# UVA-Computer-Vision-Lab/FrameINO

Hardware: AMD Instinct MI355X
Metric: denoise-steps/sec (Wan2.2-5B FrameINO, 49f 704x1280, cond+uncond DiT forward + CFG + Euler) (higher is better)
Workload: dtype bf16; 1 GPU; wan2.2-5b-49f-704x1280; layers=30, id_frames=1, hip_graph=False, parallelism=single, dead_rows_last_block=1760

## Files before the change

### frameino_amd/_lib.py

```python
import ctypes
import os
import re

_HERE = os.path.dirname(os.path.abspath(__file__))
LIB_PATH = os.environ.get("FINO_LIB_PATH") or os.path.join(_HERE, "lib", "libframeino_hip.so")
HEADER_PATH = os.path.join(os.path.dirname(_HERE), "include", "frameino_hip.h")

c_void_p, c_int, c_i64, c_float = ctypes.c_void_p, ctypes.c_int, ctypes.c_int64, ctypes.c_float

SIGNATURES = {
    "fino_version": [],
    "fino_last_error": [],
    "fino_tune_set": [c_int, c_int],
    "fino_tune_get": [c_int],
    "fino_adaln_modulate": [c_void_p, c_void_p, c_i64, c_int, c_i64, c_i64, c_void_p, c_void_p, c_i64, c_void_p,
                            c_float, c_int, c_void_p],
    "fino_layernorm": [c_void_p, c_void_p, c_i64, c_int, c_i64, c_i64, c_void_p, c_void_p, c_float, c_int, c_void_p],
    "fino_gated_residual": [c_void_p, c_void_p, c_void_p, c_i64, c_int, c_i64, c_i64, c_i64, c_void_p, c_i64,
                            c_void_p, c_int, c_void_p],
    "fino_gated_residual_staged": [c_void_p, c_void_p, c_void_p, c_i64, c_int, c_i64, c_i64, c_i64, c_void_p, c_i64,
                                   c_void_p, c_int, c_void_p],
    "fino_layernorm_zero": [c_void_p, c_void_p, c_i64, c_int, c_i64, c_i64, c_void_p, c_void_p, c_void_p, c_void_p,
                            c_i64, c_void_p, c_float, c_int, c_void_p],
    "fino_rmsnorm_rope": [c_void_p, c_i64, c_int, c_i64, c_void_p, c_float, c_void_p, c_void_p, c_int, c_int,
                          c_void_p],
    "fino_rmsnorm_rope_scaled": [c_void_p, c_i64, c_int, c_i64, c_void_p, c_float, c_void_p, c_void_p, c_int, c_float,
                                 c_int, c_void_p],
    "fino_qkv_rmsnorm_rope": [c_void_p, c_i64, c_int, c_i64, c_void_p, c_float, c_void_p, c_float, c_void_p, c_void_p, c_int,
                              c_float, c_void_p, c_void_p, c_void_p, c_int, c_void_p],
    "fino_rmsnorm_rope_scatter": [c_void_p, c_i64, c_int, c_i64, c_void_p, c_float, c_void_p, c_void_p, c_int, c_float,
                                  c_void_p, c_void_p, c_void_p, c_int, c_void_p],
    "fino_diag_mfma_peak": [c_int, c_int, c_int, c_void_p, ctypes.POINTER(ctypes.c_double), c_void_p],
    "fino_headnorm_rope": [c_void_p, c_int, c_i64, c_int, c_int, c_i64, c_i64, c_void_p, c_void_p, c_float,
                           c_void_p, c_void_p, c_i64, c_int, c_void_p],
    "fino_headnorm_rope_scaled": [c_void_p, c_int, c_i64, c_int, c_int, c_i64, c_i64, c_void_p, c_void_p, c_float,
                                  c_void_p, c_void_p, c_i64, c_float, c_int, c_void_p],
    "fino_attn_fwd": [c_void_p] * 4 + [c_int, c_int, c_i64, c_i64, c_int] + [c_i64] * 12 + [c_float, c_int, c_void_p],
    "fino_attn_fwd_ws": [c_void_p] * 4 + [c_int, c_int, c_i64, c_i64, c_int] + [c_i64] * 12 +
                        [c_float, c_int, c_void_p, c_i64, c_void_p],
    "fino_attn_workspace_bytes": [c_int, c_int, c_i64, c_i64, c_int],
    "fino_attn_tail_supported": [c_int, c_int, c_i64, c_i64, c_int],
    "fino_attn_ranges_supported": [c_int, c_int, c_i64, c_i64, c_int],
    "fino_attn_fwd_ranges": [c_void_p] * 4 + [c_int, c_int, c_i64, c_i64, c_int] + [c_i64] * 12 + [c_float, c_int, c_void_p, c_void_p],
    "fino_attn_tiles_supported": [c_int, c_int, c_i64, c_i64, c_int],
    "fino_attn_fwd_tiles": [c_void_p] * 4 + [c_int, c_int, c_i64, c_i64, c_int] + [c_i64] * 12 + [c_float, c_int, c_void_p, c_i64, c_i64,
                                                                                             c_int, c_void_p],
    "fino_attn_tile_plan_bytes": [c_int, c_int, c_i64, c_i64, c_int],
    "fino_attn_tile_plan": [c_void_p] * 2 + [c_int, c_int, c_i64, c_i64, c_int] + [c_i64] * 6 + [c_float, c_int, c_float, c_void_p,
                                                                                             c_void_p, c_int, c_void_p, c_i64, c_void_p],
    "fino_attn_fp8_ranges_supported": [c_int, c_int, c_i64, c_i64, c_int],
    "fino_attn_fwd_fp8_ranges": [c_void_p] * 4 + [c_int, c_int, c_i64, c_i64, c_int] + [c_i64] * 8 + [c_float, c_int, c_int, c_void_p,
                                                                                               c_i64, c_int, c_void_p, c_void_p],
    "fino_attn_fwd_tail": [c_void_p] * 4 + [c_int, c_int, c_i64, c_i64, c_int] + [c_i64] * 12 + [c_float, c_int, c_void_p, c_void_p,
                                                                                            c_void_p],
    "fino_attn_probs_supported": [c_int, c_int, c_i64, c_i64, c_int],
    "fino_attn_probs": [c_void_p] * 3 + [c_int, c_int, c_i64, c_i64, c_int] + [c_i64] * 6 + [c_int, c_i64, c_i64, c_float, c_int,
                                                                                         c_void_p, c_void_p, c_void_p, c_i64,
                                                                                         c_void_p, c_void_p],
    "fino_row_rrms": [c_void_p, c_i64, c_int, c_i64, c_float, c_void_p, c_int, c_void_p],
    "fino_attn_fp8_kv_bytes": [c_int, c_int, c_i64, c_int],
    "fino_attn_fwd_fp8": [c_void_p] * 4 + [c_int, c_int, c_i64, c_i64, c_int] + [c_i64] * 8 + [c_float, c_int, c_int, c_void_p,
                                                                                           c_i64, c_void_p],
    "fino_attn_fp8_smooth_kv_bytes": [c_int, c_int, c_i64, c_int],
    "fino_attn_fwd_fp8_smooth": [c_void_p] * 4 + [c_int, c_int, c_i64, c_i64, c_int] + [c_i64] * 8 + [c_float, c_int, c_int,
                                                                                                  c_void_p, c_i64, c_void_p],
    "fino_attn_fp8_smoothed_kv_bytes": [c_int, c_int, c_i64, c_int, c_int],
    "fino_attn_fwd_fp8_smoothed": [c_void_p] * 4 + [c_int, c_int, c_i64, c_i64, c_int] + [c_i64] * 8 + [c_float, c_int, c_int,
                                                                                                    c_void_p, c_i64, c_void_p, c_int],
    "fino_attn_partial_bytes": [c_int, c_int, c_i64, c_int],
    "fino_attn_partial": [c_void_p] * 3 + [c_int, c_int, c_i64, c_i64, c_int] + [c_i64] * 9 + [c_float, c_int, c_void_p,
                                                                                               c_i64, c_void_p],
    "fino_attn_merge": [c_void_p, c_int, c_int, c_i64, c_int, c_i64, c_i64, c_i64, c_void_p, c_void_p, c_void_p, c_int,
                        c_void_p],
    "fino_mxfp8_scale_bytes": [c_i64, c_i64],
    "fino_quantize_mxfp8": [c_void_p, c_void_p, c_void_p, c_i64, c_i64, c_i64, c_int, c_void_p],
    "fino_gemm_mxfp8": [c_void_p] * 6 + [c_i64] * 4 + [c_int, c_void_p, c_i64, c_void_p, c_i64, c_void_p, c_int, c_void_p],
    "fino_gemm_mxfp8_keep": [c_void_p] * 6 + [c_i64] * 4 + [c_int, c_void_p, c_i64, c_void_p, c_i64, c_void_p, c_int, c_void_p,
                             c_i64, c_void_p],
    "fino_gemm_mxfp8_q": [c_void_p] * 7 + [c_i64] * 3 + [c_int, c_int, c_void_p],
    "fino_mxfp6_bytes": [c_i64, c_i64],
    "fino_mxfp6_scale_bytes": [c_i64, c_i64],
    "fino_quantize_mxfp6": [c_void_p, c_void_p, c_void_p, c_i64, c_i64, c_i64, c_int, c_void_p],
    "fino_gemm_mxfp6": [c_void_p] * 6 + [c_i64] * 4 + [c_int, c_void_p, c_i64, c_void_p, c_i64, c_void_p, c_int, c_void_p],
    "fino_gemm_mxfp6_keep": [c_void_p] * 6 + [c_i64] * 4 + [c_int, c_void_p, c_i64, c_void_p, c_i64, c_void_p, c_int, c_void_p,
                             c_i64, c_void_p],
    "fino_traj_paint": [c_void_p, c_void_p, c_void_p, c_int, c_int, c_int, c_int, c_void_p],
    "fino_traj_blur_quantize": [c_void_p, c_void_p, c_void_p, c_void_p, c_int, c_int, c_int, c_int, c_void_p],
    "fino_groupnorm_workspace_bytes": [c_int],
    "fino_groupnorm_cl": [c_void_p, c_void_p] + [c_int] * 6 + [c_void_p, c_void_p, c_float, c_void_p, c_void_p] +
                         [c_int] * 4 + [c_void_p, c_i64, c_int, c_void_p],
    "fino_avg_pool_time2": [c_void_p, c_void_p] + [c_int] * 5 + [c_void_p],
    "fino_resize_area_pad_u8": [c_void_p, c_void_p] + [c_int] * 9 + [c_void_p],
    "fino_u8_hwc_to_chw_unit": [c_void_p, c_void_p, c_int, c_int, c_void_p],
    "fino_gemm": [c_void_p] * 4 + [c_i64] * 6 + [c_int, c_void_p, c_i64, c_void_p, c_i64, c_void_p, c_int, c_void_p],
    "fino_gemm_split_n": [c_void_p] * 4 + [c_i64] * 6 + [c_int, c_void_p, c_i64, c_void_p, c_i64, c_void_p, c_int, c_void_p,
                          c_i64, c_i64, c_int, c_void_p],
    "fino_gemm_keep": [c_void_p] * 4 + [c_i64] * 6 + [c_int, c_void_p, c_i64, c_void_p, c_i64, c_void_p, c_int, c_void_p,
                       c_i64, c_int, c_void_p],
    "fino_ln_mxfp8": [c_int, c_void_p, c_void_p, c_void_p, c_i64, c_int, c_i64, c_void_p, c_void_p, c_void_p, c_void_p, c_i64,
                      c_void_p, c_float, c_int, c_void_p],
    "fino_gemm_blocked_a": [c_void_p, c_void_p, c_void_p, c_void_p, c_i64, c_i64, c_i64, c_i64, c_i64, c_int, c_i64, c_i64, c_i64,
                            c_i64, c_void_p, c_i64, c_void_p, c_i64, c_void_p, c_int, c_int, c_void_p],
    "fino_gemm_plan": [c_i64, c_i64, ctypes.POINTER(c_i64), ctypes.POINTER(c_int)],
    "fino_skinny_linear": [c_void_p, c_void_p, c_void_p, c_void_p, c_int, c_i64, c_i64, c_int, c_int, c_void_p],
    "fino_patchify": [c_void_p, c_void_p] + [c_int] * 7 + [c_i64, c_int, c_void_p],
    "fino_unpatchify": [c_void_p, c_void_p] + [c_int] * 7 + [c_i64, c_int, c_void_p],
    "fino_wan_model_input": [c_void_p] * 5 + [c_int] * 6 + [c_void_p],
    "fino_cfg_euler_step": [c_void_p, c_void_p, c_void_p] + [c_int] * 5 + [c_float, c_void_p, c_int, c_int, c_void_p],
    "fino_cfg_unipc_step": [c_void_p] * 6 + [c_int] * 5 + [c_void_p, c_int, c_void_p],
    "fino_cfg_vpred_step": [c_void_p, c_void_p, c_i64, c_i64, c_void_p, c_int, c_int, c_void_p],
    "fino_cfg_dpm_step": [c_void_p, c_void_p, c_void_p, c_void_p, c_i64, c_i64, c_void_p, c_int, c_int, c_void_p],
    "fino_conv3d": [c_void_p] * 4 + [c_int] * 19 + [c_void_p, c_void_p, c_int, c_void_p],
    "fino_rmsnorm_silu_cl": [c_void_p, c_void_p, c_i64, c_int, c_int, c_void_p, c_int, c_int, c_void_p],
    "fino_split_bf16": [c_void_p, c_void_p, c_i64, c_int, c_i64, c_i64, c_int, ctypes.c_uint, c_void_p],
    "fino_rmsnorm_silu_cl_f32": [c_void_p, c_void_p, c_i64, c_int, c_int, c_void_p, c_int, c_int, ctypes.c_uint, c_void_p],
    "fino_conv3d_split": [c_void_p] * 4 + [c_int] * 20 + [c_void_p, c_void_p, c_void_p],
    "fino_vae_blend_tiles": [c_void_p, c_void_p] + [c_int] * 9 + [c_void_p],
    "fino_softmax_rows": [c_void_p, c_i64, c_int, c_i64, c_float, c_int, c_void_p],
    "fino_dup_up3d_add": [c_void_p] * 3 + [c_int] * 10 + [c_void_p],
    "fino_avg_down3d_add": [c_void_p] * 3 + [c_int] * 10 + [c_void_p],
    "fino_vae_unpatchify_clamp": [c_void_p, c_void_p] + [c_int] * 7 + [c_void_p],
    "fino_vae_patchify": [c_void_p, c_void_p] + [c_int] * 7 + [c_void_p],
    "fino_lora_merge": [c_void_p, c_i64, c_void_p, c_i64, c_i64, c_i64, c_int, ctypes.POINTER(c_void_p),
                        ctypes.POINTER(c_i64), ctypes.POINTER(c_void_p), ctypes.POINTER(c_i64), ctypes.POINTER(c_int),
                        ctypes.POINTER(c_float), c_int, c_void_p],
    "fino_step_cache_probe": [c_void_p, c_int, c_i64, c_void_p, c_void_p, c_int, c_void_p],
    "fino_step_cache_residual": [c_void_p, c_i64, c_void_p, c_i64, c_void_p, c_i64, c_i64, c_i64, c_int, c_int, c_void_p],
    "fino_pab_broadcast": [c_void_p, c_i64, c_void_p, c_i64, c_void_p, c_i64, c_i64, c_i64, c_void_p, c_i64, c_void_p, c_int,
                           c_void_p],
}


class StepCacheSegment(ctypes.Structure):
    _fields_ = [("h0", c_void_p), ("h1", c_void_p), ("p", c_void_p), ("r", c_void_p), ("h1_copy", c_void_p),
                ("rows", c_i64), ("ld_h0", c_i64), ("ld_h1", c_i64), ("ld_p", c_i64), ("ld_r", c_i64), ("ld_h1_copy", c_i64)]
_RESTYPES = {"fino_last_error": ctypes.c_char_p, "fino_attn_workspace_bytes": c_i64, "fino_mxfp8_scale_bytes": c_i64,
             "fino_groupnorm_workspace_bytes": c_i64,
             "fino_attn_partial_bytes": c_i64, "fino_attn_fp8_kv_bytes": c_i64, "fino_attn_fp8_smooth_kv_bytes": c_i64,
             "fino_attn_fp8_smoothed_kv_bytes": c_i64, "fino_mxfp6_bytes": c_i64,
             "fino_mxfp6_scale_bytes": c_i64, "fino_attn_tile_plan_bytes": c_i64}


ABI_VERSION = 103


def declared_symbols(header_path=HEADER_PATH):
    text = open(header_path).read()
    text = re.sub(r"/\*.*?\*/", "", text, flags=re.S)
    return sorted(set(re.findall(r"\b(fino_[a-z0-9_]+)\s*\(", text)))


def load(path=LIB_PATH):
    if not os.path.exists(path):
        raise RuntimeError(
            f"frameino_amd: HIP library not found at {path}. Build it with `python -c 'import __graft_entry__ as g; "
            f"g.build()'` (or `make -C frameino_amd/csrc`). There is no CPU fallback for the product path.")
    lib = ctypes.CDLL(path)
    lib.fino_version.restype = c_int
    if lib.fino_version() < 0 and os.environ.get("FINO_ALLOW_EXPERIMENT") != "1":
        raise RuntimeError(
            f"frameino_amd: {path} is a timing-EXPERIMENT build (compiled with -DFINO_EXPERIMENT: its kernels may skip "
            f"work and return wrong results; fino_version() = {lib.fino_version()}).  It is refused as the product library; "
            f"set FINO_ALLOW_EXPERIMENT=1 for the tools/ scripts that time it.")
    if abs(lib.fino_version()) != ABI_VERSION:
        raise RuntimeError(
            f"frameino_amd: {path} reports fino_version() = {lib.fino_version()}, this package binds ABI version "
            f"{ABI_VERSION} (include/frameino_hip.h: FINO_VERSION).  Rebuild it (`make -C frameino_amd/csrc`).")
    for name, argtypes in SIGNATURES.items():
        fn = getattr(lib, name)
        fn.argtypes = argtypes
        fn.restype = _RESTYPES.get(name, c_int)
    return lib


_lib = None


def lib():
    global _lib
    if _lib is None:
        _lib = load()
    return _lib


def check(rc, what=""):
    if rc != 0:
        raise RuntimeError(f"{what} failed ({rc}): {lib().fino_last_error().decode()}")
```

### frameino_amd/csrc/fino_gemm.hip

```cpp
#include <stdlib.h>

#include <atomic>
#include <type_traits>

#include "fino_gemm_common.h"

using namespace fino_gemm_ns;

#ifdef FINO_GEMM_STAMP
extern "C" int fino_gemm_debug_read(unsigned long long* out) {
    return (int)hipMemcpyFromSymbol(out, HIP_SYMBOL(fino_gemm_dbg), sizeof(unsigned long long) * 64);
}
#endif

namespace {

template <typename T, int EPI, bool GENERIC, bool CONV, bool KEEP = false>
__global__ __launch_bounds__(kThreads, 2) void gemm_kernel(const GemmParams p) {
    extern __shared__ __attribute__((aligned(16))) char smem[];
    typedef typename T::vec8 vec8;
    const int tid = threadIdx.x;
    const int lane = tid & 63;
    const int wave = tid >> 6;
    const int wm = wave >> 2;
    const int wn = wave & 3;

    int tm, tn;
    tile_coords(p, tm, tn);
    const int64_t m0 = (int64_t)tm * BM, n0 = (int64_t)tn * BN;

    const int srow = wave * 8 + (lane >> 3);
    const int sch = lane & 7;
    const uint16_t* a_src[4];
    const uint16_t* w_src[4];
    bool a_ok[4], w_ok[4];
    int sk[4];
#pragma unroll
    for (int j = 0; j < 4; ++j) {
        const int row = j * 64 + srow;
        const int lch = sch ^ swz(row);
        sk[j] = lch * 8;
        int64_t gm = m0 + row, gn = n0 + row;
        a_ok[j] = gm < p.m;
        w_ok[j] = gn < p.n;
        if (gm >= p.m) gm = p.m - 1;
        if (gn >= p.n) gn = p.n - 1;
        a_src[j] = p.a + gm * p.lda + sk[j];
        w_src[j] = p.w + gn * p.ldw + sk[j];
    }
    int pos_t[4], pos_h[4], pos_w[4];
    if constexpr (CONV) {
#pragma unroll
        for (int j = 0; j < 4; ++j) {
            int64_t gm = m0 + j * 64 + srow;
            if (gm >= p.m) gm = p.m - 1;
            const int hw = p.ho * p.wo;
            pos_t[j] = (int)(gm / hw);
            const int rem = (int)(gm - (int64_t)pos_t[j] * hw);
            pos_h[j] = rem / p.wo;
            pos_w[j] = rem - pos_h[j] * p.wo;
        }
    }
    auto stage = [&](int buf, int kt) {
        char* ab = smem + buf * kStageBytes;
        char* wb = ab + kTileBytes;
        const int64_t k0 = (int64_t)kt * BK;
        if constexpr (CONV) {
            const int tap = kt / p.cin_chunks;
            const int c0 = (kt - tap * p.cin_chunks) * BK;
            const int dw = tap % p.kw;
            const int dh = (tap / p.kw) % p.kh;
            const int dt = tap / (p.kw * p.kh);
            const int hlim = p.up ? 2 * p.hi : p.hi, wlim = p.up ? 2 * p.wi : p.wi;
#pragma unroll
            for (int j = 0; j < 4; ++j) {
                const int ti = pos_t[j] * p.st + dt - p.pt;
                int hi = pos_h[j] * p.sh + dh - p.ph;
                int wi = pos_w[j] * p.sw + dw - p.pw;
                const bool ok = a_ok[j] && ti >= 0 && ti < p.ti && hi >= 0 && hi < hlim && wi >= 0 && wi < wlim;
                if (p.up) { hi >>= 1; wi >>= 1; }
                const uint16_t* src = ok ? p.a + (((int64_t)ti * p.hi + hi) * p.wi + wi) * p.lda + c0 + sk[j]
                                         : p.zero_page + sk[j];
                __builtin_amdgcn_global_load_lds((const FINO_GLB void*)src,
                                                 (FINO_LDS void*)(ab + j * 8192 + wave * 1024), 16, 0, 0);
                __builtin_amdgcn_global_load_lds((const FINO_GLB void*)(w_src[j] + k0),
                                                 (FINO_LDS void*)(wb + j * 8192 + wave * 1024), 16, 0, 0);
            }
        } else if constexpr (!GENERIC) {
#pragma unroll
            for (int j = 0; j < 4; ++j) {
                __builtin_amdgcn_global_load_lds((const FINO_GLB void*)(a_src[j] + k0),
                                                 (FINO_LDS void*)(ab + j * 8192 + wave * 1024), 16, 0, 0);
                __builtin_amdgcn_global_load_lds((const FINO_GLB void*)(w_src[j] + k0),
                                                 (FINO_LDS void*)(wb + j * 8192 + wave * 1024), 16, 0, 0);
            }
        } else {
#pragma unroll
            for (int j = 0; j < 4; ++j) {
                const bool kin = k0 + sk[j] < p.k;
                uint4 va = make_uint4(0, 0, 0, 0), vw = make_uint4(0, 0, 0, 0);
                if (kin && a_ok[j]) va = *reinterpret_cast<const uint4*>(a_src[j] + k0);
                if (kin && w_ok[j]) vw = *reinterpret_cast<const uint4*>(w_src[j] + k0);
                *reinterpret_cast<uint4*>(ab + j * 8192 + tid * 16) = va;
                *reinterpret_cast<uint4*>(wb + j * 8192 + tid * 16) = vw;
            }
        }
    };

    auto stage_piece = [&](int buf, int kt, int piece) {
        char* ab = smem + buf * kStageBytes;
        char* wb = ab + kTileBytes;
        const int64_t k0 = (int64_t)kt * BK;
        const int j = piece & 3;
        if (piece >= 4) {
            __builtin_amdgcn_global_load_lds((const FINO_GLB void*)(w_src[j] + k0),
                                             (FINO_LDS void*)(wb + j * 8192 + wave * 1024), 16, 0, 0);
        } else if constexpr (CONV) {
            const int tap = kt / p.cin_chunks;
            const int c0 = (kt - tap * p.cin_chunks) * BK;
            const int dw = tap % p.kw;
            const int dh = (tap / p.kw) % p.kh;
            const int dt = tap / (p.kw * p.kh);
            const int hlim = p.up ? 2 * p.hi : p.hi, wlim = p.up ? 2 * p.wi : p.wi;
            const int ti = pos_t[j] * p.st + dt - p.pt;
            int hi = pos_h[j] * p.sh + dh - p.ph;
            int wi = pos_w[j] * p.sw + dw - p.pw;
            const bool ok = a_ok[j] && ti >= 0 && ti < p.ti && hi >= 0 && hi < hlim && wi >= 0 && wi < wlim;
            if (p.up) { hi >>= 1; wi >>= 1; }
            const uint16_t* src = ok ? p.a + (((int64_t)ti * p.hi + hi) * p.wi + wi) * p.lda + c0 + sk[j]
                                     : p.zero_page + sk[j];
            __builtin_amdgcn_global_load_lds((const FINO_GLB void*)src, (FINO_LDS void*)(ab + j * 8192 + wave * 1024),
                                             16, 0, 0);
        } else {
            __builtin_amdgcn_global_load_lds((const FINO_GLB void*)(a_src[j] + k0),
                                             (FINO_LDS void*)(ab + j * 8192 + wave * 1024), 16, 0, 0);
        }
    };

    const int frow = lane & 15;
    const int pch0 = (lane >> 4) ^ (frow >> 1);
    const int a_base = (wm * 128 + frow) * 128;
    const int w_base = kTileBytes + (wn * 64 + frow) * 128;

    f32x4_t acc[8][4];
#pragma unroll
    for (int i = 0; i < 8; ++i)
#pragma unroll
        for (int j = 0; j < 4; ++j) acc[i][j] = f32x4_t{0.f, 0.f, 0.f, 0.f};

    const int nk = (int)((p.k + BK - 1) / BK);
#define LOAD_FRAGS(SB_, KK_, WF_, AF_)                                                                           \
    {                                                                                                            \
        const int pch_ = (pch0 ^ ((KK_) << 2)) << 4;                                                             \
        _Pragma("unroll") for (int j_ = 0; j_ < 4; ++j_)                                                         \
            WF_[j_] = *reinterpret_cast<const u32x4_t*>((SB_) + w_base + j_ * 2048 + pch_);                      \
        _Pragma("unroll") for (int i_ = 0; i_ < 8; ++i_)                                                         \
            AF_[i_] = *reinterpret_cast<const u32x4_t*>((SB_) + a_base + i_ * 2048 + pch_);                      \
    }
#define MFMA_BLOCK(WF_, AF_)                                                                                     \
    _Pragma("unroll") for (int i_ = 0; i_ < 8; ++i_)                                                             \
        _Pragma("unroll") for (int j_ = 0; j_ < 4; ++j_)                                                         \
            acc[i_][j_] = T::mfma16(__builtin_bit_cast(vec8, WF_[j_]), __builtin_bit_cast(vec8, AF_[i_]), acc[i_][j_]);

    if constexpr (GENERIC) {
        stage(0, 0);
        __syncthreads();
        for (int kt = 0; kt < nk; ++kt) {
            const int cur = kt & 1;
            if (kt + 1 < nk) stage(cur ^ 1, kt + 1);
            const char* sb = smem + cur * kStageBytes;
#pragma unroll
            for (int kk = 0; kk < 2; ++kk) {
                u32x4_t wf[4], af[8];
                LOAD_FRAGS(sb, kk, wf, af)
                MFMA_BLOCK(wf, af)
            }
            __syncthreads();
        }
    } else {
        u32x4_t wfa[4], wfb[4], af[8], an;
#define LD_W(SB_, KK_, WF_)                                                                                       \
    _Pragma("unroll") for (int j_ = 0; j_ < 4; ++j_)                                                              \
        WF_[j_] = *reinterpret_cast<const u32x4_t*>((SB_) + w_base + j_ * 2048 + ((pch0 ^ ((KK_) << 2)) << 4));
#define LD_A(SB_, KK_, I_) (*reinterpret_cast<const u32x4_t*>((SB_) + a_base + (I_) * 2048 + ((pch0 ^ ((KK_) << 2)) << 4)))
#define K_STEP(WF_, SBN_, KKN_, HAS_NEXT_, DMA_)                                                                  \
    {                                                                                                             \
        if (HAS_NEXT_) an = LD_A(SBN_, KKN_, 0);                                                                  \
        _Pragma("unroll") for (int i_ = 0; i_ < 8; ++i_) {                                                        \
            if (DMA_) stage_piece(cur, kt + 2, i_);                 \
            _Pragma("unroll") for (int j_ = 0; j_ < 4; ++j_)                                                      \
                acc[i_][j_] = T::mfma16(__builtin_bit_cast(vec8, WF_[j_]), __builtin_bit_cast(vec8, af[i_]),      \
                                        acc[i_][j_]);                                                             \
            if (HAS_NEXT_) {                                                                                      \
                af[i_] = an;                                                                                      \
                if (i_ < 7) an = LD_A(SBN_, KKN_, i_ + 1);                                                        \
            }                                                                                                     \
            __builtin_amdgcn_sched_barrier(0);                                                                    \
        }                                                                                                         \
    }
        stage(0, 0);
        if (nk > 1) stage(1, 1);
        asm volatile("s_waitcnt vmcnt(0)" ::: "memory");
        __builtin_amdgcn_s_barrier();
        LD_W(smem, 0, wfa)
#pragma unroll
        for (int i = 0; i < 8; ++i) af[i] = LD_A(smem, 0, i);
#ifdef FINO_GEMM_STAMP
        unsigned long long t0, t1, t2, t3, t4, acc0 = 0, acc1 = 0, acc2 = 0, acc3 = 0;
#endif
        for (int kt = 0; kt < nk; ++kt) {
            const int cur = kt & 1;
            const char* sb = smem + cur * kStageBytes;
            const char* sbn = smem + (cur ^ 1) * kStageBytes;
#ifdef FINO_GEMM_STAMP
            __builtin_amdgcn_sched_barrier(0); STAMP(t0) __builtin_amdgcn_sched_barrier(0);
#endif
            LD_W(sb, 1, wfb)
            K_STEP(wfa, sb, 1, true, false)
#ifdef FINO_GEMM_STAMP
            __builtin_amdgcn_sched_barrier(0); STAMP(t1) __builtin_amdgcn_sched_barrier(0);
            asm volatile("s_waitcnt vmcnt(0)" ::: "memory");
            __builtin_amdgcn_sched_barrier(0); STAMP(t2) __builtin_amdgcn_sched_barrier(0);
            __builtin_amdgcn_s_barrier();
            __builtin_amdgcn_sched_barrier(0); STAMP(t3) __builtin_amdgcn_sched_barrier(0);
#else
            asm volatile("s_waitcnt vmcnt(0) lgkmcnt(0)" ::: "memory");
            __builtin_amdgcn_s_barrier();
#endif
            __builtin_amdgcn_sched_barrier(0);
            LD_W(sbn, 0, wfa)
            const bool dma = kt + 2 < nk;
            K_STEP(wfb, sbn, 0, true, dma)
#ifdef FINO_GEMM_STAMP
            __builtin_amdgcn_sched_barrier(0); STAMP(t4) __builtin_amdgcn_sched_barrier(0);
            acc0 += t1 - t0; acc1 += t2 - t1; acc2 += t3 - t2; acc3 += t4 - t3;
#endif
        }
#ifdef FINO_GEMM_STAMP
        if (blockIdx.x == 17 && lane == 0) {
            fino_gemm_dbg[wave * 8 + 0] = acc0; fino_gemm_dbg[wave * 8 + 1] = acc1;
            fino_gemm_dbg[wave * 8 + 2] = acc2; fino_gemm_dbg[wave * 8 + 3] = acc3;
            fino_gemm_dbg[wave * 8 + 4] = (unsigned long long)nk;
        }
#endif
        __syncthreads();
    }
#undef LD_W
#undef LD_A
#undef K_STEP
#undef LOAD_FRAGS
#undef MFMA_BLOCK

    gemm_epilogue<T, EPI, false, 8, KEEP>(acc, p, smem, m0, n0, tid, lane, wm, wn);
}

__device__ __forceinline__ int ablk_koff(const GemmParams& p, int kt) {
    const int b = (kt * p.a_inv) >> 16;
    const int j = (b * p.a_ginv) >> 16;
    return (b - j * p.a_groups) * (int)(p.a_grp_elems * 2) + j * (int)(p.a_blk_elems * 2) + (kt - b * p.a_tpb) * (BK * 2);
}

template <typename T, bool CONV, int MI, bool ABLK = false>
__device__ __forceinline__ void pp_mainloop(const GemmParams& p, char* smem, const int64_t m0, const int64_t n0,
                                            const int kb, const int nk, f32x4_t (&acc)[MI][4], const int tid,
                                            const int lane, const int wave, const int wm, const int wn) {
    typedef typename T::vec8 vec8;
    static_assert(MI >= 2 && MI <= 8, "tile height 64 .. 256");
    static_assert(!CONV || MI == 8, "the implicit-GEMM gather is built for 256-row tiles");
    enum : int { NA0 = (MI + 1) / 2, NA1 = MI - (MI + 1) / 2 };

    const int r8 = lane >> 3;
    const int sk = ((lane & 7) ^ ((4 * (wn & 1) + (lane >> 4)) & 7)) * 8;
    const __amdgpu_buffer_rsrc_t w_rsrc = __builtin_amdgcn_make_buffer_rsrc(
        (void*)p.w, 0, (int)(((p.n - 1) * p.ldw + p.k) * 2), 0x00020000);
    const int aq0 = wm == 0 ? 0 : NA0;
    uint32_t a_off[4], w_off[8];
    uint32_t pos[CONV ? 4 : 1];
    int ck = 0, tap_t = 0, tap_h = 0, tap_w = 0, t_first = 0, t_in_first = 0;
    int cseg = 0, seg = 0, a_koff = 0;
    const uint16_t* a_base_ptr = p.a;
    int64_t a_bytes = ((p.m - 1) * p.lda + p.k) * 2;
    if constexpr (ABLK)
        a_bytes = ((p.a_groups - 1) * p.a_grp_elems + (p.k / (BK * p.a_tpb) / p.a_groups - 1) * p.a_blk_elems +
                   (p.m - 1) * p.lda + BK * p.a_tpb) * 2;
    if constexpr (CONV) {
        const int hw = p.ho * p.wo;
        t_first = (int)(m0 / hw);
        t_in_first = t_first * p.st - p.pt;
        t_in_first = t_in_first < 0 ? 0 : t_in_first;
        const int64_t frame = (int64_t)p.hi * p.wi * p.lda;
        a_base_ptr = p.a + (int64_t)t_in_first * frame;
        a_bytes = (int64_t)(p.ti - t_in_first) * frame * 2;
        a_bytes = a_bytes > 0x7fffffffll ? 0x7fffffffll : a_bytes;
#pragma unroll
        for (int q = 0; q < NA0; ++q) {
            int64_t gm = m0 + (aq0 + q) * 32 + wn * 8 + r8;
            gm = gm < p.m ? gm : p.m - 1;
            const int t = (int)(gm / hw);
            const int rem = (int)(gm - (int64_t)t * hw);
            const int h = rem / p.wo;
            pos[q] = ((uint32_t)(t - t_first) << 24) | ((uint32_t)h << 12) | (uint32_t)(rem - h * p.wo);
        }
    }
    const __amdgpu_buffer_rsrc_t a_rsrc = __builtin_amdgcn_make_buffer_rsrc((void*)a_base_ptr, 0, (int)a_bytes, 0x00020000);
    auto conv_offsets = [&]() {
        const int hlim = p.up ? 2 * p.hi : p.hi, wlim = p.up ? 2 * p.wi : p.wi;
#pragma unroll
        for (int q = 0; q < NA0; ++q) {
            const int ti = (t_first + (int)(pos[CONV ? q : 0] >> 24)) * p.st + tap_t - p.pt;
            int hi = (int)((pos[CONV ? q : 0] >> 12) & 0xfffu) * p.sh + tap_h - p.ph;
            int wi = (int)(pos[CONV ? q : 0] & 0xfffu) * p.sw + tap_w - p.pw;
            const bool ok = (unsigned)ti < (unsigned)p.ti && (unsigned)hi < (unsigned)hlim && (unsigned)wi < (unsigned)wlim;
            if (p.up) { hi >>= 1; wi >>= 1; }
            const uint32_t off = (uint32_t)(((((ti - t_in_first) * p.hi + hi) * p.wi + wi) * (int)p.lda + sk) * 2);
            a_off[q] = ok ? off : 0x80000000u;
        }
    };
    auto conv_next = [&]() {
        if (p.a_cc > 0 && ++cseg == p.a_cc) { cseg = 0; ++seg; }
        if (++ck == p.cin_chunks) {
            ck = 0; cseg = 0; seg = 0;
            if (++tap_w == p.kw) {
                tap_w = 0;
                if (++tap_h == p.kh) { tap_h = 0; ++tap_t; }
            }
            conv_offsets();
        }
        if (p.a_cc > 0) {
            const int plane = p.a_nplanes == 3 ? (seg >= 3) + (seg >= 5) : (seg >= 2);
            a_koff = (plane * p.a_cc + cseg) * (BK * 2);
        } else {
            a_koff = ck * (BK * 2);
        }
    };
    if constexpr (CONV) {
        conv_offsets();
    } else {
#pragma unroll
        for (int q = 0; q < NA0; ++q) {
            int64_t gm = m0 + (aq0 + q) * 32 + wn * 8 + r8;
            gm = gm < p.m ? gm : p.m - 1;
            a_off[q] = (uint32_t)((gm * p.lda + sk) * 2);
        }
    }
    const int w_piece_bytes = (int)(32 * p.ldw * 2);
    const int w_pieces = CONV ? (int)((p.n - n0 + 31) / 32) : 8;
#pragma unroll
    for (int q = 0; q < 8; ++q) {
        int64_t gn = n0 + q * 32 + wn * 8 + r8;
        gn = gn < p.n ? gn : p.n - 1;
        w_off[q] = (uint32_t)((gn * p.ldw + sk) * 2);
    }
#ifndef GP_DMA_AUX
#define GP_DMA_AUX 0
#endif
#define PP_DMA_A(STAGE_, KT_, QI_)                                                                                \
    if ((QI_) < NA1 || wm == 0)                                                                                   \
        __builtin_amdgcn_raw_ptr_buffer_load_lds(                                                                 \
            a_rsrc, (FINO_LDS void*)(smem + (STAGE_) * kStageBytes + ((aq0 + (QI_)) * 32 + wn * 8) * 128), 16,    \
            a_off[QI_], CONV ? a_koff : (ABLK ? ablk_koff(p, kb + (KT_)) : (kb + (KT_)) * (BK * 2)), 0, GP_DMA_AUX);
#define PP_DMA_W(STAGE_, KT_, Q_)                                                                                 \
    if (!CONV || (Q_) < w_pieces)                                                                                 \
        __builtin_amdgcn_raw_ptr_buffer_load_lds(                                                                 \
            w_rsrc, (FINO_LDS void*)(smem + (STAGE_) * kStageBytes + kTileBytes + ((Q_) * 32 + wn * 8) * 128), 16, \
            w_off[CONV ? 0 : (Q_)], (kb + (KT_)) * (BK * 2) + (CONV ? (Q_) * w_piece_bytes : 0), 0, GP_DMA_AUX);

    const int frow = lane & 15;
    const int pch0 = (lane >> 4) ^ (frow >> 1);
    const int a_base = (wm * (16 * MI) + frow) * 128;
    const int w_base = kTileBytes + (wn * 64 + frow) * 128;

#pragma unroll
    for (int i = 0; i < MI; ++i)
#pragma unroll
        for (int j = 0; j < 4; ++j) acc[i][j] = f32x4_t{0.f, 0.f, 0.f, 0.f};

#pragma unroll
    for (int q = 0; q < 4; ++q) {
        if (q < NA0) { PP_DMA_A(0, 0, q) }
        if (wm == 0) { PP_DMA_W(0, 0, q) } else { PP_DMA_W(0, 0, 4 + q) }
    }
    if constexpr (CONV) conv_next();
    if (nk > 1) {
#pragma unroll
        for (int q = 0; q < 4; ++q) {
            if (q < NA0) { PP_DMA_A(1, 1, q) }
            if (wm == 0) { PP_DMA_W(1, 1, q) } else { PP_DMA_W(1, 1, 4 + q) }
        }
        if constexpr (CONV) conv_next();
    }
    asm volatile("s_waitcnt vmcnt(0)" ::: "memory");
    __builtin_amdgcn_s_barrier();
    if (wm == 1) __builtin_amdgcn_s_barrier();

    u32x4_t af[2][MI], wf[2][4];
#ifdef FINO_GEMM_STAMP
    unsigned long long t0, t1, t2, t3, t4, acc0 = 0, acc1 = 0, acc2 = 0, acc3 = 0;
#define PSTAMP(V_) { __builtin_amdgcn_sched_barrier(0); STAMP(V_) __builtin_amdgcn_sched_barrier(0); }
#else
#define PSTAMP(V_)
#endif
    for (int t = 0; t < nk; ++t) {
        const int cur = t & 1;
        const char* sb = smem + cur * kStageBytes;
        PSTAMP(t0)
#pragma unroll
        for (int kk = 0; kk < 2; ++kk) {
            const int pch = (pch0 ^ (kk << 2)) << 4;
#pragma unroll
            for (int j = 0; j < 4; ++j) wf[kk][j] = *reinterpret_cast<const u32x4_t*>(sb + w_base + j * 2048 + pch);
#pragma unroll
            for (int i = 0; i < MI; ++i) af[kk][i] = *reinterpret_cast<const u32x4_t*>(sb + a_base + i * 2048 + pch);
        }
        if (t >= 1 && t + 1 < nk) {
#pragma unroll
            for (int q = 0; q < NA0; ++q) PP_DMA_A(cur ^ 1, t + 1, q)
            if (wm == 0) {
#pragma unroll
                for (int q = 0; q < 8; ++q) { PP_DMA_W(cur ^ 1, t + 1, q) }
            }
            if constexpr (CONV) conv_next();
        }
        __builtin_amdgcn_sched_barrier(0);
        asm volatile("s_waitcnt lgkmcnt(0)" ::: "memory");
        PSTAMP(t1)
        __builtin_amdgcn_s_barrier();
        __builtin_amdgcn_sched_barrier(0);
        PSTAMP(t2)
#ifndef GP_ORDER
#define GP_ORDER 3
#endif
#pragma unroll
        for (int kk = 0; kk < 2; ++kk) {
#if GP_ORDER == 0
#pragma unroll
            for (int i = 0; i < MI; ++i) {
#pragma unroll
                for (int j = 0; j < 4; ++j)
                    acc[i][j] = T::mfma16(__builtin_bit_cast(vec8, wf[kk][j]), __builtin_bit_cast(vec8, af[kk][i]),
                                          acc[i][j]);
            }
#elif GP_ORDER == 1
#pragma unroll
            for (int j = 0; j < 4; ++j) {
#pragma unroll
                for (int i = 0; i < MI; ++i)
                    acc[i][j] = T::mfma16(__builtin_bit_cast(vec8, wf[kk][j]), __builtin_bit_cast(vec8, af[kk][i]),
                                          acc[i][j]);
            }
#elif GP_ORDER == 2
#pragma unroll
            for (int j = 0; j < 4; ++j) {
#pragma unroll
                for (int ii = 0; ii < MI; ++ii) {
                    const int i = ((j + 4 * kk) & 1) ? MI - 1 - ii : ii;
                    acc[i][j] = T::mfma16(__builtin_bit_cast(vec8, wf[kk][j]), __builtin_bit_cast(vec8, af[kk][i]),
                                          acc[i][j]);
                }
            }
#else
#pragma unroll
            for (int i = 0; i < MI; ++i) {
#pragma unroll
                for (int jj = 0; jj < 4; ++jj) {
                    const int j = ((i + MI * kk) & 1) ? 3 - jj : jj;
                    acc[i][j] = T::mfma16(__builtin_bit_cast(vec8, wf[kk][j]), __builtin_bit_cast(vec8, af[kk][i]),
                                          acc[i][j]);
                }
            }
#endif
        }
        __builtin_amdgcn_sched_barrier(0);
        asm volatile("s_waitcnt vmcnt(0)" ::: "memory");
        PSTAMP(t3)
        __builtin_amdgcn_s_barrier();
        __builtin_amdgcn_sched_barrier(0);
#ifdef FINO_GEMM_STAMP
        STAMP(t4)
        acc0 += t1 - t0; acc1 += t2 - t1; acc2 += t3 - t2; acc3 += t4 - t3;
#endif
    }
#ifdef FINO_GEMM_STAMP
    if (blockIdx.x == 17 && lane == 0) {
        fino_gemm_dbg[wave * 8 + 0] = acc0; fino_gemm_dbg[wave * 8 + 1] = acc1;
        fino_gemm_dbg[wave * 8 + 2] = acc2; fino_gemm_dbg[wave * 8 + 3] = acc3;
        fino_gemm_dbg[wave * 8 + 4] = (unsigned long long)nk;
    }
#endif
    if (wm == 0) __builtin_amdgcn_s_barrier();
    asm volatile("s_waitcnt vmcnt(0)" ::: "memory");
#undef PP_DMA_A
#undef PP_DMA_W
}

template <typename T, int EPI, bool CONV = false, int MI = 8, bool ABLK = false, bool KEEP = false>
__global__ __launch_bounds__(kThreads, 2) void gemm_pp_kernel(const GemmParams p) {
    extern __shared__ __attribute__((aligned(16))) char smem[];
    const int tid = threadIdx.x;
    const int lane = tid & 63;
    const int wave = __builtin_amdgcn_readfirstlane(tid >> 6);
    const int wm = wave >> 2;
    const int wn = wave & 3;
    int tm, tn;
    tile_coords(p, tm, tn);
    const int64_t m0 = (int64_t)tm * (32 * MI), n0 = (int64_t)tn * BN;
    int nk = (int)(p.k / BK);
#ifndef GP_RAGGED
#define GP_RAGGED 1
#endif
    if constexpr (GP_RAGGED && MI == 8 && !CONV && EPI != FINO_EPI_F32 && EPI != FINO_EPI_F32_RESIDUAL) {
        const int64_t rows = p.m - m0;
        if (rows <= 64) {
            f32x4_t acc2[2][4];
            pp_mainloop<T, false, 2, ABLK>(p, smem, m0, n0, 0, nk, acc2, tid, lane, wave, wm, wn);
            gemm_epilogue<T, EPI, false, 2, KEEP>(acc2, p, smem, m0, n0, tid, lane, wm, wn);
            return;
        }
        if (rows <= 128) {
            f32x4_t acc4[4][4];
            pp_mainloop<T, false, 4, ABLK>(p, smem, m0, n0, 0, nk, acc4, tid, lane, wave, wm, wn);
            gemm_epilogue<T, EPI, false, 4, KEEP>(acc4, p, smem, m0, n0, tid, lane, wm, wn);
            return;
        }
    }
    f32x4_t acc[MI][4];
#ifdef FINO_GEMM_STAMP
    unsigned long long ts0, ts1;
    STAMP(ts0)
#endif
    pp_mainloop<T, CONV, MI, ABLK>(p, smem, m0, n0, 0, nk, acc, tid, lane, wave, wm, wn);
#ifdef FINO_GEMM_STAMP
    STAMP(ts1)
    if (blockIdx.x == 17 && lane == 0) fino_gemm_dbg[wave * 8 + 5] = ts1 - ts0;
#endif
    gemm_epilogue<T, EPI, false, MI, KEEP>(acc, p, smem, m0, n0, tid, lane, wm, wn);
}

template <typename T, int EPI, bool GENERIC, bool CONV = false, bool KEEP = false>
int launch_gemm_t(const GemmParams& p, hipStream_t st) {
    static FinoPerDeviceOnce once;
    if (int rc = fino_max_smem_once(once, reinterpret_cast<const void*>(&gemm_kernel<T, EPI, GENERIC, CONV, KEEP>), kSmemBytes, "fino_gemm")) return rc;
    gemm_kernel<T, EPI, GENERIC, CONV, KEEP><<<dim3((unsigned)(p.tiles_m * p.tiles_n)), kThreads, kSmemBytes, st>>>(p);
    FINO_LAUNCH_CHECK();
    return FINO_OK;
}

template <typename T, int EPI, bool CONV = false, int MI = 8, bool ABLK = false, bool KEEP = false>
int launch_gemm_pp(const GemmParams& p, hipStream_t st) {
    static FinoPerDeviceOnce once;
    if (int rc = fino_max_smem_once(once, reinterpret_cast<const void*>(&gemm_pp_kernel<T, EPI, CONV, MI, ABLK, KEEP>), kSmemBytes, "fino_gemm")) return rc;
    gemm_pp_kernel<T, EPI, CONV, MI, ABLK, KEEP><<<dim3((unsigned)(p.tiles_m * p.tiles_n)), kThreads, kSmemBytes, st>>>(p);
    FINO_LAUNCH_CHECK();
    return FINO_OK;
}

inline int gemm_device_cus() {
    static std::atomic<int> cus[kFinoMaxDevices];
    const int dev = fino_current_device();
    int c = cus[dev].load(std::memory_order_relaxed);
    if (c == 0) {
        int n = 0;
        c = (hipDeviceGetAttribute(&n, hipDeviceAttributeMultiprocessorCount, dev) == hipSuccess && n > 0) ? n : 256;
        cus[dev].store(c, std::memory_order_relaxed);
    }
    return c;
}

struct TilePlan { int64_t rows1; int mi2; };
inline double plan_launch_cost(int64_t rows, int mi, int tiles_n, int cus) {
    if (rows <= 0) return 0.0;
    const double bm = 32.0 * mi;
    const int64_t tiles = ((rows + 32 * mi - 1) / (32 * mi)) * tiles_n;
    const double mfma_raw = 0.85 * bm / 256.0, mfma = mfma_raw > 0.80 ? mfma_raw : 0.80, deliver = (bm + 256.0) / 512.0;
    const int64_t full = tiles / cus, rem = tiles % cus;
    double c = (double)full * (mfma > deliver ? mfma : deliver);
    if (rem) {
        const double d = deliver * (double)rem / cus;
        c += mfma > d ? mfma : d;
    }
    return c + 0.07;
}
inline TilePlan plan_tiles_search(int64_t m, int tiles_n, int cus);
inline TilePlan plan_tiles(int64_t m, int tiles_n, int cus, int tile_m = 0) {
    const int forced = tile_m ? tile_m : fino_tune_get(FINO_TUNE_GEMM_TILE_M);
    if (forced >= 2 && forced <= 7) return TilePlan{0, forced};
    if (forced == 8 || m <= 0) return TilePlan{m, 8};
    static std::atomic<uint64_t> memo[64];
    const bool memoable = m < (1ll << 24) && tiles_n > 0 && tiles_n < 512 && cus > 0 && cus < 512;
    const uint64_t key = ((uint64_t)m << 18) | ((uint64_t)tiles_n << 9) | (uint64_t)cus;
    std::atomic<uint64_t>& slot = memo[(key * 0x9E3779B97F4A7C15ull) >> 58];
    if (memoable) {
        const uint64_t e = slot.load(std::memory_order_relaxed);
        if ((e & 1) && (e >> 22) == key) {
            const uint64_t r = (e >> 6) & 0xffff;
            return TilePlan{r == 0xffff ? m : (int64_t)r * 256, (int)((e >> 3) & 7) + 1};
        }
    }
    const TilePlan tp = plan_tiles_search(m, tiles_n, cus);
    if (memoable && (tp.rows1 == m || (tp.rows1 % 256 == 0 && tp.rows1 / 256 < 0xffff)) && tp.mi2 >= 2 && tp.mi2 <= 8)
        slot.store((key << 22) | ((tp.rows1 == m ? 0xffffull : (uint64_t)(tp.rows1 / 256)) << 6) |
                       ((uint64_t)(tp.mi2 - 1) << 3) | 1ull, std::memory_order_relaxed);
    return tp;
}
inline TilePlan plan_tiles_search(int64_t m, int tiles_n, int cus) {
    TilePlan best{m, 8};
    double best_c = plan_launch_cost(m, 8, tiles_n, cus);
    const double base_c = best_c;
    const int64_t rows256 = (m + 255) / 256;
    for (int64_t r1 = 0; r1 < rows256; ++r1) {
        const int64_t rows1 = r1 * 256;
        const double c1 = plan_launch_cost(rows1, 8, tiles_n, cus);
        for (int mi = 2; mi <= 8; ++mi) {
            if (rows1 > 0 && mi == 8) continue;
            const double c = c1 + plan_launch_cost(m - rows1, mi, tiles_n, cus);
            if (c < best_c - 1e-9) { best_c = c; best = TilePlan{rows1, mi}; }
        }
    }
    if (best_c > (best.rows1 > 0 ? 0.97 : 0.985) * base_c) return TilePlan{m, 8};
    return best;
}

inline bool use_pingpong() {
    static int v = -1;
    if (v < 0) {
        const char* e = getenv("FINO_GEMM_PP");
        v = (e && e[0] == '0') ? 0 : 1;
    }
    return v == 1;
}

template <typename T, int EPI, bool KEEP = false>
int launch_gemm_pp_mi(const GemmParams& p, int mi, hipStream_t st) {
    if constexpr (KEEP) {
        switch (mi) {
            case 2: return launch_gemm_pp<T, EPI, false, 2, false, true>(p, st);
            case 3: return launch_gemm_pp<T, EPI, false, 3, false, true>(p, st);
            case 4: return launch_gemm_pp<T, EPI, false, 4, false, true>(p, st);
            case 5: return launch_gemm_pp<T, EPI, false, 5, false, true>(p, st);
            case 6: return launch_gemm_pp<T, EPI, false, 6, false, true>(p, st);
            case 7: return launch_gemm_pp<T, EPI, false, 7, false, true>(p, st);
            default: return launch_gemm_pp<T, EPI, false, 8, false, true>(p, st);
        }
    }
    if (p.a_tpb > 0) {
        if constexpr (EPI == FINO_EPI_GATED_RESIDUAL) {
            switch (mi) {
                case 2: return launch_gemm_pp<T, EPI, false, 2, true>(p, st);
                case 3: return launch_gemm_pp<T, EPI, false, 3, true>(p, st);
                case 4: return launch_gemm_pp<T, EPI, false, 4, true>(p, st);
                case 5: return launch_gemm_pp<T, EPI, false, 5, true>(p, st);
                case 6: return launch_gemm_pp<T, EPI, false, 6, true>(p, st);
                case 7: return launch_gemm_pp<T, EPI, false, 7, true>(p, st);
                default: return launch_gemm_pp<T, EPI, false, 8, true>(p, st);
            }
        } else {
            fino_set_error("fino_gemm_blocked_a: epilogue must be FINO_EPI_GATED_RESIDUAL");
            return FINO_ERR_UNSUPPORTED;
        }
    }
    switch (mi) {
        case 2: return launch_gemm_pp<T, EPI, false, 2>(p, st);
        case 3: return launch_gemm_pp<T, EPI, false, 3>(p, st);
        case 4: return launch_gemm_pp<T, EPI, false, 4>(p, st);
        case 5: return launch_gemm_pp<T, EPI, false, 5>(p, st);
        case 6: return launch_gemm_pp<T, EPI, false, 6>(p, st);
        case 7: return launch_gemm_pp<T, EPI, false, 7>(p, st);
        default: return launch_gemm_pp<T, EPI, false, 8>(p, st);
    }
}

template <typename T, bool KEEP = false>
int launch_gemm_rows(GemmParams p, int64_t r0, int64_t rows, int mi, int epi, hipStream_t st) {
    p.a += r0 * p.lda;
    p.c += r0 * p.ldc;
    if (p.c2) p.c2 += r0 * p.ldc2;
    if (p.r) p.r += r0 * p.ldr;
    if (p.sel) p.sel += r0;
    p.m = rows;
    p.tiles_m = (int)((rows + 32 * mi - 1) / (32 * mi));
    if constexpr (KEEP) {
        switch (epi) {
            case FINO_EPI_RESIDUAL: return launch_gemm_pp_mi<T, FINO_EPI_RESIDUAL, true>(p, mi, st);
            case FINO_EPI_GATED_RESIDUAL_STAGED: return launch_gemm_pp_mi<T, FINO_EPI_GATED_RESIDUAL_STAGED, true>(p, mi, st);
            default: return launch_gemm_pp_mi<T, FINO_EPI_GATED_RESIDUAL, true>(p, mi, st);
        }
    }
    switch (epi) {
        case FINO_EPI_NONE: return launch_gemm_pp_mi<T, FINO_EPI_NONE>(p, mi, st);
        case FINO_EPI_GELU_TANH: return launch_gemm_pp_mi<T, FINO_EPI_GELU_TANH>(p, mi, st);
        case FINO_EPI_RESIDUAL: return launch_gemm_pp_mi<T, FINO_EPI_RESIDUAL>(p, mi, st);
        case FINO_EPI_GATED_RESIDUAL_STAGED: return launch_gemm_pp_mi<T, FINO_EPI_GATED_RESIDUAL_STAGED>(p, mi, st);
        default: return launch_gemm_pp_mi<T, FINO_EPI_GATED_RESIDUAL>(p, mi, st);
    }
}

template <typename T, bool GENERIC, bool KEEP = false>
int launch_gemm_e(const GemmParams& p, int epi, int tile_m, hipStream_t st) {
    const bool fits32 = ((p.m - 1) * p.lda + p.k) * 2 < (1ll << 31) && ((p.n - 1) * p.ldw + p.k) * 2 < (1ll << 31);
    if (epi == FINO_EPI_F32 || epi == FINO_EPI_F32_RESIDUAL) {
        if (GENERIC || !fits32) {
            fino_set_error("fino_gemm: the fp32-output epilogues need K %% 64 == 0, 16-byte aligned operands and operands < 2 GiB");
            return FINO_ERR_UNSUPPORTED;
        }
        return epi == FINO_EPI_F32 ? launch_gemm_pp<T, FINO_EPI_F32, false, 8>(p, st)
                                   : launch_gemm_pp<T, FINO_EPI_F32_RESIDUAL, false, 8>(p, st);
    }
    if (!GENERIC && use_pingpong() && fits32) {
        const TilePlan tp = plan_tiles(p.m, p.tiles_n, gemm_device_cus(), tile_m);
        if (tp.rows1 > 0)
            if (int rc = launch_gemm_rows<T, KEEP>(p, 0, tp.rows1, 8, epi, st)) return rc;
        if (tp.rows1 < p.m) return launch_gemm_rows<T, KEEP>(p, tp.rows1, p.m - tp.rows1, tp.mi2, epi, st);
        return FINO_OK;
    }
    if constexpr (KEEP) {
        switch (epi) {
            case FINO_EPI_RESIDUAL: return launch_gemm_t<T, FINO_EPI_RESIDUAL, GENERIC, false, true>(p, st);
            case FINO_EPI_GATED_RESIDUAL_STAGED: return launch_gemm_t<T, FINO_EPI_GATED_RESIDUAL_STAGED, GENERIC, false, true>(p, st);
            default: return launch_gemm_t<T, FINO_EPI_GATED_RESIDUAL, GENERIC, false, true>(p, st);
        }
    }
    switch (epi) {
        case FINO_EPI_NONE: return launch_gemm_t<T, FINO_EPI_NONE, GENERIC>(p, st);
        case FINO_EPI_GELU_TANH: return launch_gemm_t<T, FINO_EPI_GELU_TANH, GENERIC>(p, st);
        case FINO_EPI_RESIDUAL: return launch_gemm_t<T, FINO_EPI_RESIDUAL, GENERIC>(p, st);
        case FINO_EPI_GATED_RESIDUAL_STAGED: return launch_gemm_t<T, FINO_EPI_GATED_RESIDUAL_STAGED, GENERIC>(p, st);
        default: return launch_gemm_t<T, FINO_EPI_GATED_RESIDUAL, GENERIC>(p, st);
    }
}

template <int WT>
__global__ __launch_bounds__(256) void skinny_linear_kernel(const float* __restrict__ x, const void* __restrict__ w,
                                                            const void* __restrict__ b, float* __restrict__ y, int m,
                                                            int64_t n, int64_t k, int silu_input) {
    const int lane = threadIdx.x & 63;
    const int64_t col = (int64_t)blockIdx.x * 4 + (threadIdx.x >> 6);
    if (col >= n) return;
    float acc[16];
#pragma unroll
    for (int i = 0; i < 16; ++i) acc[i] = 0.f;
    for (int64_t kk = lane; kk < k; kk += 64) {
        float wv;
        if (WT == -1) wv = ((const float*)w)[col * k + kk];
        else if (WT == FINO_BF16) wv = BF16::to_f32(((const uint16_t*)w)[col * k + kk]);
        else wv = F16::to_f32(((const uint16_t*)w)[col * k + kk]);
#pragma unroll
        for (int i = 0; i < 16; ++i) {
            if (i < m) {
                float xv = x[(int64_t)i * k + kk];
                if (silu_input) xv = xv / (1.0f + __expf(-xv));
                acc[i] += xv * wv;
            }
        }
    }
    float bias = 0.f;
    if (b) {
        if (WT == -1) bias = ((const float*)b)[col];
        else if (WT == FINO_BF16) bias = BF16::to_f32(((const uint16_t*)b)[col]);
        else bias = F16::to_f32(((const uint16_t*)b)[col]);
    }
#pragma unroll
    for (int i = 0; i < 16; ++i) {
        if (i < m) {
            const float s = wave_sum(acc[i]);
            if (lane == 0) y[(int64_t)i * n + col] = s + bias;
        }
    }
}

}

extern "C" int fino_gemm_plan(int64_t m, int64_t n, int64_t* rows_256, int* tile_rows_rest) {
    if (m <= 0 || n <= 0) return FINO_ERR_ARG;
    const TilePlan tp = plan_tiles(m, (int)((n + BN - 1) / BN), gemm_device_cus());
    if (rows_256) *rows_256 = tp.rows1;
    if (tile_rows_rest) *tile_rows_rest = tp.rows1 < m ? 32 * tp.mi2 : 0;
    return FINO_OK;
}

extern "C" int fino_gemm(const void* a, const void* w, const void* bias, void* c, int64_t m, int64_t n, int64_t k,
                         int64_t lda, int64_t ldw, int64_t ldc, int epilogue, const void* r, int64_t ldr,
                         const float* gate, int64_t mod_stride, const int32_t* sel, int dtype, void* stream) {
    return fino_gemm_split_n(a, w, bias, c, m, n, k, lda, ldw, ldc, epilogue, r, ldr, gate, mod_stride, sel, dtype, nullptr,
                             0, 0, 0, stream);
}

static int gemm_impl(const void* a, const void* w, const void* bias, void* c, int64_t m, int64_t n, int64_t k, int64_t lda,
                     int64_t ldw, int64_t ldc, int epilogue, const void* r, int64_t ldr, const float* gate,
                     int64_t mod_stride, const int32_t* sel, int dtype, void* c2, int64_t ldc2, int64_t n_split, void* keep,
                     int64_t ldk, int tile_m, void* stream) {
    FINO_CHECK(dtype == FINO_BF16 || dtype == FINO_F16, FINO_ERR_ARG, "fino_gemm: dtype %d", dtype);
    FINO_CHECK(tile_m == 0 || (tile_m >= 2 && tile_m <= 8), FINO_ERR_ARG, "fino_gemm: tile_m=%d (0 = planned, 2 .. 8)", tile_m);
    if (c2 || n_split) {
        FINO_CHECK(c2 && n_split > 0 && n_split < n && n_split % BN == 0 && ldc2 % 8 == 0 && ldc2 >= n - n_split &&
                       fino_aligned16(c2) && k % BK == 0 && epilogue <= FINO_EPI_GELU_TANH,
                   FINO_ERR_ARG,
                   "fino_gemm_split_n: needs c2, 0 < n_split < N a multiple of %d, ldc2 >= N - n_split, K %% %d == 0, no "
                   "residual epilogue", BN, BK);
        FINO_CHECK(ldc >= n_split, FINO_ERR_ARG, "fino_gemm_split_n: ldc must cover the first n_split columns");
    }
    FINO_CHECK(a && w && c, FINO_ERR_ARG, "fino_gemm: null pointer");
    FINO_CHECK(m >= 0 && n > 0 && k > 0, FINO_ERR_ARG, "fino_gemm: bad shape M=%lld N=%lld K=%lld", (long long)m,
               (long long)n, (long long)k);
    FINO_CHECK(n % 8 == 0 && k % 8 == 0, FINO_ERR_ARG, "fino_gemm: N=%lld and K=%lld must be multiples of 8",
               (long long)n, (long long)k);
    FINO_CHECK(lda % 8 == 0 && ldw % 8 == 0 && ldc % 8 == 0 && lda >= k && ldw >= k && ldc >= (n_split > 0 ? n_split : n),
               FINO_ERR_ARG, "fino_gemm: leading dimensions must be multiples of 8 and cover the row");
    FINO_CHECK(fino_aligned16(a) && fino_aligned16(w) && fino_aligned16(c), FINO_ERR_ARG,
               "fino_gemm: A/W/C must be 16-byte aligned");
    FINO_CHECK(epilogue >= FINO_EPI_NONE && epilogue <= FINO_EPI_F32_RESIDUAL, FINO_ERR_ARG,
               "fino_gemm: epilogue %d", epilogue);
    if (epilogue == FINO_EPI_F32 || epilogue == FINO_EPI_F32_RESIDUAL)
        FINO_CHECK(!c2 && tile_m == 0 && fino_aligned16(bias), FINO_ERR_ARG,
                   "fino_gemm: the fp32-output epilogues take one output, the planned tiling and a 16-byte aligned fp32 bias");
    if (epilogue >= FINO_EPI_RESIDUAL && epilogue != FINO_EPI_F32)
        FINO_CHECK(r && ldr % 8 == 0 && ldr >= n && fino_aligned16(r), FINO_ERR_ARG, "fino_gemm: residual operand");
    if (epilogue == FINO_EPI_GATED_RESIDUAL || epilogue == FINO_EPI_GATED_RESIDUAL_STAGED)
        FINO_CHECK(gate && fino_aligned16(gate) && mod_stride % 4 == 0, FINO_ERR_ARG, "fino_gemm: gate operand");
    if (m == 0) return FINO_OK;
    GemmParams p = {};
    p.c2 = (uint16_t*)c2; p.ldc2 = ldc2; p.n_split = n_split;
    if (keep) { p.c2 = (uint16_t*)keep; p.ldc2 = ldk; p.n_split = 0; }
    p.a = (const uint16_t*)a; p.w = (const uint16_t*)w; p.bias = (const uint16_t*)bias; p.c = (uint16_t*)c;
    p.r = (const uint16_t*)r; p.gate = gate; p.sel = sel;
    p.m = m; p.n = n; p.k = k; p.lda = lda; p.ldw = ldw; p.ldc = ldc; p.ldr = ldr; p.mod_stride = mod_stride;
    p.tiles_m = (int)((m + BM - 1) / BM);
    p.tiles_n = (int)((n + BN - 1) / BN);
    p.group_m = fino_tune_get(FINO_TUNE_GEMM_GROUP_M);
    hipStream_t st = (hipStream_t)stream;
    const bool generic = (k % BK) != 0;
    if (p.group_m <= 0) p.group_m = gemm_default_group_m(p.tiles_n, k);
    {
        const int rk = fino_tune_get(FINO_TUNE_GEMM_RASTER);
        if (rk == 1 || (rk == 3 && (k >= 8192 || n >= 8192)) || (rk != 2 && rk != 3 && k >= 8192)) p.group_m |= 0x100;
    }
    if (keep) {
        if (dtype == FINO_BF16)
            return generic ? launch_gemm_e<BF16, true, true>(p, epilogue, tile_m, st)
                           : launch_gemm_e<BF16, false, true>(p, epilogue, tile_m, st);
        return generic ? launch_gemm_e<F16, true, true>(p, epilogue, tile_m, st)
                       : launch_gemm_e<F16, false, true>(p, epilogue, tile_m, st);
    }
    if (dtype == FINO_BF16)
        return generic ? launch_gemm_e<BF16, true>(p, epilogue, tile_m, st) : launch_gemm_e<BF16, false>(p, epilogue, tile_m, st);
    return generic ? launch_gemm_e<F16, true>(p, epilogue, tile_m, st) : launch_gemm_e<F16, false>(p, epilogue, tile_m, st);
}

extern "C" int fino_gemm_split_n(const void* a, const void* w, const void* bias, void* c, int64_t m, int64_t n, int64_t k,
                                 int64_t lda, int64_t ldw, int64_t ldc, int epilogue, const void* r, int64_t ldr,
                                 const float* gate, int64_t mod_stride, const int32_t* sel, int dtype, void* c2,
                                 int64_t ldc2, int64_t n_split, int tile_m, void* stream) {
    return gemm_impl(a, w, bias, c, m, n, k, lda, ldw, ldc, epilogue, r, ldr, gate, mod_stride, sel, dtype, c2, ldc2, n_split,
                     nullptr, 0, tile_m, stream);
}

extern "C" int fino_gemm_keep(const void* a, const void* w, const void* bias, void* c, int64_t m, int64_t n, int64_t k,
                              int64_t lda, int64_t ldw, int64_t ldc, int epilogue, const void* r, int64_t ldr,
                              const float* gate, int64_t mod_stride, const int32_t* sel, int dtype, void* keep, int64_t ldk,
                              int tile_m, void* stream) {
    FINO_CHECK(dtype == FINO_BF16 || dtype == FINO_F16, FINO_ERR_ARG, "fino_gemm_keep: dtype %d", dtype);
    FINO_CHECK(epilogue == FINO_EPI_RESIDUAL || epilogue == FINO_EPI_GATED_RESIDUAL ||
                   epilogue == FINO_EPI_GATED_RESIDUAL_STAGED,
               FINO_ERR_ARG, "fino_gemm_keep: epilogue %d (the residual epilogues %d, %d and %d keep y)", epilogue,
               FINO_EPI_RESIDUAL, FINO_EPI_GATED_RESIDUAL, FINO_EPI_GATED_RESIDUAL_STAGED);
    FINO_CHECK(keep && fino_aligned16(keep) && ldk % 8 == 0 && ldk >= n, FINO_ERR_ARG,
               "fino_gemm_keep: needs a 16-byte aligned keep buffer with ldk >= N a multiple of 8");
    return gemm_impl(a, w, bias, c, m, n, k, lda, ldw, ldc, epilogue, r, ldr, gate, mod_stride, sel, dtype, nullptr, 0, 0,
                     keep, ldk, tile_m, stream);
}

extern "C" int fino_gemm_blocked_a(const void* a, const void* w, const void* bias, void* c, int64_t m, int64_t n, int64_t k,
                                   int64_t a_block_k, int64_t a_block_stride, int a_groups, int64_t a_group_stride,
                                   int64_t lda, int64_t ldw, int64_t ldc,
                                   const void* r, int64_t ldr, const float* gate, int64_t mod_stride, const int32_t* sel,
                                   int dtype, int tile_m, void* stream) {
    FINO_CHECK(dtype == FINO_BF16 || dtype == FINO_F16, FINO_ERR_ARG, "fino_gemm_blocked_a: dtype %d", dtype);
    FINO_CHECK(tile_m == 0 || (tile_m >= 2 && tile_m <= 8), FINO_ERR_ARG, "fino_gemm_blocked_a: tile_m=%d (0 = planned, 2 .. 8)",
               tile_m);
    FINO_CHECK(a && w && c && r && gate, FINO_ERR_ARG, "fino_gemm_blocked_a: null pointer");
    FINO_CHECK(m >= 0 && n > 0 && k > 0 && n % 8 == 0, FINO_ERR_ARG, "fino_gemm_blocked_a: bad shape");
    FINO_CHECK(a_block_k > 0 && a_block_k % BK == 0 && k % a_block_k == 0 && a_block_k / BK <= 256 && k / BK <= 4096,
               FINO_ERR_ARG, "fino_gemm_blocked_a: a_block_k=%lld must be a multiple of %d dividing K=%lld",
               (long long)a_block_k, BK, (long long)k);
    FINO_CHECK(lda % 8 == 0 && lda >= a_block_k && a_block_stride % 8 == 0 && ldw % 8 == 0 && ldw >= k && ldc % 8 == 0 &&
                   ldc >= n && ldr % 8 == 0 && ldr >= n && mod_stride % 4 == 0,
               FINO_ERR_ARG, "fino_gemm_blocked_a: leading dimensions");
    FINO_CHECK(fino_aligned16(a) && fino_aligned16(w) && fino_aligned16(c) && fino_aligned16(r) && fino_aligned16(gate),
               FINO_ERR_ARG, "fino_gemm_blocked_a: 16-byte alignment required");
    const int64_t nblk = k / a_block_k;
    FINO_CHECK(a_groups >= 1 && a_groups <= 16 && nblk % a_groups == 0 && a_group_stride % 8 == 0, FINO_ERR_ARG,
               "fino_gemm_blocked_a: a_groups=%d must divide the %lld K blocks", a_groups, (long long)nblk);
    const int64_t span = ((a_groups - 1) * a_group_stride + (nblk / a_groups - 1) * a_block_stride +
                          (m > 0 ? m - 1 : 0) * lda + a_block_k) * 2;
    FINO_CHECK(span < (1ll << 31) && ((n - 1) * ldw + k) * 2 < (1ll << 31), FINO_ERR_ARG,
               "fino_gemm_blocked_a: operands must span < 2 GiB");
    if (m == 0) return FINO_OK;
    GemmParams p = {};
    p.a = (const uint16_t*)a; p.w = (const uint16_t*)w; p.bias = (const uint16_t*)bias; p.c = (uint16_t*)c;
    p.r = (const uint16_t*)r; p.gate = gate; p.sel = sel;
    p.m = m; p.n = n; p.k = k; p.lda = lda; p.ldw = ldw; p.ldc = ldc; p.ldr = ldr; p.mod_stride = mod_stride;
    p.a_tpb = (int)(a_block_k / BK); p.a_inv = (65536 + p.a_tpb - 1) / p.a_tpb; p.a_blk_elems = a_block_stride;
    p.a_groups = a_groups; p.a_ginv = (65536 + a_groups - 1) / a_groups; p.a_grp_elems = a_group_stride;
    FINO_CHECK((k / BK - 1) * ((int64_t)p.a_inv * p.a_tpb - 65536) < 65536 &&
                   (nblk - 1) * ((int64_t)p.a_ginv * a_groups - 65536) < 65536,
               FINO_ERR_UNSUPPORTED,
               "fino_gemm_blocked_a: a_block_k=%lld / a_groups=%d with K=%lld is beyond the exact range of the kernel's "
               "reciprocal index arithmetic", (long long)a_block_k, a_groups, (long long)k);
    p.tiles_m = (int)((m + BM - 1) / BM);
    p.tiles_n = (int)((n + BN - 1) / BN);
    p.group_m = fino_tune_get(FINO_TUNE_GEMM_GROUP_M);
    if (p.group_m <= 0) p.group_m = gemm_default_group_m(p.tiles_n, k);
    hipStream_t st = (hipStream_t)stream;
    const TilePlan tp = plan_tiles(p.m, p.tiles_n, gemm_device_cus(), tile_m);
    auto rows = [&](int64_t r0, int64_t nr, int mi) {
        return dtype == FINO_BF16 ? launch_gemm_rows<BF16>(p, r0, nr, mi, FINO_EPI_GATED_RESIDUAL, st)
                                  : launch_gemm_rows<F16>(p, r0, nr, mi, FINO_EPI_GATED_RESIDUAL, st);
    };
    if (tp.rows1 > 0)
        if (int rc = rows(0, tp.rows1, 8)) return rc;
    if (tp.rows1 < p.m) return rows(tp.rows1, p.m - tp.rows1, tp.mi2);
    return FINO_OK;
}

static int conv3d_impl(const void* x, const void* w, const void* bias, void* y, int t_in, int h_in, int w_in,
                       int c_in_pad, int t_out, int h_out, int w_out, int c_out_pad, int kt, int kh, int kw, int st,
                       int sh, int sw, int pt, int ph, int pw, int upsample2x, int epilogue, const void* r,
                       const void* zero_page, int dtype, int planes, void* stream);

extern "C" int fino_conv3d(const void* x, const void* w, const void* bias, void* y, int t_in, int h_in, int w_in,
                           int c_in_pad, int t_out, int h_out, int w_out, int c_out_pad, int kt, int kh, int kw, int st,
                           int sh, int sw, int pt, int ph, int pw, int upsample2x, int epilogue, const void* r,
                           const void* zero_page, int dtype, void* stream) {
    return conv3d_impl(x, w, bias, y, t_in, h_in, w_in, c_in_pad, t_out, h_out, w_out, c_out_pad, kt, kh, kw, st, sh, sw, pt, ph,
                       pw, upsample2x, epilogue, r, zero_page, dtype, 0, stream);
}

extern "C" int fino_conv3d_split(const void* x_planes, const void* w_products, const float* bias, float* y, int t_in, int h_in,
                                 int w_in, int c_in_pad, int planes, int t_out, int h_out, int w_out, int c_out_pad, int kt,
                                 int kh, int kw, int st, int sh, int sw, int pt, int ph, int pw, int upsample2x, int epilogue,
                                 const float* r, const void* zero_page, void* stream) {
    FINO_CHECK(planes == 2 || planes == 3, FINO_ERR_ARG, "fino_conv3d_split: planes = %d (2: hi | lo, 3: hi | mid | lo)", planes);
    return conv3d_impl(x_planes, w_products, bias, y, t_in, h_in, w_in, c_in_pad, t_out, h_out, w_out, c_out_pad, kt, kh, kw, st,
                       sh, sw, pt, ph, pw, upsample2x, epilogue, r, zero_page, FINO_BF16, planes, stream);
}

static int conv3d_impl(const void* x, const void* w, const void* bias, void* y, int t_in, int h_in, int w_in,
                       int c_in_pad, int t_out, int h_out, int w_out, int c_out_pad, int kt, int kh, int kw, int st,
                       int sh, int sw, int pt, int ph, int pw, int upsample2x, int epilogue, const void* r,
                       const void* zero_page, int dtype, int planes, void* stream) {
    FINO_CHECK(dtype == FINO_BF16 || dtype == FINO_F16, FINO_ERR_ARG, "fino_conv3d: dtype %d", dtype);
    FINO_CHECK(x && w && y && zero_page, FINO_ERR_ARG, "fino_conv3d: null pointer");
    FINO_CHECK(c_in_pad > 0 && c_in_pad % BK == 0, FINO_ERR_ARG,
               "fino_conv3d: c_in_pad=%d must be a multiple of %d (pad channels with zeros)", c_in_pad, BK);
    FINO_CHECK(c_out_pad > 0 && c_out_pad % 8 == 0, FINO_ERR_ARG, "fino_conv3d: c_out_pad=%d %% 8 != 0", c_out_pad);
    FINO_CHECK(t_in > 0 && h_in > 0 && w_in > 0 && t_out > 0 && h_out > 0 && w_out > 0 && kt > 0 && kh > 0 && kw > 0 &&
                   st > 0 && sh > 0 && sw > 0 && pt >= 0 && ph >= 0 && pw >= 0,
               FINO_ERR_ARG, "fino_conv3d: bad geometry");
    FINO_CHECK(epilogue == FINO_EPI_NONE || (epilogue == FINO_EPI_RESIDUAL && r), FINO_ERR_ARG,
               "fino_conv3d: epilogue %d (NONE or RESIDUAL with r)", epilogue);
    FINO_CHECK(fino_aligned16(x) && fino_aligned16(w) && fino_aligned16(y) && fino_aligned16(r) &&
                   fino_aligned16(zero_page),
               FINO_ERR_ARG, "fino_conv3d: 16-byte alignment required");
    FINO_CHECK(planes == 0 || fino_aligned16(bias), FINO_ERR_ARG, "fino_conv3d_split: bias must be 16-byte aligned");
    const int products = planes == 0 ? 1 : (planes == 2 ? 3 : 6);
    const int64_t a_width = (int64_t)(planes == 0 ? 1 : planes) * c_in_pad;
    GemmParams p = {};
    p.a = (const uint16_t*)x; p.w = (const uint16_t*)w; p.bias = (const uint16_t*)bias; p.c = (uint16_t*)y;
    p.r = (const uint16_t*)r; p.gate = nullptr; p.sel = nullptr;
    p.m = (int64_t)t_out * h_out * w_out; p.n = c_out_pad; p.k = (int64_t)kt * kh * kw * c_in_pad * products;
    p.lda = a_width; p.ldw = p.k; p.ldc = c_out_pad; p.ldr = c_out_pad; p.mod_stride = 0;
    p.a_cc = planes == 0 ? 0 : c_in_pad / BK; p.a_nplanes = planes;
    p.tiles_m = (int)((p.m + BM - 1) / BM); p.tiles_n = (int)((p.n + BN - 1) / BN);
    p.group_m = fino_tune_get(FINO_TUNE_GEMM_GROUP_M);
    p.to = t_out; p.ho = h_out; p.wo = w_out; p.ti = t_in; p.hi = h_in; p.wi = w_in;
    p.kt = kt; p.kh = kh; p.kw = kw; p.st = st; p.sh = sh; p.sw = sw; p.pt = pt; p.ph = ph; p.pw = pw;
    p.up = upsample2x; p.cin_chunks = c_in_pad / BK * products; p.zero_page = (const uint16_t*)zero_page;
    hipStream_t s = (hipStream_t)stream;
    const int64_t hw_out = (int64_t)h_out * w_out;
    const int64_t t_span = (BM - 1 + hw_out - 1) / hw_out + 1;
    const int64_t in_span_bytes = (t_span * st + kt) * (int64_t)h_in * w_in * a_width * 2;
    const bool pp = use_pingpong() && fino_tune_get(FINO_TUNE_CONV_LOOP) != 1 && in_span_bytes < (1ll << 31) &&
                    h_out < 4096 && w_out < 4096 && t_span < 256 && c_out_pad % 32 == 0 && ((p.n - 1) * p.ldw + p.k) * 2 < (1ll << 31);
    if (planes > 0) {
        if (!pp) {
            fino_set_error("fino_conv3d_split: a 256-row tile's input span (%lld bytes) exceeds the 2 GiB the gather offsets cover, "
                           "or c_out_pad %% 32 != 0 -- run the layer in chunks of fewer frames", (long long)in_span_bytes);
            return FINO_ERR_UNSUPPORTED;
        }
        return epilogue == FINO_EPI_NONE ? launch_gemm_pp<BF16, FINO_EPI_F32, true>(p, s)
                                         : launch_gemm_pp<BF16, FINO_EPI_F32_RESIDUAL, true>(p, s);
    }
    if (pp) {
        if (dtype == FINO_BF16)
            return epilogue == FINO_EPI_NONE ? launch_gemm_pp<BF16, FINO_EPI_NONE, true>(p, s)
                                             : launch_gemm_pp<BF16, FINO_EPI_RESIDUAL, true>(p, s);
        return epilogue == FINO_EPI_NONE ? launch_gemm_pp<F16, FINO_EPI_NONE, true>(p, s)
                                         : launch_gemm_pp<F16, FINO_EPI_RESIDUAL, true>(p, s);
    }
    if (dtype == FINO_BF16)
        return epilogue == FINO_EPI_NONE ? launch_gemm_t<BF16, FINO_EPI_NONE, false, true>(p, s)
                                         : launch_gemm_t<BF16, FINO_EPI_RESIDUAL, false, true>(p, s);
    return epilogue == FINO_EPI_NONE ? launch_gemm_t<F16, FINO_EPI_NONE, false, true>(p, s)
                                     : launch_gemm_t<F16, FINO_EPI_RESIDUAL, false, true>(p, s);
}

extern "C" int fino_skinny_linear(const float* x, const void* w, const void* b, float* y, int m, int64_t n,
                                  int64_t k, int w_dtype, int silu_input, void* stream) {
    FINO_CHECK(x && w && y, FINO_ERR_ARG, "fino_skinny_linear: null pointer");
    FINO_CHECK(m >= 1 && m <= 16 && n > 0 && k > 0, FINO_ERR_ARG, "fino_skinny_linear: need 1 <= M <= 16 (M=%d)", m);
    FINO_CHECK(w_dtype == -1 || w_dtype == FINO_BF16 || w_dtype == FINO_F16, FINO_ERR_ARG,
               "fino_skinny_linear: w_dtype %d", w_dtype);
    const dim3 grid((unsigned)((n + 3) / 4));
    hipStream_t st = (hipStream_t)stream;
    if (w_dtype == -1) skinny_linear_kernel<-1><<<grid, 256, 0, st>>>(x, w, b, y, m, n, k, silu_input);
    else if (w_dtype == FINO_BF16) skinny_linear_kernel<FINO_BF16><<<grid, 256, 0, st>>>(x, w, b, y, m, n, k, silu_input);
    else skinny_linear_kernel<FINO_F16><<<grid, 256, 0, st>>>(x, w, b, y, m, n, k, silu_input);
    FINO_LAUNCH_CHECK();
    return FINO_OK;
}
```

### frameino_amd/csrc/fino_gemm_common.h

```cpp
#pragma once
#include <type_traits>

#include "fino_common.h"

#ifdef FINO_GEMM_STAMP
__device__ unsigned long long fino_gemm_dbg[8 * 8];
#define STAMP(V_) { asm volatile("s_memtime %0\n\ts_waitcnt lgkmcnt(0)" : "=s"(V_) :: "memory"); }
#endif

namespace fino_gemm_ns {

constexpr int BM = 256, BN = 256, BK = 64;
constexpr int kThreads = 512;
constexpr int kTileBytes = BM * BK * 2;
constexpr int kStageBytes = 2 * kTileBytes;
constexpr int kCsStride = BN * 2 + 16;
constexpr int kSmemBytes = (2 * kStageBytes > BM * kCsStride) ? 2 * kStageBytes : BM * kCsStride;

struct GemmParams {
    const uint16_t* a;
    const uint16_t* w;
    const uint16_t* bias;
    uint16_t* c;
    const uint16_t* r;
    const float* gate;
    const int32_t* sel;
    int64_t m, n, k, lda, ldw, ldc, ldr, mod_stride;
    int tiles_m, tiles_n;
    int group_m;
    uint16_t* c2;
    int64_t ldc2, n_split;
    int a_tpb, a_inv;
    int64_t a_blk_elems;
    int a_groups, a_ginv;
    int64_t a_grp_elems;
    int to, ho, wo, ti, hi, wi;
    int kt, kh, kw, st, sh, sw, pt, ph, pw, up, cin_chunks;
    const uint16_t* zero_page;
    int a_cc, a_nplanes;
    uint8_t* cq;
    uint8_t* cs;
    int64_t cs_rows_pad;
};

__device__ __forceinline__ uint2 mx_quant8(const float (&v)[8], int& e_out) {
    float amax = 0.f;
#pragma unroll
    for (int j = 0; j < 8; ++j) amax = fmaxf(amax, fabsf(v[j]));
    amax = fmaxf(amax, __shfl_xor(amax, 1, 64));
    amax = fmaxf(amax, __shfl_xor(amax, 2, 64));
    int e = -127;
    if (amax > 0.f) {
        int ex;
        (void)frexpf(amax * (1.0f / 448.0f), &ex);
        e = ex < -127 ? -127 : (ex > 127 ? 127 : ex);
    }
    const float inv = __builtin_amdgcn_ldexpf(1.0f, -e);
    int w0 = 0, w1 = 0;
    w0 = __builtin_amdgcn_cvt_pk_fp8_f32(v[0] * inv, v[1] * inv, w0, false);
    w0 = __builtin_amdgcn_cvt_pk_fp8_f32(v[2] * inv, v[3] * inv, w0, true);
    w1 = __builtin_amdgcn_cvt_pk_fp8_f32(v[4] * inv, v[5] * inv, w1, false);
    w1 = __builtin_amdgcn_cvt_pk_fp8_f32(v[6] * inv, v[7] * inv, w1, true);
    e_out = e;
    return make_uint2((uint32_t)w0, (uint32_t)w1);
}

__device__ __forceinline__ int64_t mx_scale_index(int64_t row, int64_t col, int64_t rows_pad) {
    const int rr = (int)(row & 255);
    return ((col >> 7) * (rows_pad >> 8) + (row >> 8)) * 1024 + ((col >> 5) & 3) * 256 + (rr & 15) * 16 + (rr >> 4);
}

__device__ __forceinline__ float gelu_tanh_f32(float x) {
    const float c1 = 2.0f * 0.7978845608028654f * 1.4426950408889634f;
    const float c3 = 0.044715f * c1;
    const float e = __builtin_amdgcn_exp2f(-x * (c3 * x * x + c1));
    return x * __builtin_amdgcn_rcpf(1.0f + e);
}

inline int gemm_default_group_m(int tiles_n, int64_t k) {
    if (k >= 8192) return 1;
    if (tiles_n >= 48) return 2;
    if (tiles_n <= 12) return 16;
    return 4;
}

__device__ __forceinline__ int swz(int row) { return (row >> 1) & 7; }

__device__ __forceinline__ int xcd_remap(int orig, int nwg) {
    const int xcd = orig & 7, q = nwg >> 3, rr = nwg & 7;
    return (xcd < rr ? xcd * (q + 1) : rr * (q + 1) + (xcd - rr) * q) + (orig >> 3);
}
__device__ __forceinline__ void tile_raster(const GemmParams& p, int id, int& tm, int& tn) {
    const int GROUP_M = (p.group_m & 0xff) > 0 ? (p.group_m & 0xff) : 4;
    const int group = id / (GROUP_M * p.tiles_n);
    const int first_m = group * GROUP_M;
    const int gsz = (p.tiles_m - first_m) < GROUP_M ? (p.tiles_m - first_m) : GROUP_M;
    const int in_group = id - group * GROUP_M * p.tiles_n;
    tm = first_m + in_group % gsz;
    tn = in_group / gsz;
    if (p.group_m & 0x100) tm = p.tiles_m - 1 - tm;
}
__device__ __forceinline__ void tile_coords(const GemmParams& p, int& tm, int& tn) {
    tile_raster(p, xcd_remap((int)blockIdx.x, p.tiles_m * p.tiles_n), tm, tn);
}

template <typename T>
__device__ __forceinline__ void gemm_load_bias(const GemmParams& p, int64_t n0, int lane, int wn, float (&bv)[4][4]) {
    const bool fast = p.bias && n0 + BN <= p.n && (reinterpret_cast<uintptr_t>(p.bias) & 7) == 0;
    if (fast) {
        uint2 b4[4];
#pragma unroll
        for (int j = 0; j < 4; ++j)
            b4[j] = *reinterpret_cast<const uint2*>(p.bias + n0 + wn * 64 + j * 16 + (lane >> 4) * 4);
#pragma unroll
        for (int j = 0; j < 4; ++j) {
            bv[j][0] = T::to_f32((uint16_t)(b4[j].x & 0xffffu)); bv[j][1] = T::to_f32((uint16_t)(b4[j].x >> 16));
            bv[j][2] = T::to_f32((uint16_t)(b4[j].y & 0xffffu)); bv[j][3] = T::to_f32((uint16_t)(b4[j].y >> 16));
        }
    } else {
#pragma unroll
        for (int j = 0; j < 4; ++j) {
#pragma unroll
            for (int e = 0; e < 4; ++e) {
                int64_t gn = n0 + wn * 64 + j * 16 + (lane >> 4) * 4 + e;
                if (gn >= p.n) gn = p.n - 1;
                bv[j][e] = p.bias ? T::to_f32(p.bias[gn]) : 0.f;
            }
        }
    }
}

template <int EPI, int MI>
__device__ __forceinline__ void gemm_epilogue_f32(f32x4_t (&acc)[MI][4], const GemmParams& p, int64_t m0, int64_t n0, int lane,
                                                  int wm, int wn) {
    const float* bias = reinterpret_cast<const float*>(p.bias);
    const float* r = reinterpret_cast<const float*>(p.r);
    float* c = reinterpret_cast<float*>(p.c);
#pragma unroll
    for (int j = 0; j < 4; ++j) {
        const int64_t gn = n0 + wn * 64 + j * 16 + (lane >> 4) * 4;
        if (gn >= p.n) continue;
        float4 b4 = make_float4(0.f, 0.f, 0.f, 0.f);
        if (bias) b4 = *reinterpret_cast<const float4*>(bias + gn);
#pragma unroll
        for (int i = 0; i < MI; ++i) {
            const int64_t gm = m0 + wm * (16 * MI) + i * 16 + (lane & 15);
            if (gm >= p.m) continue;
            float4 y = make_float4(acc[i][j][0] + b4.x, acc[i][j][1] + b4.y, acc[i][j][2] + b4.z, acc[i][j][3] + b4.w);
            if (EPI == FINO_EPI_F32_RESIDUAL) {
                const float4 rv = *reinterpret_cast<const float4*>(r + gm * p.ldr + gn);
                y.x += rv.x; y.y += rv.y; y.z += rv.z; y.w += rv.w;
            }
            *reinterpret_cast<float4*>(c + gm * p.ldc + gn) = y;
        }
    }
}

template <typename T, int EPI, bool QOUT, int MI, bool KEEP = false>
__device__ __forceinline__ void gemm_epilogue_t(f32x4_t (&acc)[MI][4], const GemmParams& p, char* smem, int64_t m0,
                                                int64_t n0, int tid, int lane, int wm, int wn) {
    constexpr bool kHasRes =
        EPI == FINO_EPI_RESIDUAL || EPI == FINO_EPI_GATED_RESIDUAL || EPI == FINO_EPI_GATED_RESIDUAL_STAGED;
    constexpr bool kGated = EPI == FINO_EPI_GATED_RESIDUAL || EPI == FINO_EPI_GATED_RESIDUAL_STAGED;
    constexpr int kIters = (32 * MI * BN / 8) / kThreads;
#ifdef FINO_GEMM_STAMP
    unsigned long long te0, te1, te2;
    __builtin_amdgcn_sched_barrier(0); STAMP(te0) __builtin_amdgcn_sched_barrier(0);
#endif
    float bv[4][4];
    gemm_load_bias<T>(p, n0, lane, wn, bv);
    __builtin_amdgcn_sched_barrier(0);
    uint4 rres[kHasRes ? kIters : 1];
    int rsel[kGated ? kIters : 1];
    constexpr int kFirst = MI == 8 ? kIters / 2 : kIters;
    auto load_residual = [&](int it0, int it1) {
#pragma unroll
        for (int it = 0; it < kIters; ++it) {
            if (it < it0 || it >= it1) continue;
            const int idx = it * kThreads + tid;
            int64_t gm = m0 + (idx >> 5), gn = n0 + (idx & 31) * 8;
            gm = gm < p.m ? gm : p.m - 1;
            gn = gn < p.n ? gn : p.n - 8;
            rres[kHasRes ? it : 0] = *reinterpret_cast<const uint4*>(p.r + gm * p.ldr + gn);
            if (kGated) rsel[kGated ? it : 0] = p.sel ? p.sel[gm] : 0;
        }
    };
    if (kHasRes) load_residual(0, kFirst);
    __builtin_amdgcn_sched_barrier(0);
#pragma unroll
    for (int i = 0; i < MI; ++i) {
        const int row = wm * (16 * MI) + i * 16 + (lane & 15);
#pragma unroll
        for (int j = 0; j < 4; ++j) {
            float y[4];
#pragma unroll
            for (int e = 0; e < 4; ++e) {
                y[e] = acc[i][j][e] + bv[j][e];
                if (EPI == FINO_EPI_GELU_TANH) y[e] = gelu_tanh_f32(round_to<T>(y[e]));
            }
            const uint32_t w0 = (uint32_t)T::from_f32(y[0]) | ((uint32_t)T::from_f32(y[1]) << 16);
            const uint32_t w1 = (uint32_t)T::from_f32(y[2]) | ((uint32_t)T::from_f32(y[3]) << 16);
            const int col = wn * 64 + j * 16 + (lane >> 4) * 4;
            *reinterpret_cast<uint2*>(smem + row * kCsStride + col * 2) = make_uint2(w0, w1);
        }
    }
    __builtin_amdgcn_sched_barrier(0);
    asm volatile("s_waitcnt lgkmcnt(0)" ::: "memory");
    __builtin_amdgcn_s_barrier();
    __builtin_amdgcn_sched_barrier(0);
    if (kHasRes && kFirst < kIters) load_residual(kFirst, kIters);
    __builtin_amdgcn_sched_barrier(0);
#ifdef FINO_GEMM_STAMP
    __builtin_amdgcn_sched_barrier(0); STAMP(te1) __builtin_amdgcn_sched_barrier(0);
#endif
    int gsel = -1;
    float gg[8] = {0.f, 0.f, 0.f, 0.f, 0.f, 0.f, 0.f, 0.f};
#pragma unroll
    for (int it = 0; it < kIters; ++it) {
        const int idx = it * kThreads + tid;
        const int row = idx >> 5;
        const int ch = idx & 31;
        const int64_t gm = m0 + row, gn = n0 + ch * 8;
        if (gm >= p.m || gn >= p.n) continue;
        uint4 yv = *reinterpret_cast<const uint4*>(smem + row * kCsStride + ch * 16);
        if constexpr (KEEP) *reinterpret_cast<uint4*>(p.c2 + gm * p.ldc2 + gn) = yv;
        if (kHasRes) {
            float y[8], rv[8], o[8];
            unpack8<T>(yv, y);
            unpack8<T>(rres[kHasRes ? it : 0], rv);
            if (kGated) {
                if (rsel[kGated ? it : 0] != gsel) {
                    gsel = rsel[kGated ? it : 0];
                    const float* g = p.gate + (int64_t)gsel * p.mod_stride + gn;
                    const float4 g0 = *reinterpret_cast<const float4*>(g);
                    const float4 g1 = *reinterpret_cast<const float4*>(g + 4);
                    gg[0] = g0.x; gg[1] = g0.y; gg[2] = g0.z; gg[3] = g0.w;
                    gg[4] = g1.x; gg[5] = g1.y; gg[6] = g1.z; gg[7] = g1.w;
                }
#pragma unroll
                for (int e = 0; e < 8; ++e)
                    o[e] = rv[e] + (EPI == FINO_EPI_GATED_RESIDUAL_STAGED ? round_to<T>(y[e] * gg[e]) : y[e] * gg[e]);
            } else {
#pragma unroll
                for (int e = 0; e < 8; ++e) o[e] = rv[e] + y[e];
            }
            yv = pack8<T>(o);
        }
        if constexpr (QOUT) {
            float y[8];
            unpack8<T>(yv, y);
            int e;
            const uint2 qv = mx_quant8(y, e);
            *reinterpret_cast<uint2*>(p.cq + gm * p.n + gn) = qv;
            if ((ch & 3) == 0) p.cs[mx_scale_index(gm, gn, p.cs_rows_pad)] = (uint8_t)(e + 127);
        } else if (p.n_split > 0 && n0 >= p.n_split) {
            *reinterpret_cast<uint4*>(p.c2 + gm * p.ldc2 + (gn - p.n_split)) = yv;
        } else {
            *reinterpret_cast<uint4*>(p.c + gm * p.ldc + gn) = yv;
        }
    }
#ifdef FINO_GEMM_STAMP
    __builtin_amdgcn_sched_barrier(0); STAMP(te2) __builtin_amdgcn_sched_barrier(0);
    if (blockIdx.x == 17 && (tid & 63) == 0) {
        fino_gemm_dbg[(tid >> 6) * 8 + 6] = te1 - te0;
        fino_gemm_dbg[(tid >> 6) * 8 + 7] = te2 - te1;
    }
#endif
}

template <typename T, int EPI, bool QOUT = false, int MI = 8, bool KEEP = false>
__device__ __forceinline__ void gemm_epilogue(f32x4_t (&acc)[MI][4], const GemmParams& p, char* smem, int64_t m0,
                                              int64_t n0, int tid, int lane, int wm, int wn) {
    if constexpr (EPI == FINO_EPI_F32 || EPI == FINO_EPI_F32_RESIDUAL)
        gemm_epilogue_f32<EPI, MI>(acc, p, m0, n0, lane, wm, wn);
    else
        gemm_epilogue_t<T, EPI, QOUT, MI, KEEP>(acc, p, smem, m0, n0, tid, lane, wm, wn);
}

struct MxGemmParams {
    GemmParams g;
    const uint8_t* sa;
    const uint8_t* sw;
    int64_t m_pad, n_pad;
};

inline int mx_gemm_params(MxGemmParams& fp, const char* who, bool qout, const void* aq, const void* a_scales, const void* wq,
                          const void* w_scales, const void* bias, void* c, int64_t m, int64_t n, int64_t k, int64_t ldc,
                          int epilogue, const void* r, int64_t ldr, const float* gate, int64_t mod_stride,
                          const int32_t* sel, int dtype) {
    FINO_CHECK(dtype == FINO_BF16 || dtype == FINO_F16, FINO_ERR_ARG, "%s: dtype %d", who, dtype);
    FINO_CHECK(aq && a_scales && wq && w_scales && (qout || c), FINO_ERR_ARG, "%s: null pointer", who);
    FINO_CHECK(m >= 0 && n > 0 && k > 0 && k % 128 == 0 && n % 8 == 0, FINO_ERR_ARG,
               "%s: K=%lld must be a multiple of 128, N=%lld of 8", who, (long long)k, (long long)n);
    FINO_CHECK((qout || (ldc % 8 == 0 && ldc >= n && fino_aligned16(c))) && fino_aligned16(aq) && fino_aligned16(wq) &&
                   fino_aligned16(a_scales) && fino_aligned16(w_scales),
               FINO_ERR_ARG, "%s: alignment / leading dimension", who);
    FINO_CHECK(epilogue >= FINO_EPI_NONE && epilogue <= FINO_EPI_GATED_RESIDUAL_STAGED, FINO_ERR_ARG, "%s: epilogue %d", who,
               epilogue);
    if (epilogue >= FINO_EPI_RESIDUAL)
        FINO_CHECK(r && ldr % 8 == 0 && ldr >= n && fino_aligned16(r), FINO_ERR_ARG, "%s: residual operand", who);
    if (epilogue == FINO_EPI_GATED_RESIDUAL || epilogue == FINO_EPI_GATED_RESIDUAL_STAGED)
        FINO_CHECK(gate && fino_aligned16(gate) && mod_stride % 4 == 0, FINO_ERR_ARG, "%s: gate operand", who);
    fp = {};
    GemmParams& p = fp.g;
    p.a = (const uint16_t*)aq; p.w = (const uint16_t*)wq; p.bias = (const uint16_t*)bias; p.c = (uint16_t*)c;
    p.r = (const uint16_t*)r; p.gate = gate; p.sel = sel;
    p.m = m; p.n = n; p.k = k; p.lda = k; p.ldw = k; p.ldc = ldc; p.ldr = ldr; p.mod_stride = mod_stride;
    p.tiles_m = (int)((m + BM - 1) / BM);
    p.tiles_n = (int)((n + BN - 1) / BN);
    p.group_m = fino_tune_get(FINO_TUNE_GEMM_GROUP_M);
    fp.sa = (const uint8_t*)a_scales; fp.sw = (const uint8_t*)w_scales;
    fp.m_pad = (m + 255) / 256 * 256; fp.n_pad = (n + 255) / 256 * 256;
    return FINO_OK;
}

template <typename F>
int mx_dispatch_epilogue(int epi, F&& launch) {
    switch (epi) {
        case FINO_EPI_NONE: return launch(std::integral_constant<int, FINO_EPI_NONE>{});
        case FINO_EPI_GELU_TANH: return launch(std::integral_constant<int, FINO_EPI_GELU_TANH>{});
        case FINO_EPI_RESIDUAL: return launch(std::integral_constant<int, FINO_EPI_RESIDUAL>{});
        case FINO_EPI_GATED_RESIDUAL_STAGED: return launch(std::integral_constant<int, FINO_EPI_GATED_RESIDUAL_STAGED>{});
        default: return launch(std::integral_constant<int, FINO_EPI_GATED_RESIDUAL>{});
    }
}

inline int mx_gemm_keep_params(MxGemmParams& fp, const char* who, int epilogue, void* keep, int64_t ldk) {
    FINO_CHECK(epilogue == FINO_EPI_RESIDUAL || epilogue == FINO_EPI_GATED_RESIDUAL ||
                   epilogue == FINO_EPI_GATED_RESIDUAL_STAGED,
               FINO_ERR_ARG, "%s: epilogue %d (the residual epilogues %d, %d and %d keep y)", who, epilogue,
               FINO_EPI_RESIDUAL, FINO_EPI_GATED_RESIDUAL, FINO_EPI_GATED_RESIDUAL_STAGED);
    FINO_CHECK(keep && fino_aligned16(keep) && ldk % 8 == 0 && ldk >= fp.g.n, FINO_ERR_ARG,
               "%s: needs a 16-byte aligned keep buffer with ldk >= N a multiple of 8", who);
    fp.g.c2 = (uint16_t*)keep; fp.g.ldc2 = ldk; fp.g.n_split = 0;
    return FINO_OK;
}

template <typename F>
int mx_dispatch_keep_epilogue(int epi, F&& launch) {
    switch (epi) {
        case FINO_EPI_RESIDUAL: return launch(std::integral_constant<int, FINO_EPI_RESIDUAL>{});
        case FINO_EPI_GATED_RESIDUAL_STAGED: return launch(std::integral_constant<int, FINO_EPI_GATED_RESIDUAL_STAGED>{});
        default: return launch(std::integral_constant<int, FINO_EPI_GATED_RESIDUAL>{});
    }
}

}
```

### frameino_amd/ops.py

```python
import os

import torch

from . import _lib

BF16, F16 = 0, 1
EPI_NONE, EPI_GELU_TANH, EPI_RESIDUAL, EPI_GATED_RESIDUAL, EPI_GATED_RESIDUAL_STAGED = 0, 1, 2, 3, 4
EPI_F32, EPI_F32_RESIDUAL = 5, 6


class KernelTimer:

    active = None

    def __init__(self, names):
        self.names = set(names)
        self.events = {n: [] for n in self.names}
        self.flops = {}
        self.bytes = {}

    def __enter__(self):
        KernelTimer.active = self
        return self

    def __exit__(self, *exc):
        KernelTimer.active = None

    def summary(self):
        torch.cuda.synchronize()
        out = {}
        for n, evs in self.events.items():
            ms = [s.elapsed_time(e) for s, e in evs]
            if ms:
                out[n] = {"launches": len(ms), "avg_us": 1e3 * sum(ms) / len(ms), "total_ms": sum(ms)}
        return out


def _timed(name):
    kt = KernelTimer.active
    if kt is None or name not in kt.names:
        return None
    s, e = torch.cuda.Event(enable_timing=True), torch.cuda.Event(enable_timing=True)
    kt.events[name].append((s, e))
    s.record()
    return e


def _timed_gemm(epilogue, flops, nbytes=0.0):
    kt = KernelTimer.active
    if kt is None:
        return None
    name = "gemm" if epilogue is None else f"gemm_epi{int(epilogue)}"
    if name not in kt.names:
        name = "gemm"
        if name not in kt.names:
            return None
    ev = _timed(name)

    def done():
        ev.record()
        kt.flops[name] = kt.flops.get(name, 0.0) + flops
        kt.bytes[name] = kt.bytes.get(name, 0.0) + nbytes
    return done


def _dt(t):
    if t.dtype == torch.bfloat16:
        return BF16
    if t.dtype == torch.float16:
        return F16
    raise TypeError(f"frameino_amd: activations must be bf16 or fp16, got {t.dtype}")


F32 = 2


def _dt3(t):
    return F32 if t.dtype == torch.float32 else _dt(t)


def _stream():
    return torch.cuda.current_stream().cuda_stream


def _p(t):
    return 0 if t is None else t.data_ptr()


def _rows2d(t):
    if not t.is_cuda:
        raise RuntimeError("frameino_amd ops need CUDA(HIP) tensors; there is no CPU path")
    if t.stride(-1) != 1:
        raise ValueError("last dimension must be contiguous")
    t2 = t if t.dim() == 2 else t.reshape(-1, t.shape[-1]) if t.is_contiguous() else None
    if t2 is None:
        if t.dim() == 3 and t.shape[0] == 1:
            t2 = t[0]
        else:
            raise ValueError("need a 2-D row-strided view")
    return t2, t2.shape[0], t2.shape[1], t2.stride(0)


def _epi_operands(residual, gate):
    r2, ldr = (None, 0)
    if residual is not None:
        r2, _, _, ldr = _rows2d(residual)
    return r2, ldr, gate.stride(0) if (gate is not None and gate.dim() == 2) else 0


def _mx_pair(shape, scale_bytes, device, out):
    if out is not None:
        return out
    return (torch.empty(shape, dtype=torch.uint8, device=device), torch.zeros(scale_bytes, dtype=torch.uint8, device=device))


def adaln_modulate(x, shift, scale, sel=None, eps=1e-6, out=None):
    x2, rows, dim, ldx = _rows2d(x)
    out = torch.empty_like(x2) if out is None else out
    o2, _, _, ldy = _rows2d(out)
    assert shift.dtype == torch.float32 and scale.dtype == torch.float32
    ms = shift.stride(0) if shift.dim() == 2 else 0
    if scale.dim() == 2:
        assert scale.stride(0) == ms
    _lib.check(_lib.lib().fino_adaln_modulate(_p(x2), _p(o2), rows, dim, ldx, ldy, _p(shift), _p(scale), ms, _p(sel),
                                             eps, _dt(x), _stream()), "fino_adaln_modulate")
    return out.view(x.shape) if out.shape != x.shape and out.numel() == x.numel() else out


def layernorm(x, weight=None, bias=None, eps=1e-5, out=None):
    x2, rows, dim, ldx = _rows2d(x)
    out = torch.empty_like(x2) if out is None else out
    o2, _, _, ldy = _rows2d(out)
    for t in (weight, bias):
        assert t is None or t.dtype == torch.float32
    _lib.check(_lib.lib().fino_layernorm(_p(x2), _p(o2), rows, dim, ldx, ldy, _p(weight), _p(bias), eps, _dt(x),
                                        _stream()), "fino_layernorm")
    return out.view(x.shape) if out.shape != x.shape and out.numel() == x.numel() else out


def layernorm_zero(x, weight, bias, shift, scale, sel=None, eps=1e-5, out=None):
    x2, rows, dim, ldx = _rows2d(x)
    out = torch.empty_like(x2) if out is None else out
    o2, _, _, ldy = _rows2d(out)
    for t in (weight, bias, shift, scale):
        assert t is None or t.dtype == torch.float32
    ms = shift.stride(0) if shift.dim() == 2 else 0
    _lib.check(_lib.lib().fino_layernorm_zero(_p(x2), _p(o2), rows, dim, ldx, ldy, _p(weight), _p(bias), _p(shift),
                                             _p(scale), ms, _p(sel), eps, _dt(x), _stream()), "fino_layernorm_zero")
    return out.view(x.shape) if out.shape != x.shape and out.numel() == x.numel() else out


def gated_residual(x, y, gate=None, sel=None, out=None, staged=False):
    x2, rows, dim, ldx = _rows2d(x)
    y2, _, _, ldy = _rows2d(y)
    out = torch.empty_like(x2) if out is None else out
    o2, _, _, ldo = _rows2d(out)
    ms = gate.stride(0) if (gate is not None and gate.dim() == 2) else 0
    fn = _lib.lib().fino_gated_residual_staged if staged else _lib.lib().fino_gated_residual
    _lib.check(fn(_p(x2), _p(y2), _p(o2), rows, dim, ldx, ldy, ldo, _p(gate), ms, _p(sel), _dt(x), _stream()),
               "fino_gated_residual")
    return out.view(x.shape) if out.shape != x.shape and out.numel() == x.numel() else out


SCALE_FOLDED = -1.0
LOG2E = 1.4426950408889634


def rmsnorm_rope_(x, weight, eps, cos=None, sin=None, head_dim=0, out_scale=1.0):
    x2, rows, dim, ldx = _rows2d(x)
    if cos is not None:
        assert cos.dtype == torch.float32 and cos.is_contiguous() and cos.shape == (rows, head_dim // 2)
        assert sin.dtype == torch.float32 and sin.is_contiguous() and sin.shape == cos.shape
    _lib.check(_lib.lib().fino_rmsnorm_rope_scaled(_p(x2), rows, dim, ldx, _p(weight), eps, _p(cos), _p(sin), head_dim,
                                                  float(out_scale), _dt(x), _stream()), "fino_rmsnorm_rope")
    return x


def qkv_rmsnorm_rope_(qkv, dim, q_weight, q_eps, k_weight, k_eps, cos, sin, head_dim, q_out_scale=1.0, out=None,
                      head_off=None, head_ld=None):
    x2, rows, width, ldx = _rows2d(qkv)
    assert width == 3 * dim
    assert cos.dtype == torch.float32 and cos.is_contiguous() and cos.shape == (rows, head_dim // 2) and sin.shape == cos.shape
    if out is not None:
        assert head_off.dtype == torch.int64 and head_off.numel() == 3 * (dim // head_dim) and head_off.is_contiguous()
        assert head_ld.dtype == torch.int64 and head_ld.numel() == dim // head_dim and out.is_contiguous()
    _lib.check(_lib.lib().fino_qkv_rmsnorm_rope(_p(x2), rows, dim, ldx, _p(q_weight), q_eps, _p(k_weight), k_eps, _p(cos),
                                                _p(sin), head_dim, float(q_out_scale), _p(out), _p(head_off), _p(head_ld),
                                                _dt(qkv), _stream()), "fino_qkv_rmsnorm_rope")
    return qkv if out is None else out


def rmsnorm_rope_scatter(x, weight, eps, cos, sin, head_dim, out, head_off, head_ld, out_scale=1.0):
    x2, rows, dim, ldx = _rows2d(x)
    assert head_off.dtype == torch.int64 and head_ld.dtype == torch.int64 and head_off.is_cuda and head_ld.is_cuda
    assert head_off.numel() == dim // head_dim == head_ld.numel() and out.is_contiguous() and out.dtype == x.dtype
    if cos is not None:
        assert cos.dtype == torch.float32 and cos.is_contiguous() and cos.shape == (rows, head_dim // 2)
        assert sin.dtype == torch.float32 and sin.is_contiguous() and sin.shape == cos.shape
    _lib.check(_lib.lib().fino_rmsnorm_rope_scatter(_p(x2), rows, dim, ldx, _p(weight), eps, _p(cos), _p(sin), head_dim,
                                                    float(out_scale), _p(out), _p(head_off), _p(head_ld), _dt(x),
                                                    _stream()), "fino_rmsnorm_rope_scatter")
    return out


def headnorm_rope_(x, heads, head_dim, weight, bias, eps, cos=None, sin=None, rope_row0=0, out_scale=1.0):
    assert x.dim() == 3 and x.stride(2) == 1
    b, rows, _ = x.shape
    _lib.check(_lib.lib().fino_headnorm_rope_scaled(_p(x), b, rows, heads, head_dim, x.stride(1), x.stride(0), _p(weight),
                                                   _p(bias), eps, _p(cos), _p(sin), rope_row0, float(out_scale), _dt(x),
                                                   _stream()), "fino_headnorm_rope")
    return x


SPLIT_ATTENTION_TAIL = os.environ.get("FINO_ATTN_SPLIT", "1") != "0"
_attn_ws = {}


def _attention_workspace(b, heads, lq, lk, dh, device):
    need = _lib.lib().fino_attn_workspace_bytes(b, heads, lq, lk, dh)
    if need <= 0:
        return None, 0
    key = (device.index, torch.cuda.current_stream().cuda_stream)
    ws = _attn_ws.get(key)
    if ws is None or ws.numel() * 4 < need:
        ws = _attn_ws[key] = torch.empty(need // 4, dtype=torch.float32, device=device)
    return ws, need


def _attn_args(q, k, v, heads, out, scale):
    assert q.dim() == 3 and k.dim() == 3 and v.dim() == 3
    b, lq, hd = q.shape
    lk = k.shape[1]
    dh = hd // heads
    for t in (q, k, v):
        assert t.stride(2) == 1 and t.is_cuda
    if out is None:
        out = torch.empty((b, lq, hd), dtype=q.dtype, device=q.device)
    scale = dh ** -0.5 if scale is None else scale
    return b, lq, lk, hd, dh, out, scale


def _check_ranges(ranges, lq):
    nqb = (lq + 255) // 256
    assert ranges.dtype == torch.int32 and ranges.is_cuda and ranges.is_contiguous() and tuple(ranges.shape) == (nqb, 3, 2), \
        f"ranges: an int32 device tensor [{nqb}, 3, 2] is needed, got {ranges.dtype} {tuple(ranges.shape)} on {ranges.device}"


def _timed_attn(b, lq, lk, hd, ranges=None, nbytes=False):
    name = "attn_self" if ranges is not None or lk > 1024 else "attn_cross"
    ev = _timed(name)
    if ev is None:
        return None

    def done():
        ev.record()
        kt_ = KernelTimer.active
        pairs = lq * lk if ranges is None else _ranges_pairs(ranges, lq, lk)
        kt_.flops[name] = kt_.flops.get(name, 0.0) + 4.0 * b * pairs * hd
        if nbytes:
            kt_.bytes[name] = kt_.bytes.get(name, 0.0) + 2.0 * b * hd * (2 * lq + 2 * lk)
    return done


def attention(q, k, v, heads, out=None, scale=None):
    b, lq, lk, hd, dh, out, scale = _attn_args(q, k, v, heads, out, scale)
    done = _timed_attn(b, lq, lk, hd, nbytes=True)
    ws, ws_bytes = _attention_workspace(b, heads, lq, lk, dh, q.device) if SPLIT_ATTENTION_TAIL else (None, 0)
    _lib.check(_lib.lib().fino_attn_fwd_ws(_p(q), _p(k), _p(v), _p(out), b, heads, lq, lk, dh,
                                          q.stride(0), q.stride(1), dh, k.stride(0), k.stride(1), dh,
                                          v.stride(0), v.stride(1), dh, out.stride(0), out.stride(1), dh,
                                          float(scale), _dt(q), _p(ws), ws_bytes, _stream()), "fino_attn_fwd_ws")
    if done is not None:
        done()
    return out


def _ranges_pairs(ranges, lq, lk):
    nta = (lk + 63) // 64
    pairs = 0.0
    for i, blk in enumerate(ranges.clamp(0, nta).tolist()):
        keys = sum(max(0, min(e * 64, lk) - s * 64) for s, e in blk)
        pairs += float(min(256, lq - 256 * i)) * keys
    return pairs


def attention_ranges_supported(b, heads, lq, lk, dh):
    return bool(_lib.lib().fino_attn_ranges_supported(int(b), int(heads), int(lq), int(lk), int(dh)))


def attention_ranges(q, k, v, heads, ranges, out=None, scale=None):
    b, lq, lk, hd, dh, out, scale = _attn_args(q, k, v, heads, out, scale)
    _check_ranges(ranges, lq)
    done = _timed_attn(b, lq, lk, hd, ranges, nbytes=True)
    _lib.check(_lib.lib().fino_attn_fwd_ranges(_p(q), _p(k), _p(v), _p(out), b, heads, lq, lk, dh,
                                              q.stride(0), q.stride(1), dh, k.stride(0), k.stride(1), dh,
                                              v.stride(0), v.stride(1), dh, out.stride(0), out.stride(1), dh,
                                              float(scale), _dt(q), _p(ranges), _stream()), "fino_attn_fwd_ranges")
    if done is not None:
        done()
    return out


def attention_tiles_supported(b, heads, lq, lk, dh):
    return bool(_lib.lib().fino_attn_tiles_supported(int(b), int(heads), int(lq), int(lk), int(dh)))


_MASK_DTYPES = tuple(d for d in (torch.int32, getattr(torch, "uint32", None)) if d is not None)


def _check_tile_mask(mask, b, heads, lq, lk):
    nqb, nta = (lq + 255) // 256, (lk + 63) // 64
    ok = (isinstance(mask, torch.Tensor) and mask.dtype in _MASK_DTYPES and mask.is_cuda and mask.dim() == 4
          and mask.is_contiguous() and mask.shape[0] in (1, b) and mask.shape[1] in (1, heads) and mask.shape[2] == nqb
          and mask.shape[3] * 32 >= nta)
    if not ok:
        got = f"{mask.dtype} {tuple(mask.shape)} on {mask.device}" if isinstance(mask, torch.Tensor) else type(mask)
        raise ValueError(f"mask: a contiguous int32 / uint32 device tensor [{b} | 1, {heads} | 1, {nqb}, >= {(nta + 31) // 32}] is "
                         f"needed, got {got}")
    words = mask.shape[3]
    return words, (mask.shape[1] * nqb * words if mask.shape[0] == b and b > 1 else 0), (nqb * words if mask.shape[1] == heads and heads > 1 else 0)


def _tile_mask_bits(mask, lk):
    from .window_attention import unpack_tile_mask
    return unpack_tile_mask(mask, lk)


def tile_mask_density(mask, lk):
    return float(_tile_mask_bits(mask, lk).float().mean())


def attention_tile_plan_bytes(b, heads, lq, lk, dh):
    return int(_lib.lib().fino_attn_tile_plan_bytes(int(b), int(heads), int(lq), int(lk), int(dh)))


_plan_ws = {}


def attention_tile_plan(q, k, heads, cdf, keep_ranges=None, scale=None, out=None, workspace=None):
    assert q.dim() == 3 and k.dim() == 3 and q.shape[0] == k.shape[0] and q.shape[2] == k.shape[2]
    for t in (q, k):
        assert t.stride(2) == 1 and t.is_cuda
    b, lq, hd = q.shape
    lk = k.shape[1]
    dh = hd // heads
    nqb, words = (lq + 255) // 256, ((lk + 63) // 64 + 31) // 32
    if keep_ranges is not None:
        _check_ranges(keep_ranges, lq)
    if out is None:
        out = torch.empty((b, heads, nqb, words), dtype=torch.int32, device=q.device)
    assert out.dtype in _MASK_DTYPES and out.is_cuda and out.is_contiguous() and \
        tuple(out.shape[:3]) == (b, heads, nqb) and out.dim() == 4 and out.shape[3] * 32 >= (lk + 63) // 64, \
        f"out: a contiguous int32 device tensor [{b}, {heads}, {nqb}, >= {words}] is needed, got {out.dtype} {tuple(out.shape)}"
    need = _lib.lib().fino_attn_tile_plan_bytes(b, heads, lq, lk, dh)
    if need <= 0:
        raise NotImplementedError(f"attention_tile_plan: B={b} H={heads} Lq={lq} Lk={lk} head_dim={dh} is not supported "
                                  f"(head_dim 64 | 128, at most 65536 keys)")
    if workspace is None:
        key = (q.device.index, torch.cuda.current_stream().cuda_stream)
        workspace = _plan_ws.get(key)
        if workspace is None or workspace.numel() * 4 < need:
            workspace = _plan_ws[key] = torch.empty(need // 4, dtype=torch.float32, device=q.device)
    assert workspace.dtype == torch.float32 and workspace.is_cuda and workspace.is_contiguous() and workspace.numel() * 4 >= need
    scale = dh ** -0.5 if scale is None else scale
    ev = _timed("attn_tile_plan")
    _lib.check(_lib.lib().fino_attn_tile_plan(_p(q), _p(k), b, heads, lq, lk, dh, q.stride(0), q.stride(1), dh,
                                             k.stride(0), k.stride(1), dh, float(scale), _dt(q), float(cdf),
                                             _p(keep_ranges), _p(out), out.shape[3], _p(workspace), workspace.numel() * 4,
                                             _stream()), "fino_attn_tile_plan")
    if ev is not None:
        ev.record()
    return out


def attention_tiles(q, k, v, heads, mask, out=None, scale=None):
    b, lq, lk, hd, dh, out, scale = _attn_args(q, k, v, heads, out, scale)
    words, mask_bs, mask_hs = _check_tile_mask(mask, b, heads, lq, lk)
    ev = _timed("attn_self")
    _lib.check(_lib.lib().fino_attn_fwd_tiles(_p(q), _p(k), _p(v), _p(out), b, heads, lq, lk, dh,
                                             q.stride(0), q.stride(1), dh, k.stride(0), k.stride(1), dh,
                                             v.stride(0), v.stride(1), dh, out.stride(0), out.stride(1), dh,
                                             float(scale), _dt(q), _p(mask), mask_bs, mask_hs, words, _stream()),
               "fino_attn_fwd_tiles")
    if ev is not None:
        ev.record()
        kt_ = KernelTimer.active
        bits = _tile_mask_bits(mask, lk).expand(b, heads, -1, -1).to(torch.float64)
        keys = torch.full((bits.shape[-1],), 64.0, dtype=torch.float64)
        keys[-1] = lk - 64 * (bits.shape[-1] - 1)
        rows = torch.tensor([min(256, lq - 256 * i) for i in range(bits.shape[2])], dtype=torch.float64)
        pairs = float(((bits * keys).sum(-1) * rows).sum())
        kt_.flops["attn_self"] = kt_.flops.get("attn_self", 0.0) + 4.0 * pairs * dh
        kt_.bytes["attn_self"] = kt_.bytes.get("attn_self", 0.0) + 2.0 * b * hd * (2 * lq + 2 * lk)
    return out


def attention_tail_supported(b, heads, lq, lk, dh):
    return bool(_lib.lib().fino_attn_tail_supported(int(b), int(heads), int(lq), int(lk), int(dh)))


def attention_tail(q, k, v, heads, lk_b, tail_mult, out=None, scale=None):
    import ctypes
    b, lq, lk, hd, dh, out, scale = _attn_args(q, k, v, heads, out, scale)
    assert len(lk_b) == b and len(tail_mult) == b
    lk_arr = (ctypes.c_int * b)(*[int(x) for x in lk_b])
    mult_arr = (ctypes.c_float * b)(*[float(x) for x in tail_mult])
    ev = _timed("attn_cross")
    _lib.check(_lib.lib().fino_attn_fwd_tail(_p(q), _p(k), _p(v), _p(out), b, heads, lq, lk, dh,
                                            q.stride(0), q.stride(1), dh, k.stride(0), k.stride(1), dh,
                                            v.stride(0), v.stride(1), dh, out.stride(0), out.stride(1), dh,
                                            float(scale), _dt(q), ctypes.cast(lk_arr, ctypes.c_void_p),
                                            ctypes.cast(mult_arr, ctypes.c_void_p), _stream()), "fino_attn_fwd_tail")
    if ev is not None:
        ev.record()
        kt_ = KernelTimer.active
        kt_.flops["attn_cross"] = kt_.flops.get("attn_cross", 0.0) + 4.0 * lq * hd * sum(int(x) for x in lk_b)
    return out


def attention_probs_supported(b, heads, lq, lk, dh):
    return bool(_lib.lib().fino_attn_probs_supported(int(b), int(heads), int(lq), int(lk), int(dh)))


def row_rrms(x, eps, out=None):
    x2, rows, dim, ldx = _rows2d(x)
    if out is None:
        out = torch.empty(rows, dtype=torch.float32, device=x.device)
    assert out.dtype == torch.float32 and out.is_contiguous() and out.numel() >= rows
    _lib.check(_lib.lib().fino_row_rrms(_p(x2), rows, dim, ldx, float(eps), _p(out), _dt(x), _stream()), "fino_row_rrms")
    return out


def attention_probs(q, k, heads, lk_b, tail_mult, kp, out=None, scale=None, q_rrms=None, q_weight=None):
    import ctypes
    assert q.dim() == 3 and k.dim() == 3
    b, lq, hd = q.shape
    lk = k.shape[1]
    dh = hd // heads
    for t in (q, k):
        assert t.stride(2) == 1 and t.is_cuda
    if out is None:
        out = torch.empty((b, lq, heads * kp), dtype=q.dtype, device=q.device)
    assert out.shape == (b, lq, heads * kp) and out.stride(2) == 1
    scale = dh ** -0.5 if scale is None else scale
    lk_arr = (ctypes.c_int * b)(*[int(x) for x in lk_b])
    mult_arr = (ctypes.c_float * b)(*[float(x) for x in tail_mult])
    ev = _timed("attn_cross")
    _lib.check(_lib.lib().fino_attn_probs(_p(q), _p(k), _p(out), b, heads, lq, lk, dh, q.stride(0), q.stride(1), dh,
                                         k.stride(0), k.stride(1), dh, int(kp), out.stride(0), out.stride(1), float(scale),
                                         _dt(q), ctypes.cast(lk_arr, ctypes.c_void_p), ctypes.cast(mult_arr, ctypes.c_void_p),
                                         _p(q_rrms), q_rrms.stride(0) if q_rrms is not None else 0, _p(q_weight), _stream()),
               "fino_attn_probs")
    if ev is not None:
        ev.record()
        kt_ = KernelTimer.active
        kt_.flops["attn_cross"] = kt_.flops.get("attn_cross", 0.0) + 2.0 * lq * hd * sum(int(x) for x in lk_b)
    return out


_attn_fp8_ws = {}


FP8_P_EXP2, FP8_P_RAMP = 0, 1
FP8_P_MODES = {"exp2": FP8_P_EXP2, "ramp": FP8_P_RAMP}
_p_env = os.environ.get("FINO_FP8_P_MODE", "ramp")
if _p_env not in FP8_P_MODES:
    raise ValueError(f"FINO_FP8_P_MODE={_p_env!r}: expected one of {' | '.join(FP8_P_MODES)} (how the opt-in fp8 attention turns a "
                     f"softmax weight into its e4m3 byte; 'ramp' -- a piecewise-linear exp2, the default since round 4 -- adds "
                     f"~0.3e-2 to the 5.5e-2 rel-RMS of the fp8 operands, 'exp2' is the exact form)")
FP8_P_DEFAULT = FP8_P_MODES[_p_env]


def _attn_fp8_workspace(need, device):
    key = (device.index, torch.cuda.current_stream().cuda_stream)
    ws = _attn_fp8_ws.get(key)
    if ws is None or ws.numel() < need:
        ws = _attn_fp8_ws[key] = torch.empty(need, dtype=torch.uint8, device=device)
    return ws


def _fp8_smooth_flags(smooth_k, smooth_v):
    return (1 if smooth_k else 0) | (2 if smooth_v else 0)


def attention_fp8(q, k, v, heads, out=None, scale=None, p_mode=None, smooth_k=False, smooth_v=False):
    p_mode = FP8_P_DEFAULT if p_mode is None else FP8_P_MODES.get(p_mode, p_mode)
    b, lq, lk, hd, dh, out, scale = _attn_args(q, k, v, heads, out, scale)
    flags = _fp8_smooth_flags(smooth_k, smooth_v)
    fwd = "fino_attn_fwd_fp8_smoothed" if smooth_v else ("fino_attn_fwd_fp8_smooth" if smooth_k else "fino_attn_fwd_fp8")
    need = _lib.lib().fino_attn_fp8_smoothed_kv_bytes(b, heads, lk, dh, flags)
    if need <= 0:
        raise RuntimeError(f"attention_fp8: head_dim {dh} is not supported (64 or 128)")
    ws = _attn_fp8_workspace(need, q.device)
    done = _timed_attn(b, lq, lk, hd)
    _lib.check(getattr(_lib.lib(), fwd)(_p(q), _p(k), _p(v), _p(out), b, heads, lq, lk, dh, q.stride(0), q.stride(1),
                                        k.stride(0), k.stride(1), v.stride(0), v.stride(1), out.stride(0), out.stride(1),
                                        float(scale), _dt(q), int(p_mode), _p(ws), need, _stream(),
                                        *((flags,) if smooth_v else ())), fwd)
    if done is not None:
        done()
    return out


def attention_fp8_ranges_supported(b, heads, lq, lk, dh):
    return bool(_lib.lib().fino_attn_fp8_ranges_supported(int(b), int(heads), int(lq), int(lk), int(dh)))


def attention_fp8_ranges(q, k, v, heads, ranges, out=None, scale=None, p_mode=None, smooth_k=False, smooth_v=False):
    p_mode = FP8_P_DEFAULT if p_mode is None else FP8_P_MODES.get(p_mode, p_mode)
    b, lq, lk, hd, dh, out, scale = _attn_args(q, k, v, heads, out, scale)
    _check_ranges(ranges, lq)
    if dh != 64:
        raise RuntimeError(f"attention_fp8_ranges: head_dim {dh} is not supported (64 only)")
    flags = _fp8_smooth_flags(smooth_k, smooth_v)
    need = _lib.lib().fino_attn_fp8_smoothed_kv_bytes(b, heads, lk, dh, flags)
    ws = _attn_fp8_workspace(need, q.device)
    done = _timed_attn(b, lq, lk, hd, ranges)
    _lib.check(_lib.lib().fino_attn_fwd_fp8_ranges(_p(q), _p(k), _p(v), _p(out), b, heads, lq, lk, dh, q.stride(0), q.stride(1),
                                                  k.stride(0), k.stride(1), v.stride(0), v.stride(1), out.stride(0),
                                                  out.stride(1), float(scale), _dt(q), int(p_mode), _p(ws), need,
                                                  flags, _p(ranges), _stream()), "fino_attn_fwd_fp8_ranges")
    if done is not None:
        done()
    return out


def attention_partial_floats(batch, heads, lq, head_dim):
    return _lib.lib().fino_attn_partial_bytes(batch, heads, lq, head_dim) // 4


def attention_partial(q, k, v, heads, out=None, scale=None):
    assert q.dim() == 3 and k.dim() == 3 and v.dim() == 3
    b, lq, hd = q.shape
    lk = k.shape[1]
    dh = hd // heads
    for t in (q, k, v):
        assert t.stride(2) == 1 and t.is_cuda
    need = _lib.lib().fino_attn_partial_bytes(b, heads, lq, dh)
    if out is None or out.numel() * 4 < need:
        out = torch.empty(need // 4, dtype=torch.float32, device=q.device)
    scale = dh ** -0.5 if scale is None else scale
    _lib.check(_lib.lib().fino_attn_partial(_p(q), _p(k), _p(v), b, heads, lq, lk, dh, q.stride(0), q.stride(1), dh,
                                           k.stride(0), k.stride(1), dh, v.stride(0), v.stride(1), dh, float(scale),
                                           _dt(q), _p(out), need, _stream()), "fino_attn_partial")
    return out


def attention_merge(parts, batch, lq, heads, head_dim, dtype, out=None):
    assert 1 <= len(parts) <= 3
    if out is None:
        out = torch.empty((batch, lq, heads * head_dim), dtype=dtype, device=parts[0].device)
    ps = list(parts) + [None] * (3 - len(parts))
    _lib.check(_lib.lib().fino_attn_merge(_p(out), batch, heads, lq, head_dim, out.stride(0), out.stride(1), head_dim,
                                         _p(ps[0]), _p(ps[1]), _p(ps[2]), _dt(out), _stream()), "fino_attn_merge")
    return out


def gemm_plan(m, n):
    import ctypes
    r, t = ctypes.c_int64(), ctypes.c_int()
    _lib.check(_lib.lib().fino_gemm_plan(m, n, ctypes.byref(r), ctypes.byref(t)), "fino_gemm_plan")
    return r.value, t.value


def gemm(a, w, bias=None, epilogue=EPI_NONE, residual=None, gate=None, sel=None, out=None, out2=None, split=0, tile_m=0,
         keep=None):
    a2, m, k, lda = _rows2d(a)
    assert w.dim() == 2 and w.stride(1) == 1 and w.shape[1] == k and w.dtype == a.dtype
    n = w.shape[0]
    if out is None:
        out = torch.empty((m, split or n), dtype=a.dtype, device=a.device)
    o2, _, _, ldc = _rows2d(out)
    if out2 is not None:
        if keep is not None:
            raise ValueError("gemm: keep= goes with a residual epilogue, out2= / split= with none: they do not combine")
        assert 0 < split < n and residual is None
        c2, _, _, ldc2 = _rows2d(out2)
        done = _timed_gemm(None, 2.0 * m * n * k)
        _lib.check(_lib.lib().fino_gemm_split_n(_p(a2), _p(w), _p(bias), _p(o2), m, n, k, lda, w.stride(0), ldc, epilogue,
                                               0, 0, 0, 0, 0, _dt(a), _p(c2), ldc2, split, tile_m, _stream()),
                   "fino_gemm_split_n")
        if done is not None:
            done()
        return out, out2
    r2, ldr, ms = _epi_operands(residual, gate)
    if bias is not None:
        assert bias.dtype == a.dtype and bias.is_contiguous()
    done = _timed_gemm(epilogue, 2.0 * m * n * k, 2.0 * (m * k + n * k + m * n * (2 if residual is not None else 1)))
    if keep is not None:
        k2, km, kn, ldk = _rows2d(keep)
        assert (km, kn) == (m, n) and keep.dtype == a.dtype and keep.is_cuda
        _lib.check(_lib.lib().fino_gemm_keep(_p(a2), _p(w), _p(bias), _p(o2), m, n, k, lda, w.stride(0), ldc, epilogue,
                                            _p(r2), ldr, _p(gate), ms, _p(sel), _dt(a), _p(k2), ldk, tile_m, _stream()),
                   "fino_gemm_keep")
    elif tile_m:
        _lib.check(_lib.lib().fino_gemm_split_n(_p(a2), _p(w), _p(bias), _p(o2), m, n, k, lda, w.stride(0), ldc, epilogue,
                                               _p(r2), ldr, _p(gate), ms, _p(sel), _dt(a), None, 0, 0, tile_m, _stream()),
                   "fino_gemm_split_n")
    else:
        _lib.check(_lib.lib().fino_gemm(_p(a2), _p(w), _p(bias), _p(o2), m, n, k, lda, w.stride(0), ldc, epilogue, _p(r2),
                                       ldr, _p(gate), ms, _p(sel), _dt(a), _stream()), "fino_gemm")
    if done is not None:
        done()
    return out


def gemm_blocked_a(a_blocks, rows, w, bias, residual, gate, sel, out, tile_m=0):
    if a_blocks.dim() == 3:
        a_blocks = a_blocks[None]
    assert a_blocks.dim() == 4 and a_blocks.stride(3) == 1 and w.dtype == a_blocks.dtype and w.stride(1) == 1
    groups, peers, _, bk = a_blocks.shape
    n, k = w.shape
    assert k == groups * peers * bk and residual.shape == (rows, n) and out.shape == (rows, n)
    r2, _, _, ldr = _rows2d(residual)
    o2, _, _, ldc = _rows2d(out)
    ms = gate.stride(0) if gate.dim() == 2 else 0
    done = _timed_gemm(None, 2.0 * rows * n * k)
    _lib.check(_lib.lib().fino_gemm_blocked_a(_p(a_blocks), _p(w), _p(bias), _p(o2), rows, n, k, bk, a_blocks.stride(1),
                                              groups, a_blocks.stride(0), a_blocks.stride(2), w.stride(0), ldc, _p(r2),
                                              ldr, _p(gate), ms, _p(sel), _dt(a_blocks), tile_m, _stream()),
               "fino_gemm_blocked_a")
    if done is not None:
        done()
    return out


def quantize_mxfp8(x, out=None):
    x2, rows, cols, ldx = _rows2d(x)
    nbytes = _lib.lib().fino_mxfp8_scale_bytes(rows, cols)
    if nbytes <= 0:
        raise ValueError(f"quantize_mxfp8: cols={cols} must be a positive multiple of 128")
    q, s = _mx_pair((rows, cols), nbytes, x.device, out)
    _lib.check(_lib.lib().fino_quantize_mxfp8(_p(x2), _p(q), _p(s), rows, cols, ldx, _dt(x), _stream()),
               "fino_quantize_mxfp8")
    return q, s


def ln_mxfp8(mode, x, weight=None, bias=None, shift=None, scale=None, sel=None, eps=1e-6, out=None):
    x2, rows, dim, ldx = _rows2d(x)
    nbytes = _lib.lib().fino_mxfp8_scale_bytes(rows, dim)
    if nbytes <= 0:
        raise ValueError(f"ln_mxfp8: dim={dim} must be a positive multiple of 128")
    q, s = _mx_pair((rows, dim), nbytes, x.device, out)
    for t in (weight, bias, shift, scale):
        assert t is None or t.dtype == torch.float32
    ms = shift.stride(0) if (shift is not None and shift.dim() == 2) else 0
    _lib.check(_lib.lib().fino_ln_mxfp8(mode, _p(x2), _p(q), _p(s), rows, dim, ldx, _p(weight), _p(bias), _p(shift),
                                       _p(scale), ms, _p(sel), eps, _dt(x), _stream()), "fino_ln_mxfp8")
    return q, s


def _mx_gemm(entry, aq, a_scales, wq, w_scales, bias, epilogue, residual, gate, sel, out, out_dtype, m, n, k, keep=None):
    if out is None:
        out = torch.empty((m, n), dtype=out_dtype, device=aq.device)
    o2, _, _, ldc = _rows2d(out)
    r2, ldr, ms = _epi_operands(residual, gate)
    done = _timed_gemm(None, 2.0 * m * n * k)
    if keep is not None:
        k2, km, kn, ldk = _rows2d(keep)
        assert (km, kn) == (m, n) and keep.dtype == out.dtype and keep.is_cuda
        entry += "_keep"
        _lib.check(getattr(_lib.lib(), entry)(_p(aq), _p(a_scales), _p(wq), _p(w_scales), _p(bias), _p(o2), m, n, k, ldc,
                                              epilogue, _p(r2), ldr, _p(gate), ms, _p(sel), _dt(out), _p(k2), ldk, _stream()),
                   entry)
    else:
        _lib.check(getattr(_lib.lib(), entry)(_p(aq), _p(a_scales), _p(wq), _p(w_scales), _p(bias), _p(o2), m, n, k, ldc,
                                              epilogue, _p(r2), ldr, _p(gate), ms, _p(sel), _dt(out), _stream()), entry)
    if done is not None:
        done()
    return out


def gemm_mxfp8(aq, a_scales, wq, w_scales, bias=None, epilogue=EPI_NONE, residual=None, gate=None, sel=None, out=None,
               out_dtype=torch.bfloat16, keep=None):
    m, k = aq.shape
    n = wq.shape[0]
    assert wq.shape[1] == k and aq.dtype == torch.uint8 and wq.dtype == torch.uint8 and aq.is_contiguous() \
        and wq.is_contiguous()
    return _mx_gemm("fino_gemm_mxfp8", aq, a_scales, wq, w_scales, bias, epilogue, residual, gate, sel, out, out_dtype, m, n, k,
                    keep)


def gemm_mxfp8_q(aq, a_scales, wq, w_scales, bias, epilogue=EPI_NONE, out=None):
    m, k = aq.shape
    n = wq.shape[0]
    assert bias is not None and wq.shape[1] == k
    q, s = _mx_pair((m, n), _lib.lib().fino_mxfp8_scale_bytes(m, n), aq.device, out)
    done = _timed_gemm(None, 2.0 * m * n * k)
    _lib.check(_lib.lib().fino_gemm_mxfp8_q(_p(aq), _p(a_scales), _p(wq), _p(w_scales), _p(bias), _p(q), _p(s), m, n, k,
                                           epilogue, _dt(bias), _stream()), "fino_gemm_mxfp8_q")
    if done is not None:
        done()
    return q, s


def quantize_mxfp6(x, out=None):
    x2, rows, cols, ldx = _rows2d(x)
    nbytes = _lib.lib().fino_mxfp6_scale_bytes(rows, cols)
    if nbytes <= 0:
        raise ValueError(f"quantize_mxfp6: cols={cols} must be a positive multiple of 128")
    q, s = _mx_pair(_lib.lib().fino_mxfp6_bytes(rows, cols), nbytes, x.device, out)
    _lib.check(_lib.lib().fino_quantize_mxfp6(_p(x2), _p(q), _p(s), rows, cols, ldx, _dt(x), _stream()),
               "fino_quantize_mxfp6")
    q.mx_shape = (rows, cols)
    return q, s


def gemm_mxfp6(aq, a_scales, wq, w_scales, bias=None, epilogue=EPI_NONE, residual=None, gate=None, sel=None, out=None,
               out_dtype=torch.bfloat16, m=None, n=None, k=None, keep=None):
    assert aq.dtype == torch.uint8 and wq.dtype == torch.uint8 and aq.is_contiguous() and wq.is_contiguous()
    sa_, sw_ = getattr(aq, "mx_shape", None), getattr(wq, "mx_shape", None)
    m = m if m is not None else (sa_[0] if sa_ else None)
    n = n if n is not None else (sw_[0] if sw_ else None)
    k = k if k is not None else (sa_[1] if sa_ else (sw_[1] if sw_ else None))
    if m is None or n is None or k is None:
        raise ValueError("gemm_mxfp6: operands without mx_shape need m / n / k")
    if sw_ and sw_[1] != k:
        raise ValueError(f"gemm_mxfp6: K of A ({k}) and of W ({sw_[1]}) differ")
    lib = _lib.lib()
    if aq.numel() != lib.fino_mxfp6_bytes(m, k) or wq.numel() != lib.fino_mxfp6_bytes(n, k):
        raise ValueError(f"gemm_mxfp6: operand sizes {aq.numel()} / {wq.numel()} do not match M={m} N={n} K={k}")
    return _mx_gemm("fino_gemm_mxfp6", aq, a_scales, wq, w_scales, bias, epilogue, residual, gate, sel, out, out_dtype, m, n, k,
                    keep)


def skinny_linear(x, w, b=None, silu_input=False):
    assert x.dtype == torch.float32 and x.dim() == 2 and x.is_contiguous() and w.is_contiguous()
    m, k = x.shape
    n = w.shape[0]
    wd = -1 if w.dtype == torch.float32 else _dt(w)
    if b is not None:
        assert b.dtype == w.dtype
    y = torch.empty((m, n), dtype=torch.float32, device=x.device)
    _lib.check(_lib.lib().fino_skinny_linear(_p(x), _p(w), _p(b), _p(y), m, n, k, wd, int(silu_input), _stream()),
               "fino_skinny_linear")
    return y


def patchify(x, patch, out=None):
    assert x.dim() == 4 and x.is_contiguous()
    c, f, h, w = x.shape
    pt, ph, pw = patch
    L = (f // pt) * (h // ph) * (w // pw)
    if out is None:
        out = torch.empty((L, c * pt * ph * pw), dtype=x.dtype, device=x.device)
    _lib.check(_lib.lib().fino_patchify(_p(x), _p(out), c, f, h, w, pt, ph, pw, out.stride(0), _dt(x), _stream()),
               "fino_patchify")
    return out


def unpatchify(y, cout, frames, height, width, patch, out=None):
    pt, ph, pw = patch
    if out is None:
        out = torch.empty((cout, frames, height, width), dtype=y.dtype, device=y.device)
    _lib.check(_lib.lib().fino_unpatchify(_p(y), _p(out), cout, frames, height, width, pt, ph, pw, y.stride(0), _dt(y),
                                         _stream()), "fino_unpatchify")
    return out


def wan_model_input(lat, cond, id_lat, traj, dtype, out=None):
    c, fg, h, w = lat.shape
    nid = 0 if id_lat is None else id_lat.shape[1]
    for t in (lat, cond, id_lat, traj):
        assert t is None or (t.dtype == torch.float32 and t.is_contiguous())
    assert traj.shape == (c, fg + nid, h, w) and cond.shape == (c, 1, h, w)
    if out is None:
        out = torch.empty((2 * c, fg + nid, h, w), dtype=dtype, device=lat.device)
    _lib.check(_lib.lib().fino_wan_model_input(_p(lat), _p(cond), _p(id_lat), _p(traj), _p(out), c, fg, nid, h, w,
                                              _dt(out), _stream()), "fino_wan_model_input")
    return out


def cfg_euler_step_(lat, cond_pred, uncond_pred, guidance, dt_dev, round_out=True):
    c, fg, h, w = lat.shape
    ft = cond_pred.shape[1]
    assert lat.dtype == torch.float32 and lat.is_contiguous() and cond_pred.is_contiguous()
    assert dt_dev.dtype == torch.float32 and dt_dev.is_cuda
    _lib.check(_lib.lib().fino_cfg_euler_step(_p(cond_pred), _p(uncond_pred), _p(lat), c, fg, ft, h, w, float(guidance),
                                             _p(dt_dev), int(round_out), _dt(cond_pred), _stream()),
               "fino_cfg_euler_step")
    return lat


def cfg_unipc_step_(x, last, m0, m1, cond_pred, uncond_pred, coef_dev):
    c, fg, h, w = x.shape
    ft = cond_pred.shape[1]
    for t in (x, last, m0, m1):
        assert t.dtype == torch.float32 and t.is_contiguous() and t.shape == x.shape
    assert coef_dev.dtype == torch.float32 and coef_dev.numel() >= 10 and cond_pred.is_contiguous()
    _lib.check(_lib.lib().fino_cfg_unipc_step(_p(cond_pred), _p(uncond_pred), _p(x), _p(last), _p(m0), _p(m1), c, fg,
                                             ft, h, w, _p(coef_dev), _dt(cond_pred), _stream()), "fino_cfg_unipc_step")
    return x


def cfg_vpred_step_(lat, pred, coef_dev, has_uncond=True):
    assert lat.is_contiguous() and pred.is_contiguous() and coef_dev.dtype == torch.float32 and lat.dtype == pred.dtype
    _lib.check(_lib.lib().fino_cfg_vpred_step(_p(pred), _p(lat), lat.numel(), pred[0].numel(), _p(coef_dev),
                                             int(has_uncond), _dt(lat), _stream()), "fino_cfg_vpred_step")
    return lat


def cfg_dpm_step_(lat, pred, x0_old, noise, coef_dev, has_uncond=True):
    assert lat.is_contiguous() and pred.is_contiguous() and noise.is_contiguous() and x0_old.is_contiguous()
    assert coef_dev.dtype == torch.float32 and coef_dev.numel() >= 9 and lat.dtype == pred.dtype == noise.dtype
    assert x0_old.dtype == torch.float32 and x0_old.numel() == lat.numel() == noise.numel()
    _lib.check(_lib.lib().fino_cfg_dpm_step(_p(pred), _p(lat), _p(x0_old), _p(noise), lat.numel(), pred[0].numel(),
                                           _p(coef_dev), int(has_uncond), _dt(lat), _stream()), "fino_cfg_dpm_step")
    return lat


_ZERO_PAGE = {}


def zero_page(device):
    z = _ZERO_PAGE.get(str(device))
    if z is None:
        z = _ZERO_PAGE[str(device)] = torch.zeros(256, dtype=torch.uint8, device=device)
    return z


def conv3d_cl(x, w2, bias, kernel, stride=(1, 1, 1), pad=(0, 0, 0), out_thw=None, upsample2x=False, residual=None,
              out=None):
    assert x.dim() == 4 and x.is_contiguous() and w2.is_contiguous()
    t, h, w, cin = x.shape
    kt, kh, kw = kernel
    cout = w2.shape[0]
    assert w2.shape[1] == kt * kh * kw * cin, (w2.shape, kernel, cin)
    if out_thw is None:
        up = 2 if upsample2x else 1
        out_thw = ((t + pad[0] - kt) // stride[0] + 1, (h * up + 2 * pad[1] - kh) // stride[1] + 1,
                   (w * up + 2 * pad[2] - kw) // stride[2] + 1)
    to, ho, wo = out_thw
    if out is None:
        out = torch.empty((to, ho, wo, cout), dtype=x.dtype, device=x.device)
    ev = _timed("conv3d")
    _lib.check(_lib.lib().fino_conv3d(_p(x), _p(w2), _p(bias), _p(out), t, h, w, cin, to, ho, wo, cout, kt, kh, kw,
                                     stride[0], stride[1], stride[2], pad[0], pad[1], pad[2], int(upsample2x),
                                     EPI_RESIDUAL if residual is not None else EPI_NONE, _p(residual),
                                     _p(zero_page(x.device)), _dt(x), _stream()), "fino_conv3d")
    if ev is not None:
        ev.record()
        kt_ = KernelTimer.active
        kt_.flops["conv3d"] = kt_.flops.get("conv3d", 0.0) + 2.0 * to * ho * wo * cout * w2.shape[1]
    return out


def rmsnorm_silu_cl(x, gamma, c_valid, silu=True, out=None):
    assert x.is_contiguous() and gamma.dtype == torch.float32
    cpad = x.shape[-1]
    rows = x.numel() // cpad
    out = torch.empty_like(x) if out is None else out
    _lib.check(_lib.lib().fino_rmsnorm_silu_cl(_p(x), _p(out), rows, c_valid, cpad, _p(gamma), int(silu), _dt(x),
                                              _stream()), "fino_rmsnorm_silu_cl")
    return out


def softmax_rows_(s, n, scale):
    assert s.dim() == 2 and s.stride(1) == 1
    _lib.check(_lib.lib().fino_softmax_rows(_p(s), s.shape[0], n, s.stride(0), float(scale), _dt3(s), _stream()),
               "fino_softmax_rows")
    return s


def dup_up3d_add(main, x, c_in, c_out, factor_t, factor_s):
    t, h, w, cin_pad = x.shape
    out = torch.empty_like(main)
    assert main.shape == (1 + (t - 1) * factor_t, h * factor_s, w * factor_s, main.shape[3])
    _lib.check(_lib.lib().fino_dup_up3d_add(_p(main), _p(x), _p(out), t, h, w, c_in, cin_pad, c_out, main.shape[3],
                                           factor_t, factor_s, _dt3(x), _stream()), "fino_dup_up3d_add")
    return out


def avg_down3d_add(main, x, c_in, c_out, factor_t, factor_s):
    t, h, w, cin_pad = x.shape
    out = torch.empty_like(main)
    _lib.check(_lib.lib().fino_avg_down3d_add(_p(main), _p(x), _p(out), t, h, w, c_in, cin_pad, c_out, main.shape[3],
                                             factor_t, factor_s, _dt3(x), _stream()), "fino_avg_down3d_add")
    return out


def vae_unpatchify_clamp(y, channels, patch):
    t, h, w, cpad = y.shape
    out = torch.empty((channels, t, h * patch, w * patch), dtype=torch.float32, device=y.device)
    _lib.check(_lib.lib().fino_vae_unpatchify_clamp(_p(y), _p(out), t, h, w, cpad, channels, patch, _dt3(y), _stream()),
               "fino_vae_unpatchify_clamp")
    return out


def vae_patchify(x, c_pad, patch, dtype):
    c, t, hp, wp = x.shape
    assert x.dtype == torch.float32 and x.is_contiguous()
    y = torch.empty((t, hp // patch, wp // patch, c_pad), dtype=dtype, device=x.device)
    _lib.check(_lib.lib().fino_vae_patchify(_p(x), _p(y), t, hp // patch, wp // patch, c_pad, c, patch, _dt3(y),
                                           _stream()), "fino_vae_patchify")
    return y


SPLIT_PRODUCTS = {2: ((0, 0), (0, 1), (1, 0)),
                  3: ((0, 0), (0, 1), (0, 2), (1, 0), (1, 1), (2, 0))}


def _pack_planes(planes):
    v = 0
    for i, q in enumerate(planes):
        v |= int(q) << (2 * i)
    return v


def split_bf16(x, layout, nplanes=3, out=None):
    assert x.dtype == torch.float32 and x.stride(-1) == 1
    x2 = x if x.dim() == 2 else x.reshape(-1, x.shape[-1])
    rows, cols = x2.shape
    prod = SPLIT_PRODUCTS[nplanes]
    planes = tuple(range(nplanes)) if layout == "planes" else tuple(p[0 if layout == "A" else 1] for p in prod)
    nseg = len(planes)
    if out is None:
        out = torch.empty(tuple(x.shape[:-1]) + (nseg * cols,), dtype=torch.bfloat16, device=x.device)
    assert out.is_contiguous() and out.numel() == rows * nseg * cols
    _lib.check(_lib.lib().fino_split_bf16(_p(x2), _p(out), rows, cols, x2.stride(0), nseg * cols, nseg, _pack_planes(planes),
                                         _stream()), "fino_split_bf16")
    return out


def rmsnorm_silu_cl_f32(x, gamma, c_valid, silu=True, split=None, nplanes=3):
    assert x.is_contiguous() and x.dtype == torch.float32 and gamma.dtype == torch.float32
    cpad = x.shape[-1]
    rows = x.numel() // cpad
    if split is None:
        planes, out = (), torch.empty_like(x)
    else:
        prod = SPLIT_PRODUCTS[nplanes]
        planes = tuple(range(nplanes)) if split == "planes" else tuple(p[0 if split == "A" else 1] for p in prod)
        out = torch.empty(tuple(x.shape[:-1]) + (len(planes) * cpad,), dtype=torch.bfloat16, device=x.device)
    _lib.check(_lib.lib().fino_rmsnorm_silu_cl_f32(_p(x), _p(out), rows, c_valid, cpad, _p(gamma), int(silu), len(planes),
                                                  _pack_planes(planes), _stream()), "fino_rmsnorm_silu_cl_f32")
    return out


def conv3d_split_cl(xp, w6, bias, kernel, nplanes, stride=(1, 1, 1), pad=(0, 0, 0), out_thw=None, upsample2x=False,
                    residual=None):
    assert xp.dim() == 4 and xp.is_contiguous() and w6.is_contiguous() and xp.dtype == torch.bfloat16 and w6.dtype == torch.bfloat16
    t, h, w, cw = xp.shape
    cin = cw // nplanes
    kt, kh, kw = kernel
    cout = w6.shape[0]
    nprod = len(SPLIT_PRODUCTS[nplanes])
    assert cin * nplanes == cw and w6.shape[1] == kt * kh * kw * nprod * cin, (xp.shape, w6.shape, kernel)
    assert bias is None or bias.dtype == torch.float32
    if out_thw is None:
        up = 2 if upsample2x else 1
        out_thw = ((t + pad[0] - kt) // stride[0] + 1, (h * up + 2 * pad[1] - kh) // stride[1] + 1,
                   (w * up + 2 * pad[2] - kw) // stride[2] + 1)
    to, ho, wo = out_thw
    out = torch.empty((to, ho, wo, cout), dtype=torch.float32, device=xp.device)
    if residual is not None:
        assert residual.dtype == torch.float32 and residual.is_contiguous() and residual.shape == out.shape
    ev = _timed("conv3d")
    _lib.check(_lib.lib().fino_conv3d_split(_p(xp), _p(w6), _p(bias), _p(out), t, h, w, cin, nplanes, to, ho, wo, cout, kt, kh, kw,
                                           stride[0], stride[1], stride[2], pad[0], pad[1], pad[2], int(upsample2x),
                                           EPI_RESIDUAL if residual is not None else EPI_NONE, _p(residual),
                                           _p(zero_page(xp.device)), _stream()), "fino_conv3d_split")
    if ev is not None:
        ev.record()
        kt_ = KernelTimer.active
        kt_.flops["conv3d"] = kt_.flops.get("conv3d", 0.0) + 2.0 * to * ho * wo * cout * w6.shape[1]
    return out


def gemm_f32(a_split, w_split, bias=None, residual=None, out=None):
    a2, m, k, lda = _rows2d(a_split)
    assert w_split.dim() == 2 and w_split.stride(1) == 1 and w_split.shape[1] == k and a_split.dtype == w_split.dtype == torch.bfloat16
    n = w_split.shape[0]
    if out is None:
        out = torch.empty((m, n), dtype=torch.float32, device=a_split.device)
    assert out.dtype == torch.float32 and out.stride(-1) == 1
    o2 = out if out.dim() == 2 else out.view(-1, out.shape[-1])
    r2, ldr = None, 0
    if residual is not None:
        assert residual.dtype == torch.float32 and residual.stride(-1) == 1
        r2 = residual if residual.dim() == 2 else residual.view(-1, residual.shape[-1])
        ldr = r2.stride(0)
    assert bias is None or (bias.dtype == torch.float32 and bias.is_contiguous())
    _lib.check(_lib.lib().fino_gemm(_p(a2), _p(w_split), _p(bias), _p(o2), m, n, k, lda, w_split.stride(0), o2.stride(0),
                                   EPI_F32_RESIDUAL if residual is not None else EPI_F32, _p(r2), ldr, None, 0, None, BF16,
                                   _stream()), "fino_gemm")
    return out


def vae_blend_tiles_(a, b, extent, axis):
    assert a.dim() == 4 and b.dim() == 4 and a.is_contiguous() and b.is_contiguous() and a.dtype == b.dtype
    assert a.shape[0] == b.shape[0] and a.shape[3] == b.shape[3]
    _lib.check(_lib.lib().fino_vae_blend_tiles(_p(a), _p(b), a.shape[0], a.shape[1], a.shape[2], b.shape[1], b.shape[2],
                                              a.shape[3], int(extent), int(axis), _dt(a), _stream()), "fino_vae_blend_tiles")
    return b


_GN_WS = {}


def groupnorm_cl(x, c_valid, groups, gamma, beta, eps=1e-6, mod=None, silu=False, out=None):
    assert x.dim() == 4 and x.is_contiguous() and gamma.dtype == torch.float32 and beta.dtype == torch.float32
    t, h, w, cp = x.shape
    out = torch.empty_like(x) if out is None else out
    need = _lib.lib().fino_groupnorm_workspace_bytes(cp)
    key = (x.device.index, torch.cuda.current_stream().cuda_stream, cp)
    ws = _GN_WS.get(key)
    if ws is None:
        ws = _GN_WS[key] = torch.empty(need // 4, dtype=torch.float32, device=x.device)
    ms = mh = None
    tz = hz = wz = 0
    if mod is not None:
        ms, mh = mod
        assert ms.shape == mh.shape and ms.shape[3] == cp and ms.is_contiguous() and mh.is_contiguous() \
            and ms.dtype == x.dtype
        tz, hz, wz = ms.shape[:3]
    _lib.check(_lib.lib().fino_groupnorm_cl(_p(x), _p(out), t, h, w, c_valid, cp, groups, _p(gamma), _p(beta), eps,
                                           _p(ms), _p(mh), tz, hz, wz, int(silu), _p(ws), need, _dt(x), _stream()),
               "fino_groupnorm_cl")
    return out


def avg_pool_time2(x):
    t, h, w, cp = x.shape
    assert x.is_contiguous() and t > 1
    out = torch.empty(((t & 1) + (t - (t & 1)) // 2, h, w, cp), dtype=x.dtype, device=x.device)
    _lib.check(_lib.lib().fino_avg_pool_time2(_p(x), _p(out), t, h, w, cp, _dt(x), _stream()), "fino_avg_pool_time2")
    return out


LORA_MAX_ADAPTERS = 8


def lora_merge_(w_base, adapters, out=None):
    out = w_base if out is None else out
    if not (w_base.is_cuda and out.is_cuda):
        raise RuntimeError("frameino_amd ops need CUDA(HIP) tensors; there is no CPU path")
    if w_base.dim() != 2 or out.shape != w_base.shape or out.dtype != w_base.dtype:
        raise ValueError(f"lora_merge_: weight {tuple(w_base.shape)} {w_base.dtype} / out {tuple(out.shape)} {out.dtype}")
    if w_base.stride(1) != 1 or out.stride(1) != 1:
        raise ValueError("lora_merge_: the weight's last dimension must be contiguous")
    if len(adapters) > LORA_MAX_ADAPTERS:
        raise ValueError(f"lora_merge_: {len(adapters)} adapters in one call (at most {LORA_MAX_ADAPTERS})")
    n, k = w_base.shape
    na = len(adapters)
    ptr_a, ptr_b = (_lib.c_void_p * max(na, 1))(), (_lib.c_void_p * max(na, 1))()
    lda, ldb = (_lib.c_i64 * max(na, 1))(), (_lib.c_i64 * max(na, 1))()
    rank, scale = (_lib.c_int * max(na, 1))(), (_lib.c_float * max(na, 1))()
    for i, (a, b, s) in enumerate(adapters):
        r = a.shape[0]
        if a.dim() != 2 or b.dim() != 2 or a.shape[1] != k or b.shape != (n, r):
            raise ValueError(f"lora_merge_: adapter {i}: A {tuple(a.shape)} / B {tuple(b.shape)} for a weight {tuple(w_base.shape)}")
        if a.dtype != w_base.dtype or b.dtype != w_base.dtype or not (a.is_cuda and b.is_cuda):
            raise ValueError(f"lora_merge_: adapter {i}: factors must be {w_base.dtype} device tensors")
        if a.stride(1) != 1 or b.stride(1) != 1:
            raise ValueError(f"lora_merge_: adapter {i}: factors need a contiguous last dimension")
        ptr_a[i], ptr_b[i] = a.data_ptr(), b.data_ptr()
        lda[i], ldb[i], rank[i], scale[i] = a.stride(0), b.stride(0), r, float(s)
    _lib.check(_lib.lib().fino_lora_merge(_p(w_base), w_base.stride(0), _p(out), out.stride(0), n, k, na, ptr_a, lda, ptr_b,
                                          ldb, rank, scale, _dt3(w_base), _stream()), "fino_lora_merge")
    return out


STEP_CACHE_MAX_SEGMENTS = 4
_STEP_CACHE_WS = {}


def _rows_of(t, dtype, what):
    if not t.is_cuda:
        raise RuntimeError("frameino_amd ops need CUDA(HIP) tensors; there is no CPU path")
    if t.dim() != 2 or t.stride(1) != 1 or t.dtype != dtype:
        raise ValueError(f"{what}: need a row-strided [rows, D] {dtype} tensor, got {tuple(t.shape)} {t.dtype} strides {t.stride()}")
    return t


def step_cache_probe(h0, h1, p, r, h1_copy=None):
    one = not isinstance(h0, (list, tuple))
    h0, h1, p, r = ([t] for t in (h0, h1, p, r)) if one else (h0, h1, p, r)
    n = len(h0)
    h1_copy = ([h1_copy] if one else h1_copy) if h1_copy is not None else [None] * n
    if not (1 <= n <= STEP_CACHE_MAX_SEGMENTS) or not (len(h1) == len(p) == len(r) == len(h1_copy) == n):
        raise ValueError(f"step_cache_probe: {n} segments (1 .. {STEP_CACHE_MAX_SEGMENTS}), one entry per operand each")
    dt, d, dev = h0[0].dtype, h0[0].shape[-1], h0[0].device
    segs = (_lib.StepCacheSegment * n)()
    for s in range(n):
        rows = h0[s].shape[0]
        for t, what in ((h0[s], "h0"), (h1[s], "h1"), (p[s], "p"), (r[s], "r"), (h1_copy[s], "h1_copy")):
            if t is not None and (_rows_of(t, dt, f"step_cache_probe {what}").shape != (rows, d) or t.device != dev):
                raise ValueError(f"step_cache_probe: segment {s}: {what} is {tuple(t.shape)} on {t.device}, want {(rows, d)} on {dev}")
        g = segs[s]
        g.h0, g.h1, g.p, g.r, g.h1_copy = _p(h0[s]), _p(h1[s]), _p(p[s]), _p(r[s]), _p(h1_copy[s])
        g.rows, g.ld_h0, g.ld_h1, g.ld_r = rows, h0[s].stride(0), h1[s].stride(0), r[s].stride(0)
        g.ld_p = p[s].stride(0) if p[s] is not None else 0
        g.ld_h1_copy = h1_copy[s].stride(0) if h1_copy[s] is not None else 0
    key = (str(dev), _stream())
    if key not in _STEP_CACHE_WS:
        _STEP_CACHE_WS[key] = (torch.zeros((STEP_CACHE_MAX_SEGMENTS, 2), dtype=torch.float32, device=dev),
                               torch.empty(2 * STEP_CACHE_MAX_SEGMENTS * 1024, dtype=torch.float32, device=dev))
    sums, ws = _STEP_CACHE_WS[key]
    _lib.check(_lib.lib().fino_step_cache_probe(segs, n, d, _p(sums), _p(ws), _dt3(h0[0]), _stream()), "fino_step_cache_probe")
    return sums[:n]


def step_cache_residual(a, b, out=None, subtract=True):
    _rows_of(a, a.dtype, "step_cache_residual a")
    _rows_of(b, a.dtype, "step_cache_residual b")
    out = torch.empty_like(a) if out is None else _rows_of(out, a.dtype, "step_cache_residual out")
    if a.shape != b.shape or out.shape != a.shape:
        raise ValueError(f"step_cache_residual: shapes {tuple(a.shape)} / {tuple(b.shape)} / {tuple(out.shape)}")
    rows, d = a.shape
    _lib.check(_lib.lib().fino_step_cache_residual(_p(a), a.stride(0), _p(b), b.stride(0), _p(out), out.stride(0), rows, d,
                                                   int(bool(subtract)), _dt3(a), _stream()), "fino_step_cache_residual")
    return out


def pab_broadcast(x, y, gate=None, sel=None, out=None):
    _rows_of(x, x.dtype, "pab_broadcast x")
    _rows_of(y, x.dtype, "pab_broadcast y")
    out = torch.empty_like(x) if out is None else _rows_of(out, x.dtype, "pab_broadcast out")
    if x.shape != y.shape or out.shape != x.shape:
        raise ValueError(f"pab_broadcast: shapes {tuple(x.shape)} / {tuple(y.shape)} / {tuple(out.shape)}")
    if gate is not None:
        assert gate.dtype == torch.float32 and gate.stride(-1) == 1 and gate.shape[-1] == x.shape[1]
    rows, d = x.shape
    ms = gate.stride(0) if (gate is not None and gate.dim() == 2) else 0
    _lib.check(_lib.lib().fino_pab_broadcast(_p(x), x.stride(0), _p(y), y.stride(0), _p(out), out.stride(0), rows, d, _p(gate),
                                             ms, _p(sel), _dt(x), _stream()), "fino_pab_broadcast")
    return out
```

### include/frameino_hip.h

```cpp
#ifndef FRAMEINO_HIP_H
#define FRAMEINO_HIP_H
#include <stdint.h>

#ifdef __cplusplus
extern "C" {
#endif

#define FINO_VERSION 103

enum { FINO_BF16 = 0, FINO_F16 = 1, FINO_F32 = 2 };
enum {
    FINO_OK = 0,
    FINO_ERR_ARG = -1,
    FINO_ERR_LAUNCH = -2,
    FINO_ERR_UNSUPPORTED = -3
};

int fino_version(void);
const char* fino_last_error(void);

enum { FINO_TUNE_GEMM_GROUP_M = 0, FINO_TUNE_GEMM_RASTER = 1, FINO_TUNE_CONV_LOOP = 2, FINO_TUNE_GEMM_TILE_M = 3,
       FINO_TUNE_ATTN_KERNEL = 4, FINO_TUNE_ATTN_FP8_KERNEL = 5, FINO_TUNE_ATTN_WALK_GRID = 6, FINO_TUNE_COUNT = 8 };
int fino_tune_set(int key, int value);
int fino_tune_get(int key);

int fino_adaln_modulate(const void* x, void* y, int64_t rows, int dim, int64_t ldx, int64_t ldy,
                        const float* shift, const float* scale, int64_t mod_stride, const int32_t* sel,
                        float eps, int dtype, void* stream);

int fino_layernorm(const void* x, void* y, int64_t rows, int dim, int64_t ldx, int64_t ldy, const float* w,
                   const float* b, float eps, int dtype, void* stream);

int fino_gated_residual(const void* x, const void* y, void* out, int64_t rows, int dim, int64_t ldx, int64_t ldy,
                        int64_t ldo, const float* gate, int64_t mod_stride, const int32_t* sel, int dtype,
                        void* stream);

int fino_gated_residual_staged(const void* x, const void* y, void* out, int64_t rows, int dim, int64_t ldx, int64_t ldy,
                               int64_t ldo, const float* gate, int64_t mod_stride, const int32_t* sel, int dtype,
                               void* stream);

int fino_layernorm_zero(const void* x, void* y, int64_t rows, int dim, int64_t ldx, int64_t ldy, const float* w,
                        const float* b, const float* shift, const float* scale, int64_t mod_stride, const int32_t* sel,
                        float eps, int dtype, void* stream);

int fino_ln_mxfp8(int mode, const void* x, void* q, void* scales, int64_t rows, int dim, int64_t ldx, const float* w,
                  const float* b, const float* shift, const float* scale, int64_t mod_stride, const int32_t* sel,
                  float eps, int dtype, void* stream);

int fino_rmsnorm_rope(void* x, int64_t rows, int dim, int64_t ldx, const void* weight, float eps,
                      const float* cos_t, const float* sin_t, int head_dim, int dtype, void* stream);
int fino_rmsnorm_rope_scaled(void* x, int64_t rows, int dim, int64_t ldx, const void* weight, float eps,
                             const float* cos_t, const float* sin_t, int head_dim, float out_scale, int dtype,
                             void* stream);

int fino_rmsnorm_rope_scatter(const void* x, int64_t rows, int dim, int64_t ldx, const void* weight, float eps,
                              const float* cos_t, const float* sin_t, int head_dim, float out_scale, void* out,
                              const int64_t* head_off, const int64_t* head_ld, int dtype, void* stream);

int fino_qkv_rmsnorm_rope(void* qkv, int64_t rows, int dim, int64_t ldx, const void* q_weight, float q_eps,
                          const void* k_weight, float k_eps, const float* cos_t, const float* sin_t, int head_dim,
                          float q_out_scale, void* out, const int64_t* head_off, const int64_t* head_ld, int dtype,
                          void* stream);

int fino_headnorm_rope(void* x, int batch, int64_t rows, int heads, int head_dim, int64_t ldx, int64_t batch_stride,
                       const void* w, const void* b, float eps, const float* cos_t, const float* sin_t,
                       int64_t rope_row0, int dtype, void* stream);
int fino_headnorm_rope_scaled(void* x, int batch, int64_t rows, int heads, int head_dim, int64_t ldx,
                              int64_t batch_stride, const void* w, const void* b, float eps, const float* cos_t,
                              const float* sin_t, int64_t rope_row0, float out_scale, int dtype, void* stream);

#define FINO_ATTN_SCALE_FOLDED (-1.0f)
int fino_attn_fwd(const void* q, const void* k, const void* v, void* o, int batch, int heads, int64_t lq,
                  int64_t lk, int head_dim, int64_t q_bs, int64_t q_rs, int64_t q_hs, int64_t k_bs, int64_t k_rs,
                  int64_t k_hs, int64_t v_bs, int64_t v_rs, int64_t v_hs, int64_t o_bs, int64_t o_rs,
                  int64_t o_hs, float scale, int dtype, void* stream);
enum { FINO_FP8_P_EXP2 = 0, FINO_FP8_P_RAMP = 1 };
int64_t fino_attn_fp8_kv_bytes(int batch, int heads, int64_t lk, int head_dim);
int fino_attn_fwd_fp8(const void* q, const void* k, const void* v, void* o, int batch, int heads, int64_t lq, int64_t lk,
                      int head_dim, int64_t q_bs, int64_t q_rs, int64_t k_bs, int64_t k_rs, int64_t v_bs, int64_t v_rs,
                      int64_t o_bs, int64_t o_rs, float scale, int dtype, int p_mode, void* kv_workspace,
                      int64_t kv_workspace_bytes, void* stream);
int64_t fino_attn_fp8_smooth_kv_bytes(int batch, int heads, int64_t lk, int head_dim);
int fino_attn_fwd_fp8_smooth(const void* q, const void* k, const void* v, void* o, int batch, int heads, int64_t lq, int64_t lk,
                             int head_dim, int64_t q_bs, int64_t q_rs, int64_t k_bs, int64_t k_rs, int64_t v_bs, int64_t v_rs,
                             int64_t o_bs, int64_t o_rs, float scale, int dtype, int p_mode, void* kv_workspace,
                             int64_t kv_workspace_bytes, void* stream);
#define FINO_FP8_SMOOTH_K 1
#define FINO_FP8_SMOOTH_V 2
int64_t fino_attn_fp8_smoothed_kv_bytes(int batch, int heads, int64_t lk, int head_dim, int smooth);
int fino_attn_fwd_fp8_smoothed(const void* q, const void* k, const void* v, void* o, int batch, int heads, int64_t lq, int64_t lk,
                               int head_dim, int64_t q_bs, int64_t q_rs, int64_t k_bs, int64_t k_rs, int64_t v_bs, int64_t v_rs,
                               int64_t o_bs, int64_t o_rs, float scale, int dtype, int p_mode, void* kv_workspace,
                               int64_t kv_workspace_bytes, void* stream, int smooth);

int fino_attn_tail_supported(int batch, int heads, int64_t lq, int64_t lk, int head_dim);
int fino_attn_fwd_tail(const void* q, const void* k, const void* v, void* o, int batch, int heads, int64_t lq, int64_t lk,
                       int head_dim, int64_t q_bs, int64_t q_rs, int64_t q_hs, int64_t k_bs, int64_t k_rs, int64_t k_hs,
                       int64_t v_bs, int64_t v_rs, int64_t v_hs, int64_t o_bs, int64_t o_rs, int64_t o_hs, float scale,
                       int dtype, const int* lk_b, const float* tail_mult, void* stream);

int fino_attn_ranges_supported(int batch, int heads, int64_t lq, int64_t lk, int head_dim);
int fino_attn_fwd_ranges(const void* q, const void* k, const void* v, void* o, int batch, int heads, int64_t lq, int64_t lk,
                         int head_dim, int64_t q_bs, int64_t q_rs, int64_t q_hs, int64_t k_bs, int64_t k_rs, int64_t k_hs,
                         int64_t v_bs, int64_t v_rs, int64_t v_hs, int64_t o_bs, int64_t o_rs, int64_t o_hs, float scale,
                         int dtype, const int* ranges, void* stream);
int fino_attn_tiles_supported(int batch, int heads, int64_t lq, int64_t lk, int head_dim);
int fino_attn_fwd_tiles(const void* q, const void* k, const void* v, void* o, int batch, int heads, int64_t lq, int64_t lk,
                        int head_dim, int64_t q_bs, int64_t q_rs, int64_t q_hs, int64_t k_bs, int64_t k_rs, int64_t k_hs,
                        int64_t v_bs, int64_t v_rs, int64_t v_hs, int64_t o_bs, int64_t o_rs, int64_t o_hs, float scale,
                        int dtype, const uint32_t* mask, int64_t mask_bs, int64_t mask_hs, int words, void* stream);
int64_t fino_attn_tile_plan_bytes(int batch, int heads, int64_t lq, int64_t lk, int head_dim);
int fino_attn_tile_plan(const void* q, const void* k, int batch, int heads, int64_t lq, int64_t lk, int head_dim, int64_t q_bs,
                        int64_t q_rs, int64_t q_hs, int64_t k_bs, int64_t k_rs, int64_t k_hs, float scale, int dtype, float cdf,
                        const int* keep_ranges, uint32_t* mask, int words, void* workspace, int64_t workspace_bytes,
                        void* stream);
int fino_attn_fp8_ranges_supported(int batch, int heads, int64_t lq, int64_t lk, int head_dim);
int fino_attn_fwd_fp8_ranges(const void* q, const void* k, const void* v, void* o, int batch, int heads, int64_t lq, int64_t lk,
                             int head_dim, int64_t q_bs, int64_t q_rs, int64_t k_bs, int64_t k_rs, int64_t v_bs, int64_t v_rs,
                             int64_t o_bs, int64_t o_rs, float scale, int dtype, int p_mode, void* kv_workspace,
                             int64_t kv_workspace_bytes, int smooth_k, const int* ranges, void* stream);

int fino_attn_probs_supported(int batch, int heads, int64_t lq, int64_t lk, int head_dim);
int fino_attn_probs(const void* q, const void* k, void* p, int batch, int heads, int64_t lq, int64_t lk, int head_dim,
                    int64_t q_bs, int64_t q_rs, int64_t q_hs, int64_t k_bs, int64_t k_rs, int64_t k_hs, int kp, int64_t p_bs,
                    int64_t p_rs, float scale, int dtype, const int* lk_b, const float* tail_mult, const float* q_rrms,
                    int64_t q_rrms_bs, const void* q_weight, void* stream);
int fino_row_rrms(const void* x, int64_t rows, int dim, int64_t ldx, float eps, float* rrms, int dtype, void* stream);

int64_t fino_attn_partial_bytes(int batch, int heads, int64_t lq, int head_dim);
int fino_attn_partial(const void* q, const void* k, const void* v, int batch, int heads, int64_t lq, int64_t lk,
                      int head_dim, int64_t q_bs, int64_t q_rs, int64_t q_hs, int64_t k_bs, int64_t k_rs, int64_t k_hs,
                      int64_t v_bs, int64_t v_rs, int64_t v_hs, float scale, int dtype, void* partial,
                      int64_t partial_bytes, void* stream);
int fino_attn_merge(void* o, int batch, int heads, int64_t lq, int head_dim, int64_t o_bs, int64_t o_rs, int64_t o_hs,
                    const void* part0, const void* part1, const void* part2, int dtype, void* stream);


int64_t fino_attn_workspace_bytes(int batch, int heads, int64_t lq, int64_t lk, int head_dim);
int fino_attn_fwd_ws(const void* q, const void* k, const void* v, void* o, int batch, int heads, int64_t lq,
                     int64_t lk, int head_dim, int64_t q_bs, int64_t q_rs, int64_t q_hs, int64_t k_bs, int64_t k_rs,
                     int64_t k_hs, int64_t v_bs, int64_t v_rs, int64_t v_hs, int64_t o_bs, int64_t o_rs, int64_t o_hs,
                     float scale, int dtype, void* workspace, int64_t workspace_bytes, void* stream);

enum { FINO_EPI_NONE = 0, FINO_EPI_GELU_TANH = 1, FINO_EPI_RESIDUAL = 2, FINO_EPI_GATED_RESIDUAL = 3,
       FINO_EPI_GATED_RESIDUAL_STAGED = 4, FINO_EPI_F32 = 5, FINO_EPI_F32_RESIDUAL = 6 };
int fino_gemm(const void* a, const void* w, const void* bias, void* c, int64_t m, int64_t n, int64_t k,
              int64_t lda, int64_t ldw, int64_t ldc, int epilogue, const void* r, int64_t ldr, const float* gate,
              int64_t mod_stride, const int32_t* sel, int dtype, void* stream);
int fino_gemm_split_n(const void* a, const void* w, const void* bias, void* c, int64_t m, int64_t n, int64_t k, int64_t lda,
                      int64_t ldw, int64_t ldc, int epilogue, const void* r, int64_t ldr, const float* gate,
                      int64_t mod_stride, const int32_t* sel, int dtype, void* c2, int64_t ldc2, int64_t n_split,
                      int tile_m, void* stream);
int fino_gemm_keep(const void* a, const void* w, const void* bias, void* c, int64_t m, int64_t n, int64_t k, int64_t lda,
                   int64_t ldw, int64_t ldc, int epilogue, const void* r, int64_t ldr, const float* gate,
                   int64_t mod_stride, const int32_t* sel, int dtype, void* keep, int64_t ldk, int tile_m, void* stream);
int fino_gemm_blocked_a(const void* a, const void* w, const void* bias, void* c, int64_t m, int64_t n, int64_t k,
                        int64_t a_block_k, int64_t a_block_stride, int a_groups, int64_t a_group_stride, int64_t lda,
                        int64_t ldw, int64_t ldc, const void* r, int64_t ldr, const float* gate, int64_t mod_stride,
                        const int32_t* sel, int dtype, int tile_m, void* stream);

int fino_gemm_plan(int64_t m, int64_t n, int64_t* rows_256, int* tile_rows_rest);
int fino_skinny_linear(const float* x, const void* w, const void* b, float* y, int m, int64_t n, int64_t k,
                       int w_dtype, int silu_input, void* stream);

int fino_patchify(const void* x, void* a, int channels, int frames, int height, int width, int pt, int ph, int pw,
                  int64_t lda, int dtype, void* stream);
int fino_unpatchify(const void* y, void* out, int cout, int frames, int height, int width, int pt, int ph, int pw,
                    int64_t ldy, int dtype, void* stream);

int fino_wan_model_input(const float* lat, const float* cond, const float* id_lat, const float* traj, void* out,
                         int channels, int gen_frames, int id_frames, int height, int width, int dtype, void* stream);
int fino_cfg_euler_step(const void* cond_pred, const void* uncond_pred, float* lat, int channels, int gen_frames,
                        int total_frames, int height, int width, float guidance, const float* dt_dev, int round_out,
                        int dtype, void* stream);

int fino_cfg_unipc_step(const void* cond_pred, const void* uncond_pred, float* x, float* last, float* m0, float* m1,
                        int channels, int gen_frames, int total_frames, int height, int width, const float* coef_dev,
                        int dtype, void* stream);

int fino_cfg_vpred_step(const void* pred, void* lat, int64_t n_lat, int64_t batch_stride, const float* coef_dev,
                        int has_uncond, int dtype, void* stream);

int fino_cfg_dpm_step(const void* pred, void* lat, float* x0_old, const void* noise, int64_t n_lat, int64_t batch_stride,
                      const float* coef_dev, int has_uncond, int dtype, void* stream);

int fino_conv3d(const void* x, const void* w, const void* bias, void* y, int t_in, int h_in, int w_in, int c_in_pad,
                int t_out, int h_out, int w_out, int c_out_pad, int kt, int kh, int kw, int st, int sh, int sw, int pt,
                int ph, int pw, int upsample2x, int epilogue, const void* r, const void* zero_page, int dtype,
                void* stream);
int fino_rmsnorm_silu_cl(const void* x, void* y, int64_t rows, int c_valid, int c_pad, const float* gamma, int silu,
                         int dtype, void* stream);
int fino_softmax_rows(void* s, int64_t rows, int n, int64_t ld, float scale, int dtype, void* stream);
int fino_dup_up3d_add(const void* main_in, const void* x, void* out, int t_in, int h_in, int w_in, int c_in,
                      int c_in_pad, int c_out, int c_out_pad, int factor_t, int factor_s, int dtype, void* stream);
int fino_avg_down3d_add(const void* main_in, const void* x, void* out, int t_in, int h_in, int w_in, int c_in,
                        int c_in_pad, int c_out, int c_out_pad, int factor_t, int factor_s, int dtype, void* stream);
int fino_vae_unpatchify_clamp(const void* y, float* out, int t, int h, int w, int c_pad, int channels, int patch,
                              int dtype, void* stream);
int fino_vae_patchify(const float* x, void* y, int t, int h, int w, int c_pad, int channels, int patch, int dtype,
                      void* stream);
int fino_split_bf16(const float* x, void* out, int64_t rows, int cols, int64_t ldx, int64_t ldo, int nseg,
                    unsigned planes_packed, void* stream);
int fino_rmsnorm_silu_cl_f32(const float* x, void* y, int64_t rows, int c_valid, int c_pad, const float* gamma, int silu,
                             int nseg, unsigned planes_packed, void* stream);
int fino_conv3d_split(const void* x_planes, const void* w_products, const float* bias, float* y, int t_in, int h_in, int w_in,
                      int c_in_pad, int planes, int t_out, int h_out, int w_out, int c_out_pad, int kt, int kh, int kw, int st,
                      int sh, int sw, int pt, int ph, int pw, int upsample2x, int epilogue, const float* r,
                      const void* zero_page, void* stream);

int64_t fino_mxfp8_scale_bytes(int64_t rows, int64_t cols);
int fino_quantize_mxfp8(const void* x, void* q, void* scales, int64_t rows, int64_t cols, int64_t ldx, int dtype,
                        void* stream);
int fino_gemm_mxfp8(const void* aq, const void* a_scales, const void* wq, const void* w_scales, const void* bias,
                    void* c, int64_t m, int64_t n, int64_t k, int64_t ldc, int epilogue, const void* r, int64_t ldr,
                    const float* gate, int64_t mod_stride, const int32_t* sel, int out_dtype, void* stream);
int fino_gemm_mxfp8_keep(const void* aq, const void* a_scales, const void* wq, const void* w_scales, const void* bias,
                         void* c, int64_t m, int64_t n, int64_t k, int64_t ldc, int epilogue, const void* r, int64_t ldr,
                         const float* gate, int64_t mod_stride, const int32_t* sel, int out_dtype, void* keep, int64_t ldk,
                         void* stream);
int fino_gemm_mxfp8_q(const void* aq, const void* a_scales, const void* wq, const void* w_scales, const void* bias,
                      void* cq, void* c_scales, int64_t m, int64_t n, int64_t k, int epilogue, int bias_dtype,
                      void* stream);

int64_t fino_mxfp6_bytes(int64_t rows, int64_t cols);
int64_t fino_mxfp6_scale_bytes(int64_t rows, int64_t cols);
int fino_quantize_mxfp6(const void* x, void* q, void* scales, int64_t rows, int64_t cols, int64_t ldx, int dtype,
                        void* stream);
int fino_gemm_mxfp6(const void* aq, const void* a_scales, const void* wq, const void* w_scales, const void* bias,
                    void* c, int64_t m, int64_t n, int64_t k, int64_t ldc, int epilogue, const void* r, int64_t ldr,
                    const float* gate, int64_t mod_stride, const int32_t* sel, int out_dtype, void* stream);
int fino_gemm_mxfp6_keep(const void* aq, const void* a_scales, const void* wq, const void* w_scales, const void* bias,
                         void* c, int64_t m, int64_t n, int64_t k, int64_t ldc, int epilogue, const void* r, int64_t ldr,
                         const float* gate, int64_t mod_stride, const int32_t* sel, int out_dtype, void* keep, int64_t ldk,
                         void* stream);

int fino_traj_paint(const int32_t* points, const int32_t* frame_offsets, float* canvas, int frames, int height, int width,
                    int radius, void* stream);
int fino_traj_blur_quantize(const float* canvas, float* scratch, float* out, const float* taps_dev, int taps, int planes,
                            int height, int width, void* stream);


int64_t fino_groupnorm_workspace_bytes(int c_pad);
int fino_groupnorm_cl(const void* x, void* y, int t, int h, int w, int channels, int c_pad, int groups,
                      const float* gamma, const float* beta, float eps, const void* mod_scale, const void* mod_shift,
                      int tz, int hz, int wz, int silu, void* workspace, int64_t workspace_bytes, int dtype,
                      void* stream);
int fino_avg_pool_time2(const void* x, void* y, int t_in, int h, int w, int c_pad, int dtype, void* stream);
int fino_vae_blend_tiles(const void* a, void* b, int t, int h_a, int w_a, int h_b, int w_b, int c_pad, int extent, int axis,
                         int dtype, void* stream);

int fino_resize_area_pad_u8(const void* src, void* dst, int src_h, int src_w, int region_h, int region_w, int out_h,
                            int out_w, int off_y, int off_x, int fill, void* stream);
int fino_u8_hwc_to_chw_unit(const void* src, float* dst, int height, int width, void* stream);

enum { FINO_LORA_MAX_ADAPTERS = 8, FINO_LORA_MAX_TOTAL_RANK = 1024 };
int fino_lora_merge(const void* w_base, int64_t ldw_base, void* w_out, int64_t ldw_out, int64_t n, int64_t k,
                    int n_adapters, const void* const* a, const int64_t* lda, const void* const* b, const int64_t* ldb,
                    const int* rank, const float* scale, int dtype, void* stream);

typedef struct {
    const void* h0;
    const void* h1;
    const void* p;
    void* r;
    void* h1_copy;
    int64_t rows, ld_h0, ld_h1, ld_p, ld_r, ld_h1_copy;
} FinoStepCacheSegment;
enum { FINO_STEP_CACHE_MAX_SEGMENTS = 4, FINO_STEP_CACHE_BLOCKS = 1024,
       FINO_STEP_CACHE_WORKSPACE_FLOATS = 2 * FINO_STEP_CACHE_MAX_SEGMENTS * FINO_STEP_CACHE_BLOCKS };
int fino_step_cache_probe(const FinoStepCacheSegment* segs, int nseg, int64_t dim, float* sums, float* workspace, int dtype,
                          void* stream);
int fino_step_cache_residual(const void* a, int64_t lda, const void* b, int64_t ldb, void* out, int64_t ldo, int64_t rows,
                             int64_t dim, int subtract, int dtype, void* stream);
int fino_pab_broadcast(const void* x, int64_t ldx, const void* y, int64_t ldy, void* out, int64_t ldo, int64_t rows,
                       int64_t dim, const float* gate, int64_t mod_stride, const int32_t* sel, int dtype, void* stream);

int fino_diag_mfma_peak(int kind, int waves_per_simd, int iters, void* scratch, double* flops, void* stream);

#ifdef __cplusplus
}
#endif
#endif
```

Measured before the change: 3.772 denoise-steps/s.

## Add three-stage LDS ring for short GEMM tiles and single mixed-tile launch

Gives the ping-pong GEMM mainloop a three-stage LDS ring for tile heights up to 160 rows. Loads run two k-steps ahead and use partial vmcnt waits, so short tiles that cannot hide load latency with two stages get more overlap. It also adds a fused kernel that runs the 256-row tiles and the ragged remainder tiles in one launch, and teaches the tile planner a cheaper cost floor for ring-3 tiles. The costs are more LDS per block, which can lower occupancy, more template instantiations, and planner heuristics that may choose worse splits.

```diff
diff --git a/frameino_amd/_lib.py b/frameino_amd/_lib.py
--- a/frameino_amd/_lib.py
+++ b/frameino_amd/_lib.py
@@ -102,6 +102,7 @@
     "fino_gemm_blocked_a": [c_void_p, c_void_p, c_void_p, c_void_p, c_i64, c_i64, c_i64, c_i64, c_i64, c_int, c_i64, c_i64, c_i64,
                             c_i64, c_void_p, c_i64, c_void_p, c_i64, c_void_p, c_int, c_int, c_void_p],
     "fino_gemm_plan": [c_i64, c_i64, ctypes.POINTER(c_i64), ctypes.POINTER(c_int)],
+    "fino_gemm_plan_launches": [c_i64, c_i64, c_int, ctypes.POINTER(c_i64), ctypes.POINTER(c_int), ctypes.POINTER(c_int)],
     "fino_skinny_linear": [c_void_p, c_void_p, c_void_p, c_void_p, c_int, c_i64, c_i64, c_int, c_int, c_void_p],
     "fino_patchify": [c_void_p, c_void_p] + [c_int] * 7 + [c_i64, c_int, c_void_p],
     "fino_unpatchify": [c_void_p, c_void_p] + [c_int] * 7 + [c_i64, c_int, c_void_p],
diff --git a/frameino_amd/csrc/fino_gemm.hip b/frameino_amd/csrc/fino_gemm.hip
--- a/frameino_amd/csrc/fino_gemm.hip
+++ b/frameino_amd/csrc/fino_gemm.hip
@@ -260,14 +260,16 @@
     return (b - j * p.a_groups) * (int)(p.a_grp_elems * 2) + j * (int)(p.a_blk_elems * 2) + (kt - b * p.a_tpb) * (BK * 2);
 }
 
-template <typename T, bool CONV, int MI, bool ABLK = false>
+template <typename T, bool CONV, int MI, bool ABLK = false, int RING = 2>
 __device__ __forceinline__ void pp_mainloop(const GemmParams& p, char* smem, const int64_t m0, const int64_t n0,
                                             const int kb, const int nk, f32x4_t (&acc)[MI][4], const int tid,
                                             const int lane, const int wave, const int wm, const int wn) {
     typedef typename T::vec8 vec8;
     static_assert(MI >= 2 && MI <= 8, "tile height 64 .. 256");
     static_assert(!CONV || MI == 8, "the implicit-GEMM gather is built for 256-row tiles");
+    static_assert(RING == 2 || (RING == 3 && MI <= 5 && !CONV), "three stages fit tiles of <= 160 rows");
     enum : int { NA0 = (MI + 1) / 2, NA1 = MI - (MI + 1) / 2 };
+    enum : int { kABytes = RING == 3 ? 32 * MI * 128 : kTileBytes, kStBytes = kABytes + kTileBytes };
 
     const int r8 = lane >> 3;
     const int sk = ((lane & 7) ^ ((4 * (wn & 1) + (lane >> 4)) & 7)) * 8;
@@ -357,18 +359,18 @@
 #define PP_DMA_A(STAGE_, KT_, QI_)                                                                                \
     if ((QI_) < NA1 || wm == 0)                                                                                   \
         __builtin_amdgcn_raw_ptr_buffer_load_lds(                                                                 \
-            a_rsrc, (FINO_LDS void*)(smem + (STAGE_) * kStageBytes + ((aq0 + (QI_)) * 32 + wn * 8) * 128), 16,    \
+            a_rsrc, (FINO_LDS void*)(smem + (STAGE_) * kStBytes + ((aq0 + (QI_)) * 32 + wn * 8) * 128), 16,       \
             a_off[QI_], CONV ? a_koff : (ABLK ? ablk_koff(p, kb + (KT_)) : (kb + (KT_)) * (BK * 2)), 0, GP_DMA_AUX);
 #define PP_DMA_W(STAGE_, KT_, Q_)                                                                                 \
     if (!CONV || (Q_) < w_pieces)                                                                                 \
         __builtin_amdgcn_raw_ptr_buffer_load_lds(                                                                 \
-            w_rsrc, (FINO_LDS void*)(smem + (STAGE_) * kStageBytes + kTileBytes + ((Q_) * 32 + wn * 8) * 128), 16, \
+            w_rsrc, (FINO_LDS void*)(smem + (STAGE_) * kStBytes + kABytes + ((Q_) * 32 + wn * 8) * 128), 16,       \
             w_off[CONV ? 0 : (Q_)], (kb + (KT_)) * (BK * 2) + (CONV ? (Q_) * w_piece_bytes : 0), 0, GP_DMA_AUX);
 
     const int frow = lane & 15;
     const int pch0 = (lane >> 4) ^ (frow >> 1);
     const int a_base = (wm * (16 * MI) + frow) * 128;
-    const int w_base = kTileBytes + (wn * 64 + frow) * 128;
+    const int w_base = kABytes + (wn * 64 + frow) * 128;
 
 #pragma unroll
     for (int i = 0; i < MI; ++i)
@@ -400,19 +402,41 @@
 #else
 #define PSTAMP(V_)
 #endif
+    const uint32_t lds0 = (uint32_t)(uintptr_t)(FINO_LDS char*)smem;
+    int cur = 0;
     for (int t = 0; t < nk; ++t) {
-        const int cur = t & 1;
-        const char* sb = smem + cur * kStageBytes;
+        const char* sb = smem + cur * kStBytes;
         PSTAMP(t0)
 #pragma unroll
         for (int kk = 0; kk < 2; ++kk) {
             const int pch = (pch0 ^ (kk << 2)) << 4;
-#pragma unroll
-            for (int j = 0; j < 4; ++j) wf[kk][j] = *reinterpret_cast<const u32x4_t*>(sb + w_base + j * 2048 + pch);
-#pragma unroll
-            for (int i = 0; i < MI; ++i) af[kk][i] = *reinterpret_cast<const u32x4_t*>(sb + a_base + i * 2048 + pch);
-        }
-        if (t >= 1 && t + 1 < nk) {
+            if constexpr (RING == 3) {
+                const uint32_t wa = lds0 + cur * kStBytes + w_base + pch, aa = lds0 + cur * kStBytes + a_base + pch;
+#pragma unroll
+                for (int j = 0; j < 4; ++j)
+                    asm volatile("ds_read_b128 %0, %1 offset:%2" : "=v"(wf[kk][j]) : "v"(wa), "n"(j * 2048));
+#pragma unroll
+                for (int i = 0; i < MI; ++i)
+                    asm volatile("ds_read_b128 %0, %1 offset:%2" : "=v"(af[kk][i]) : "v"(aa), "n"(i * 2048));
+            } else {
+#pragma unroll
+                for (int j = 0; j < 4; ++j) wf[kk][j] = *reinterpret_cast<const u32x4_t*>(sb + w_base + j * 2048 + pch);
+#pragma unroll
+                for (int i = 0; i < MI; ++i) af[kk][i] = *reinterpret_cast<const u32x4_t*>(sb + a_base + i * 2048 + pch);
+            }
+        }
+        const bool ahead = RING == 3 && t + 2 < nk;
+        if constexpr (RING == 3) {
+            if (ahead) {
+                const int nxt = cur == 0 ? 2 : cur - 1;
+#pragma unroll
+                for (int q = 0; q < NA0; ++q) PP_DMA_A(nxt, t + 2, q)
+                if (wm == 0) {
+#pragma unroll
+                    for (int q = 0; q < 8; ++q) { PP_DMA_W(nxt, t + 2, q) }
+                }
+            }
+        } else if (t >= 1 && t + 1 < nk) {
 #pragma unroll
             for (int q = 0; q < NA0; ++q) PP_DMA_A(cur ^ 1, t + 1, q)
             if (wm == 0) {
@@ -471,7 +495,14 @@
 #endif
         }
         __builtin_amdgcn_sched_barrier(0);
-        asm volatile("s_waitcnt vmcnt(0)" ::: "memory");
+        if (ahead) {
+            if (wm == 0) asm volatile("s_waitcnt vmcnt(%0)" :: "n"(NA0 + 8) : "memory");
+            else asm volatile("s_waitcnt vmcnt(%0)" :: "n"(NA1) : "memory");
+        } else {
+            asm volatile("s_waitcnt vmcnt(0)" ::: "memory");
+        }
+        if constexpr (RING == 3) cur = cur == 2 ? 0 : cur + 1;
+        else cur ^= 1;
         PSTAMP(t3)
         __builtin_amdgcn_s_barrier();
         __builtin_amdgcn_sched_barrier(0);
@@ -493,7 +524,7 @@
 #undef PP_DMA_W
 }
 
-template <typename T, int EPI, bool CONV = false, int MI = 8, bool ABLK = false, bool KEEP = false>
+template <typename T, int EPI, bool CONV = false, int MI = 8, bool ABLK = false, bool KEEP = false, int RING = 2>
 __global__ __launch_bounds__(kThreads, 2) void gemm_pp_kernel(const GemmParams p) {
     extern __shared__ __attribute__((aligned(16))) char smem[];
     const int tid = threadIdx.x;
@@ -508,11 +539,15 @@
 #ifndef GP_RAGGED
 #define GP_RAGGED 1
 #endif
+#ifndef GP_RAGGED_RING
+#define GP_RAGGED_RING 3
+#endif
+    static_assert(3 * (64 * 128 + kTileBytes) <= kSmemBytes, "three 64-row stages inside the 256-row launch's LDS");
     if constexpr (GP_RAGGED && MI == 8 && !CONV && EPI != FINO_EPI_F32 && EPI != FINO_EPI_F32_RESIDUAL) {
         const int64_t rows = p.m - m0;
         if (rows <= 64) {
             f32x4_t acc2[2][4];
-            pp_mainloop<T, false, 2, ABLK>(p, smem, m0, n0, 0, nk, acc2, tid, lane, wave, wm, wn);
+            pp_mainloop<T, false, 2, ABLK, GP_RAGGED_RING>(p, smem, m0, n0, 0, nk, acc2, tid, lane, wave, wm, wn);
             gemm_epilogue<T, EPI, false, 2, KEEP>(acc2, p, smem, m0, n0, tid, lane, wm, wn);
             return;
         }
@@ -528,12 +563,77 @@
     unsigned long long ts0, ts1;
     STAMP(ts0)
 #endif
-    pp_mainloop<T, CONV, MI, ABLK>(p, smem, m0, n0, 0, nk, acc, tid, lane, wave, wm, wn);
+    pp_mainloop<T, CONV, MI, ABLK, RING>(p, smem, m0, n0, 0, nk, acc, tid, lane, wave, wm, wn);
 #ifdef FINO_GEMM_STAMP
     STAMP(ts1)
     if (blockIdx.x == 17 && lane == 0) fino_gemm_dbg[wave * 8 + 5] = ts1 - ts0;
 #endif
     gemm_epilogue<T, EPI, false, MI, KEEP>(acc, p, smem, m0, n0, tid, lane, wm, wn);
+}
+
+template <typename T, int EPI, int MI, int RING, bool KEEP>
+__device__ __forceinline__ void gemm_pp_tile(const GemmParams& p, char* smem, int64_t m0, int64_t n0, int tid, int lane,
+                                             int wave, int wm, int wn) {
+    f32x4_t acc[MI][4];
+    pp_mainloop<T, false, MI, false, RING>(p, smem, m0, n0, 0, (int)(p.k / BK), acc, tid, lane, wave, wm, wn);
+    gemm_epilogue<T, EPI, false, MI, KEEP>(acc, p, smem, m0, n0, tid, lane, wm, wn);
+}
+template <typename T, int EPI, bool KEEP = false>
+__global__ __launch_bounds__(kThreads, 2) void gemm_mix_kernel(const GemmParams p, const int tall_m, const int mi2) {
+    extern __shared__ __attribute__((aligned(16))) char smem[];
+    const int tid = threadIdx.x;
+    const int lane = tid & 63;
+    const int wave = __builtin_amdgcn_readfirstlane(tid >> 6);
+    const int wm = wave >> 2, wn = wave & 3;
+    const int n_tall = tall_m * p.tiles_n;
+    int tm, tn;
+    if ((int)blockIdx.x < n_tall) {
+        tile_raster_rows(p, tall_m, xcd_remap((int)blockIdx.x, n_tall), tm, tn);
+        gemm_pp_tile<T, EPI, 8, 2, KEEP>(p, smem, (int64_t)tm * BM, (int64_t)tn * BN, tid, lane, wave, wm, wn);
+        return;
+    }
+    const int64_t rows1 = (int64_t)tall_m * BM;
+    const int low_m = (int)((p.m - rows1 + 32 * mi2 - 1) / (32 * mi2));
+    tile_raster_rows(p, low_m, xcd_remap((int)blockIdx.x - n_tall, low_m * p.tiles_n), tm, tn);
+    const int64_t m0 = rows1 + (int64_t)tm * (32 * mi2), n0 = (int64_t)tn * BN;
+    switch (mi2) {
+        case 2: gemm_pp_tile<T, EPI, 2, 3, KEEP>(p, smem, m0, n0, tid, lane, wave, wm, wn); break;
+        case 3: gemm_pp_tile<T, EPI, 3, 3, KEEP>(p, smem, m0, n0, tid, lane, wave, wm, wn); break;
+        case 4: gemm_pp_tile<T, EPI, 4, 3, KEEP>(p, smem, m0, n0, tid, lane, wave, wm, wn); break;
+        default: gemm_pp_tile<T, EPI, 5, 3, KEEP>(p, smem, m0, n0, tid, lane, wave, wm, wn); break;
+    }
+}
+
+template <typename T, int EPI, bool KEEP = false>
+int launch_gemm_mix(const GemmParams& p, int64_t rows1, int mi2, hipStream_t st) {
+    constexpr int max_bytes = 3 * (32 * 5 * 128 + kTileBytes);
+    static_assert(max_bytes <= 160 * 1024 && max_bytes >= kSmemBytes, "LDS of a CU");
+    static FinoPerDeviceOnce once;
+    if (int rc = fino_max_smem_once(once, reinterpret_cast<const void*>(&gemm_mix_kernel<T, EPI, KEEP>), max_bytes, "fino_gemm")) return rc;
+    const int ring_bytes = 3 * (32 * mi2 * 128 + kTileBytes);
+    const int smem_bytes = ring_bytes > kSmemBytes ? ring_bytes : kSmemBytes;
+    const int tall_m = (int)(rows1 / BM);
+    const int64_t low_m = (p.m - rows1 + 32 * mi2 - 1) / (32 * mi2);
+    gemm_mix_kernel<T, EPI, KEEP><<<dim3((unsigned)((tall_m + low_m) * p.tiles_n)), kThreads, smem_bytes, st>>>(p, tall_m, mi2);
+    FINO_LAUNCH_CHECK();
+    return FINO_OK;
+}
+template <typename T, bool KEEP = false>
+int launch_gemm_mix_e(const GemmParams& p, int64_t rows1, int mi2, int epi, hipStream_t st) {
+    if constexpr (KEEP) {
+        switch (epi) {
+            case FINO_EPI_RESIDUAL: return launch_gemm_mix<T, FINO_EPI_RESIDUAL, true>(p, rows1, mi2, st);
+            case FINO_EPI_GATED_RESIDUAL_STAGED: return launch_gemm_mix<T, FINO_EPI_GATED_RESIDUAL_STAGED, true>(p, rows1, mi2, st);
+            default: return launch_gemm_mix<T, FINO_EPI_GATED_RESIDUAL, true>(p, rows1, mi2, st);
+        }
+    }
+    switch (epi) {
+        case FINO_EPI_NONE: return launch_gemm_mix<T, FINO_EPI_NONE>(p, rows1, mi2, st);
+        case FINO_EPI_GELU_TANH: return launch_gemm_mix<T, FINO_EPI_GELU_TANH>(p, rows1, mi2, st);
+        case FINO_EPI_RESIDUAL: return launch_gemm_mix<T, FINO_EPI_RESIDUAL>(p, rows1, mi2, st);
+        case FINO_EPI_GATED_RESIDUAL_STAGED: return launch_gemm_mix<T, FINO_EPI_GATED_RESIDUAL_STAGED>(p, rows1, mi2, st);
+        default: return launch_gemm_mix<T, FINO_EPI_GATED_RESIDUAL>(p, rows1, mi2, st);
+    }
 }
 
 template <typename T, int EPI, bool GENERIC, bool CONV = false, bool KEEP = false>
@@ -545,13 +645,22 @@
     return FINO_OK;
 }
 
-template <typename T, int EPI, bool CONV = false, int MI = 8, bool ABLK = false, bool KEEP = false>
+template <typename T, int EPI, bool CONV = false, int MI = 8, bool ABLK = false, bool KEEP = false, int RING = 2>
 int launch_gemm_pp(const GemmParams& p, hipStream_t st) {
+    constexpr int smem_bytes = RING == 3 ? 3 * (32 * MI * 128 + kTileBytes) : kSmemBytes;
+    static_assert(smem_bytes <= 160 * 1024 && smem_bytes >= 32 * MI * kCsStride, "LDS of a CU; the epilogue's rows");
     static FinoPerDeviceOnce once;
-    if (int rc = fino_max_smem_once(once, reinterpret_cast<const void*>(&gemm_pp_kernel<T, EPI, CONV, MI, ABLK, KEEP>), kSmemBytes, "fino_gemm")) return rc;
-    gemm_pp_kernel<T, EPI, CONV, MI, ABLK, KEEP><<<dim3((unsigned)(p.tiles_m * p.tiles_n)), kThreads, kSmemBytes, st>>>(p);
+    if (int rc = fino_max_smem_once(once, reinterpret_cast<const void*>(&gemm_pp_kernel<T, EPI, CONV, MI, ABLK, KEEP, RING>), smem_bytes, "fino_gemm")) return rc;
+    gemm_pp_kernel<T, EPI, CONV, MI, ABLK, KEEP, RING><<<dim3((unsigned)(p.tiles_m * p.tiles_n)), kThreads, smem_bytes, st>>>(p);
     FINO_LAUNCH_CHECK();
     return FINO_OK;
+}
+
+template <typename T, int EPI, int MI, bool ABLK = false, bool KEEP = false>
+int launch_gemm_pp_ring(const GemmParams& p, hipStream_t st) {
+    if constexpr (MI <= 5)
+        if (!(fino_tune_get(FINO_TUNE_GEMM_RING) & 1)) return launch_gemm_pp<T, EPI, false, MI, ABLK, KEEP, 3>(p, st);
+    return launch_gemm_pp<T, EPI, false, MI, ABLK, KEEP>(p, st);
 }
 
 inline int gemm_device_cus() {
@@ -566,12 +675,14 @@
     return c;
 }
 
-struct TilePlan { int64_t rows1; int mi2; };
-inline double plan_launch_cost(int64_t rows, int mi, int tiles_n, int cus) {
+struct TilePlan { int64_t rows1; int mi2; bool one; };
+inline double plan_launch_cost(int64_t rows, int mi, int tiles_n, int cus, bool ring3) {
     if (rows <= 0) return 0.0;
     const double bm = 32.0 * mi;
     const int64_t tiles = ((rows + 32 * mi - 1) / (32 * mi)) * tiles_n;
-    const double mfma_raw = 0.85 * bm / 256.0, mfma = mfma_raw > 0.80 ? mfma_raw : 0.80, deliver = (bm + 256.0) / 512.0;
+    static const double floor3[6] = {0, 0, 0.38, 0.43, 0.48, 0.55};
+    const double floor = ring3 && mi <= 5 ? floor3[mi] : 0.80;
+    const double mfma_raw = 0.85 * bm / 256.0, mfma = mfma_raw > floor ? mfma_raw : floor, deliver = (bm + 256.0) / 512.0;
     const int64_t full = tiles / cus, rem = tiles % cus;
     double c = (double)full * (mfma > deliver ? mfma : deliver);
     if (rem) {
@@ -580,43 +691,59 @@
     }
     return c + 0.07;
 }
-inline TilePlan plan_tiles_search(int64_t m, int tiles_n, int cus);
-inline TilePlan plan_tiles(int64_t m, int tiles_n, int cus, int tile_m = 0) {
+inline TilePlan plan_tiles_search(int64_t m, int tiles_n, int cus, bool ring3, bool may_mix);
+inline TilePlan plan_tiles(int64_t m, int tiles_n, int cus, int tile_m = 0, bool may_mix = true) {
     const int forced = tile_m ? tile_m : fino_tune_get(FINO_TUNE_GEMM_TILE_M);
-    if (forced >= 2 && forced <= 7) return TilePlan{0, forced};
-    if (forced == 8 || m <= 0) return TilePlan{m, 8};
+    if (forced >= 2 && forced <= 7) return TilePlan{0, forced, false};
+    if (forced == 8 || m <= 0) return TilePlan{m, 8, false};
+    const int knob = fino_tune_get(FINO_TUNE_GEMM_RING);
+    const bool ring3 = !(knob & 1);
+    may_mix = may_mix && ring3 && !(knob & 2);
+    if (const int fmi = (knob >> 4) & 15; fmi >= 2 && fmi <= 7) {
+        const int64_t rows1 = (int64_t)(knob >> 8) * 256 < m ? (int64_t)(knob >> 8) * 256 : m;
+        return TilePlan{rows1, rows1 == m ? 8 : fmi, may_mix && fmi <= 5 && rows1 > 0 && rows1 < m};
+    }
     static std::atomic<uint64_t> memo[64];
-    const bool memoable = m < (1ll << 24) && tiles_n > 0 && tiles_n < 512 && cus > 0 && cus < 512;
+    const bool memoable = knob == 0 && may_mix && m < (1ll << 24) && tiles_n > 0 && tiles_n < 512 && cus > 0 && cus < 512;
     const uint64_t key = ((uint64_t)m << 18) | ((uint64_t)tiles_n << 9) | (uint64_t)cus;
     std::atomic<uint64_t>& slot = memo[(key * 0x9E3779B97F4A7C15ull) >> 58];
     if (memoable) {
         const uint64_t e = slot.load(std::memory_order_relaxed);
         if ((e & 1) && (e >> 22) == key) {
             const uint64_t r = (e >> 6) & 0xffff;
-            return TilePlan{r == 0xffff ? m : (int64_t)r * 256, (int)((e >> 3) & 7) + 1};
-        }
-    }
-    const TilePlan tp = plan_tiles_search(m, tiles_n, cus);
+            return TilePlan{r == 0xffff ? m : (int64_t)r * 256, (int)((e >> 3) & 7) + 1, ((e >> 2) & 1) != 0};
+        }
+    }
+    const TilePlan tp = plan_tiles_search(m, tiles_n, cus, ring3, may_mix);
     if (memoable && (tp.rows1 == m || (tp.rows1 % 256 == 0 && tp.rows1 / 256 < 0xffff)) && tp.mi2 >= 2 && tp.mi2 <= 8)
         slot.store((key << 22) | ((tp.rows1 == m ? 0xffffull : (uint64_t)(tp.rows1 / 256)) << 6) |
-                       ((uint64_t)(tp.mi2 - 1) << 3) | 1ull, std::memory_order_relaxed);
+                       ((uint64_t)(tp.mi2 - 1) << 3) | (tp.one ? 4ull : 0ull) | 1ull, std::memory_order_relaxed);
     return tp;
 }
-inline TilePlan plan_tiles_search(int64_t m, int tiles_n, int cus) {
-    TilePlan best{m, 8};
-    double best_c = plan_launch_cost(m, 8, tiles_n, cus);
+inline TilePlan plan_tiles_search_priced(int64_t m, int tiles_n, int cus, bool ring3, bool may_mix);
+inline TilePlan plan_tiles_search(int64_t m, int tiles_n, int cus, bool ring3, bool may_mix) {
+    if (ring3 && may_mix && ((m + 255) / 256) * tiles_n >= 3 * (int64_t)cus)
+        return plan_tiles_search_priced(m, tiles_n, cus, true, true);
+    return plan_tiles_search_priced(m, tiles_n, cus, false, false);
+}
+inline TilePlan plan_tiles_search_priced(int64_t m, int tiles_n, int cus, bool ring3, bool may_mix) {
+    TilePlan best{m, 8, false};
+    double best_c = plan_launch_cost(m, 8, tiles_n, cus, ring3);
     const double base_c = best_c;
     const int64_t rows256 = (m + 255) / 256;
     for (int64_t r1 = 0; r1 < rows256; ++r1) {
         const int64_t rows1 = r1 * 256;
-        const double c1 = plan_launch_cost(rows1, 8, tiles_n, cus);
+        const double c1 = plan_launch_cost(rows1, 8, tiles_n, cus, ring3);
         for (int mi = 2; mi <= 8; ++mi) {
             if (rows1 > 0 && mi == 8) continue;
-            const double c = c1 + plan_launch_cost(m - rows1, mi, tiles_n, cus);
-            if (c < best_c - 1e-9) { best_c = c; best = TilePlan{rows1, mi}; }
-        }
-    }
-    if (best_c > (best.rows1 > 0 ? 0.97 : 0.985) * base_c) return TilePlan{m, 8};
+            const bool one = may_mix && rows1 > 0 && mi <= 5;
+            const double c1_one = (double)((r1 * tiles_n + cus - 1) / cus);
+            const double c = (one ? c1_one : c1) + plan_launch_cost(m - rows1, mi, tiles_n, cus, ring3);
+            if (ring3 && c > (rows1 > 0 && !one ? 0.97 : 0.985) * base_c) continue;
+            if (c < best_c - 1e-9) { best_c = c; best = TilePlan{rows1, mi, one}; }
+        }
+    }
+    if (best_c > (best.rows1 > 0 && !best.one ? 0.97 : 0.985) * base_c) return TilePlan{m, 8, false};
     return best;
 }
 
@@ -633,24 +760,24 @@
 int launch_gemm_pp_mi(const GemmParams& p, int mi, hipStream_t st) {
     if constexpr (KEEP) {
         switch (mi) {
-            case 2: return launch_gemm_pp<T, EPI, false, 2, false, true>(p, st);
-            case 3: return launch_gemm_pp<T, EPI, false, 3, false, true>(p, st);
-            case 4: return launch_gemm_pp<T, EPI, false, 4, false, true>(p, st);
-            case 5: return launch_gemm_pp<T, EPI, false, 5, false, true>(p, st);
-            case 6: return launch_gemm_pp<T, EPI, false, 6, false, true>(p, st);
-            case 7: return launch_gemm_pp<T, EPI, false, 7, false, true>(p, st);
+            case 2: return launch_gemm_pp_ring<T, EPI, 2, false, true>(p, st);
+            case 3: return launch_gemm_pp_ring<T, EPI, 3, false, true>(p, st);
+            case 4: return launch_gemm_pp_ring<T, EPI, 4, false, true>(p, st);
+            case 5: return launch_gemm_pp_ring<T, EPI, 5, false, true>(p, st);
+            case 6: return launch_gemm_pp_ring<T, EPI, 6, false, true>(p, st);
+            case 7: return launch_gemm_pp_ring<T, EPI, 7, false, true>(p, st);
             default: return launch_gemm_pp<T, EPI, false, 8, false, true>(p, st);
         }
     }
     if (p.a_tpb > 0) {
         if constexpr (EPI == FINO_EPI_GATED_RESIDUAL) {
             switch (mi) {
-                case 2: return launch_gemm_pp<T, EPI, false, 2, true>(p, st);
-                case 3: return launch_gemm_pp<T, EPI, false, 3, true>(p, st);
-                case 4: return launch_gemm_pp<T, EPI, false, 4, true>(p, st);
-                case 5: return launch_gemm_pp<T, EPI, false, 5, true>(p, st);
-                case 6: return launch_gemm_pp<T, EPI, false, 6, true>(p, st);
-                case 7: return launch_gemm_pp<T, EPI, false, 7, true>(p, st);
+                case 2: return launch_gemm_pp_ring<T, EPI, 2, true>(p, st);
+                case 3: return launch_gemm_pp_ring<T, EPI, 3, true>(p, st);
+                case 4: return launch_gemm_pp_ring<T, EPI, 4, true>(p, st);
+                case 5: return launch_gemm_pp_ring<T, EPI, 5, true>(p, st);
+                case 6: return launch_gemm_pp_ring<T, EPI, 6, true>(p, st);
+                case 7: return launch_gemm_pp_ring<T, EPI, 7, true>(p, st);
                 default: return launch_gemm_pp<T, EPI, false, 8, true>(p, st);
             }
         } else {
@@ -659,12 +786,12 @@
         }
     }
     switch (mi) {
-        case 2: return launch_gemm_pp<T, EPI, false, 2>(p, st);
-        case 3: return launch_gemm_pp<T, EPI, false, 3>(p, st);
-        case 4: return launch_gemm_pp<T, EPI, false, 4>(p, st);
-        case 5: return launch_gemm_pp<T, EPI, false, 5>(p, st);
-        case 6: return launch_gemm_pp<T, EPI, false, 6>(p, st);
-        case 7: return launch_gemm_pp<T, EPI, false, 7>(p, st);
+        case 2: return launch_gemm_pp_ring<T, EPI, 2>(p, st);
+        case 3: return launch_gemm_pp_ring<T, EPI, 3>(p, st);
+        case 4: return launch_gemm_pp_ring<T, EPI, 4>(p, st);
+        case 5: return launch_gemm_pp_ring<T, EPI, 5>(p, st);
+        case 6: return launch_gemm_pp_ring<T, EPI, 6>(p, st);
+        case 7: return launch_gemm_pp_ring<T, EPI, 7>(p, st);
         default: return launch_gemm_pp<T, EPI, false, 8>(p, st);
     }
 }
@@ -707,6 +834,7 @@
     }
     if (!GENERIC && use_pingpong() && fits32) {
         const TilePlan tp = plan_tiles(p.m, p.tiles_n, gemm_device_cus(), tile_m);
+        if (tp.one) return launch_gemm_mix_e<T, KEEP>(p, tp.rows1, tp.mi2, epi, st);
         if (tp.rows1 > 0)
             if (int rc = launch_gemm_rows<T, KEEP>(p, 0, tp.rows1, 8, epi, st)) return rc;
         if (tp.rows1 < p.m) return launch_gemm_rows<T, KEEP>(p, tp.rows1, p.m - tp.rows1, tp.mi2, epi, st);
@@ -770,10 +898,15 @@
 }
 
 extern "C" int fino_gemm_plan(int64_t m, int64_t n, int64_t* rows_256, int* tile_rows_rest) {
-    if (m <= 0 || n <= 0) return FINO_ERR_ARG;
-    const TilePlan tp = plan_tiles(m, (int)((n + BN - 1) / BN), gemm_device_cus());
+    return fino_gemm_plan_launches(m, n, 0, rows_256, tile_rows_rest, nullptr);
+}
+
+extern "C" int fino_gemm_plan_launches(int64_t m, int64_t n, int cus, int64_t* rows_256, int* tile_rows_rest, int* launches) {
+    if (m <= 0 || n <= 0 || cus < 0) return FINO_ERR_ARG;
+    const TilePlan tp = plan_tiles(m, (int)((n + BN - 1) / BN), cus > 0 ? cus : gemm_device_cus());
     if (rows_256) *rows_256 = tp.rows1;
     if (tile_rows_rest) *tile_rows_rest = tp.rows1 < m ? 32 * tp.mi2 : 0;
+    if (launches) *launches = (tp.rows1 > 0 && tp.rows1 < m && !tp.one) ? 2 : 1;
     return FINO_OK;
 }
 
@@ -910,7 +1043,7 @@
     p.group_m = fino_tune_get(FINO_TUNE_GEMM_GROUP_M);
     if (p.group_m <= 0) p.group_m = gemm_default_group_m(p.tiles_n, k);
     hipStream_t st = (hipStream_t)stream;
-    const TilePlan tp = plan_tiles(p.m, p.tiles_n, gemm_device_cus(), tile_m);
+    const TilePlan tp = plan_tiles(p.m, p.tiles_n, gemm_device_cus(), tile_m, false);
     auto rows = [&](int64_t r0, int64_t nr, int mi) {
         return dtype == FINO_BF16 ? launch_gemm_rows<BF16>(p, r0, nr, mi, FINO_EPI_GATED_RESIDUAL, st)
                                   : launch_gemm_rows<F16>(p, r0, nr, mi, FINO_EPI_GATED_RESIDUAL, st);
diff --git a/frameino_amd/csrc/fino_gemm_common.h b/frameino_amd/csrc/fino_gemm_common.h
--- a/frameino_amd/csrc/fino_gemm_common.h
+++ b/frameino_amd/csrc/fino_gemm_common.h
@@ -90,15 +90,18 @@
     const int xcd = orig & 7, q = nwg >> 3, rr = nwg & 7;
     return (xcd < rr ? xcd * (q + 1) : rr * (q + 1) + (xcd - rr) * q) + (orig >> 3);
 }
-__device__ __forceinline__ void tile_raster(const GemmParams& p, int id, int& tm, int& tn) {
+__device__ __forceinline__ void tile_raster_rows(const GemmParams& p, int tiles_m, int id, int& tm, int& tn) {
     const int GROUP_M = (p.group_m & 0xff) > 0 ? (p.group_m & 0xff) : 4;
     const int group = id / (GROUP_M * p.tiles_n);
     const int first_m = group * GROUP_M;
-    const int gsz = (p.tiles_m - first_m) < GROUP_M ? (p.tiles_m - first_m) : GROUP_M;
+    const int gsz = (tiles_m - first_m) < GROUP_M ? (tiles_m - first_m) : GROUP_M;
     const int in_group = id - group * GROUP_M * p.tiles_n;
     tm = first_m + in_group % gsz;
     tn = in_group / gsz;
-    if (p.group_m & 0x100) tm = p.tiles_m - 1 - tm;
+    if (p.group_m & 0x100) tm = tiles_m - 1 - tm;
+}
+__device__ __forceinline__ void tile_raster(const GemmParams& p, int id, int& tm, int& tn) {
+    tile_raster_rows(p, p.tiles_m, id, tm, tn);
 }
 __device__ __forceinline__ void tile_coords(const GemmParams& p, int& tm, int& tn) {
     tile_raster(p, xcd_remap((int)blockIdx.x, p.tiles_m * p.tiles_n), tm, tn);
diff --git a/frameino_amd/ops.py b/frameino_amd/ops.py
--- a/frameino_amd/ops.py
+++ b/frameino_amd/ops.py
@@ -561,6 +561,14 @@
     r, t = ctypes.c_int64(), ctypes.c_int()
     _lib.check(_lib.lib().fino_gemm_plan(m, n, ctypes.byref(r), ctypes.byref(t)), "fino_gemm_plan")
     return r.value, t.value
+
+
+def gemm_plan_launches(m, n, cus=0):
+    import ctypes
+    r, t, l = ctypes.c_int64(), ctypes.c_int(), ctypes.c_int()
+    _lib.check(_lib.lib().fino_gemm_plan_launches(m, n, cus, ctypes.byref(r), ctypes.byref(t), ctypes.byref(l)),
+               "fino_gemm_plan_launches")
+    return r.value, t.value, l.value
 
 
 def gemm(a, w, bias=None, epilogue=EPI_NONE, residual=None, gate=None, sel=None, out=None, out2=None, split=0, tile_m=0,
diff --git a/include/frameino_hip.h b/include/frameino_hip.h
--- a/include/frameino_hip.h
+++ b/include/frameino_hip.h
@@ -20,7 +20,8 @@
 const char* fino_last_error(void);
 
 enum { FINO_TUNE_GEMM_GROUP_M = 0, FINO_TUNE_GEMM_RASTER = 1, FINO_TUNE_CONV_LOOP = 2, FINO_TUNE_GEMM_TILE_M = 3,
-       FINO_TUNE_ATTN_KERNEL = 4, FINO_TUNE_ATTN_FP8_KERNEL = 5, FINO_TUNE_ATTN_WALK_GRID = 6, FINO_TUNE_COUNT = 8 };
+       FINO_TUNE_ATTN_KERNEL = 4, FINO_TUNE_ATTN_FP8_KERNEL = 5, FINO_TUNE_ATTN_WALK_GRID = 6, FINO_TUNE_GEMM_RING = 7,
+       FINO_TUNE_COUNT = 8 };
 int fino_tune_set(int key, int value);
 int fino_tune_get(int key);
 
@@ -160,6 +161,7 @@
                         const int32_t* sel, int dtype, int tile_m, void* stream);
 
 int fino_gemm_plan(int64_t m, int64_t n, int64_t* rows_256, int* tile_rows_rest);
+int fino_gemm_plan_launches(int64_t m, int64_t n, int cus, int64_t* rows_256, int* tile_rows_rest, int* launches);
 int fino_skinny_linear(const float* x, const void* w, const void* b, float* y, int m, int64_t n, int64_t k,
                        int w_dtype, int silu_input, void* stream);
 
```

After: 3.797 denoise-steps/s, median of 6. About the same (+0.7%).
